# PhucNguyenAH/tacotron2_subword

Hardware: AMD Instinct MI355X
Metric: mel_frames_per_sec_train (higher is better)
Workload: dtype bf16; 1 GPU; BERT_Tacotron2 default hparams (SMA), full training iteration fwd+loss+bwd+clip+Adam, B=64/GPU, 100 phones, 60 sub-word tokens, 400 frames, 80-mel; global_batch=64, frames_per_item=400, parallelism=dp1, torch_ops=loss reductions, cat/transpose copies, persistent_chains=True, recurrent_steps_bf16=True

## Files before the change

include/t2amd.h:

```cpp
#ifndef T2AMD_H
#define T2AMD_H
#include <stddef.h>
#include <stdint.h>

#ifdef __cplusplus
extern "C" {
#endif

#define T2_ATTN_SMA 0
#define T2_ATTN_LSA 1
#define T2_ATTN_DCA 4
#define T2_ATTN_GMM 3
#define T2_ATTN_FWD2 2

enum {
    T2_SITE_PRENET1 = 1, T2_SITE_PRENET2 = 2, T2_SITE_PRENET1_SUB = 3, T2_SITE_PRENET2_SUB = 4,
    T2_SITE_ATT_H = 5, T2_SITE_ATT_C = 6, T2_SITE_ATT_H_SUB = 7, T2_SITE_ATT_C_SUB = 8,
    T2_SITE_DEC_H = 9, T2_SITE_DEC_C = 10, T2_SITE_NOISE = 11, T2_SITE_NOISE_SUB = 12,
    T2_SITE_ENC0 = 16,
    T2_SITE_ENCSUB0 = 20,
    T2_SITE_POSTNET0 = 24
};

const char* t2_last_error(void);
// ... 107 lines not shown
int t2_decoder_forward(const t2_dims* dims, const t2_decoder_weights* w, const t2_decoder_fwd_args* a, void* stream);

typedef struct t2_lstm_grads { float *w_ih, *w_hh, *b_ih, *b_hh; } t2_lstm_grads;
typedef struct t2_attention_grads { float *wq, *wm, *v, *loc_conv, *loc_dense, *mlp_b1, *mlp_w2, *mlp_b2, *dca_T, *dca_bT, *dca_P; } t2_attention_grads;
typedef struct t2_decoder_grads {
    float *prenet_w1, *prenet_w2, *prenet_sub_w1, *prenet_sub_w2;
    t2_lstm_grads att, att_sub;
    t2_attention_grads attn, attn_sub;
    t2_lstm_grads dec;
    float *proj_w, *proj_b, *gate_w, *gate_b;
} t2_decoder_grads;
typedef struct t2_decoder_bwd_layout {
    size_t total_floats;
    size_t ddout, ddin, dgd, dga, dgas, dctx, dctxs, dq, dqs, dv, dvs, dpm, dpms, carry, carrys;
    size_t carryc, carrycs, dlconv, dlconvs, dldense, dldenses;
    size_t dcd, dca, dcas, partd, parta, dp2, dp2s, dp1, dmel_t, dgate_t, dg16a, dg16d, colsum_ws, gemm_ws, gemm_ws_floats;
    size_t chain, chain_floats;
} t2_decoder_bwd_layout;
int t2_decoder_bwd_layout_query(const t2_dims* dims, int B, int T, int Tin, int Tsub, t2_decoder_bwd_layout* out);
typedef struct t2_decoder_bwd_args {
    int B, T, Tin, Tsub;
    const float* memory; const float* memory_sub;
    const float* align; const float* align_sub;
    const float* d_mel;
    const float* d_gate;
    const float* d_align;
    const float* d_align_sub;
    float* d_memory;
    float* d_memory_sub;
    const float* ws;
    float* bws;
    int training; int prenet_dropout; uint64_t seed;
    int defer_weight_grads;
} t2_decoder_bwd_args;
int t2_decoder_backward(const t2_dims* dims, const t2_decoder_weights* w, const t2_decoder_grads* g,
                        const t2_decoder_bwd_args* a, void* stream);

typedef struct t2_decoder_infer_args {
    int B, Tin, Tsub, max_steps, poll_every;
    float gate_threshold;
    const float* memory; const float* memory_sub;
    const int32_t* mem_lengths; const int32_t* sub_lengths;
    float* mel_out;
    float* gate_out;
    float* align;
    float* align_sub;
    int32_t* stop_index;
    int32_t* done_count;
    float* ws;
    int prenet_dropout; uint64_t seed;
    int* steps_run_host;
} t2_decoder_infer_args;
int t2_decoder_infer(const t2_dims* dims, const t2_decoder_weights* w, const t2_decoder_infer_args* a, void* stream);

int t2_finalize_bct(const float* in_btc, float* out_bct, int B, int T, int C, const int32_t* lengths, float fill, void* stream);
int t2_mask_bt(float* x, int B, int T, const int32_t* lengths, float fill, void* stream);

typedef struct t2_conv_bn_args {
    int B, T, Cin, Cout, K;
    const float* x;
    const float* w; const float* bias;
    const float* gamma; const float* beta;
    float* run_mean; float* run_var;
    int training; float eps; int act; float drop_p; uint64_t seed; uint32_t site;
    const float* residual;
    float* z; float* mean; float* invstd; float* var;
    float* y;
    float* ws; size_t ws_floats;
    const void* x16; void* y16; int handoff;
} t2_conv_bn_args;
int t2_conv_bn_forward(const t2_conv_bn_args* a, void* stream);
typedef struct t2_conv_bn_bwd_args {
    int B, T, Cin, Cout, K;
    const float* x; const float* w; const float* gamma; const float* beta;
    const float* z; const float* mean; const float* invstd;
    int training; float eps; int act; float drop_p; uint64_t seed; uint32_t site;
    const float* dy;
    float* dw; float* dbias; float* dgamma; float* dbeta;
    float* dx; int dx_accumulate;
    float* ws; size_t ws_floats;
    const void* x16; int handoff;
} t2_conv_bn_bwd_args;
int t2_conv_bn_backward(const t2_conv_bn_bwd_args* a, void* stream);

int t2_embedding_forward(const int64_t* ids, const float* table, float* out, int rows, int dim, void* stream);
int t2_embedding_backward(const int64_t* ids, const float* dout, float* dtable, int rows, int dim, int vocab, void* stream);

typedef struct t2_lstm_seq_args {
    int nstreams, B, T, H;
    const float* pre[4];
    const float* w_hh[4];
    int reverse[4];
    const int32_t* lengths;
    float* h[4]; long ldh;
    float* c[4];
    float* gates[4];
    float* ws; size_t ws_floats;
} t2_lstm_seq_args;
size_t t2_lstm_seq_chain_ws_floats(int nstreams, int B, int H, int backward);
int t2_lstm_seq_forward(const t2_lstm_seq_args* a, void* stream);
typedef struct t2_lstm_seq_bwd_args {
    int nstreams, B, T, H;
    const float* w_hh[4]; int reverse[4];
    const float* h[4]; long ldh; const float* c[4]; const float* gates[4];
    const float* dh[4]; long lddh;
    float* dpre[4];
    float* dw_hh[4];
    float* ws; size_t ws_floats;
} t2_lstm_seq_bwd_args;
int t2_lstm_seq_backward(const t2_lstm_seq_bwd_args* a, void* stream);

typedef struct t2_gemm_args {
    const float* A; const float* B; float* C; int M, N, K;
    long sam, sak, sbn, sbk, ldc; int batch; long bsA, bsB, bsC;
    float alpha, beta; const float* bias; int act; int crow_mod; long crow_mul;
    float* ws; size_t ws_bytes; int splitk;
} t2_gemm_args;
int t2_gemm_ex(const t2_gemm_args* a, void* stream);
int t2_prof_gemm(const t2_gemm_args* a, int reps, float* ms_total, float* ms_kernel, void* stream);
enum { T2_GEMM_F32_64 = 0, T2_GEMM_F32_128, T2_GEMM_BF16CONV, T2_GEMM_SRC128, T2_GEMM_SRC256, T2_GEMM_SRC256KM };
enum { T2_GEMM_OPERAND_FP32 = 0, T2_GEMM_OPERAND_STAGED, T2_GEMM_OPERAND_CALLER };
typedef struct t2_gemm_plan_opts {
    int conv_a, conv_b, conv_T, conv_C, fp32_only;
    int a16, b16; long lda16, ldb16; int a16_kmajor, b16_kmajor, split16;
} t2_gemm_plan_opts;
typedef struct t2_gemm_plan_info {
    int kernel; const char* name;
    int split;
    int splitk, kchunks;
    int a_src, b_src;
    size_t stage_bytes_a, stage_bytes_b;
} t2_gemm_plan_info;
int t2_gemm_plan(const t2_gemm_args* a, const t2_gemm_plan_opts* opts, t2_gemm_plan_info* out);
enum { T2_CHAIN_LSTM = 0, T2_CHAIN_SMA, T2_CHAIN_LSA, T2_CHAIN_ENC };
enum { T2_CHAIN_FORWARD = 0, T2_CHAIN_BACKWARD };
enum { T2_CHAIN_OK = 0, T2_CHAIN_REFUSE_SHAPE, T2_CHAIN_REFUSE_NO_INSTANCE, T2_CHAIN_REFUSE_DEVICE, T2_CHAIN_REFUSE_CLAIM,
       T2_CHAIN_REFUSE_QUERY_PART, T2_CHAIN_REFUSE_LDS, T2_CHAIN_REFUSE_LSA_RESIDENT, T2_CHAIN_REFUSE_SHORT_MEMORY,
       T2_CHAIN_REFUSE_LSA_SPLIT, T2_CHAIN_REFUSE_NO_SAVED_TILES, T2_CHAIN_REFUSE_WORKSPACE, T2_CHAIN_REFUSALS };
enum { T2_CHAIN_PARTS = 11 };
typedef struct t2_chain_shape {
    int kind, dec, NS, B, H, E, A, P, M, Hd, F, Kc, Tin[2];
    int saved_tiles;
    size_t ws_floats;
} t2_chain_shape;
typedef struct t2_chain_plan_info {
    int covered, reason; const char* reason_text;
    int instance; const char* instance_name; int grid; size_t lds_bytes;
    int UT, RT, CS, MT, lds_Tc, lds_Tin, lds_Jp, lds_Jm, Jp[2], Jm[2];
    size_t q_bytes, total_bytes, ws_bytes;
    size_t part_off[T2_CHAIN_PARTS], part_bytes[T2_CHAIN_PARTS]; const char* part_name[T2_CHAIN_PARTS];
    size_t clear_off, clear_bytes, pass_clear_bytes[3];
} t2_chain_plan_info;
int t2_chain_plan(const t2_chain_shape* shape, int direction, int cus, int claimed, int no_resident, t2_chain_plan_info* out);
enum { T2_PASS_FORWARD = 0, T2_PASS_BACKWARD, T2_PASS_INFER };
enum { T2_PASS_MAX_BOUNDS = 64 };
typedef struct t2_pass_env {
    int precision, split_steps, chain, chain_bwd, overlap, cus, claimed, no_resident, saved_tiles;
} t2_pass_env;
typedef struct t2_pass_chain {
    int asked, on, reason; const char* reason_text;
    int instance; const char* instance_name; int grid;
} t2_pass_chain;
typedef struct t2_scratch_carve {
    size_t w_ih16_off, w_ih16_bytes, dg16_off, dg16_bytes, rest_off, rest_bytes, total_bytes;
} t2_scratch_carve;
typedef struct t2_decoder_pass_plan_info {
    t2_decoder_layout layout; t2_decoder_bwd_layout bwd_layout;
    int use16, split, pre16;
    t2_scratch_carve scratch;
    t2_pass_chain chain_a, chain_b;
    int chained, clear, saves_tiles, overlap;
    int nbounds, bounds[T2_PASS_MAX_BOUNDS];
    int poison_words, poll; size_t shadow_floats;
    int defer, share, chunk_cast; size_t ddin_ws_off, ddin_ws_bytes;
    int dec_wgrads, dec_wgrads_staged, tail_on_side, tail_share;
    t2_scratch_carve tail_scratch;
    int nsplit, lsa_chain, dq_parts;
} t2_decoder_pass_plan_info;
int t2_decoder_pass_plan(const t2_dims* dims, int pass, int B, int T, int Tin, int Tsub, const t2_pass_env* env, int defer_weight_grads,
                         int poll_every, t2_decoder_pass_plan_info* out);
int t2_conv_handoff_plan(const t2_gemm_args* a, const t2_gemm_plan_opts* opts, int* taken, t2_gemm_plan_info* out);
int t2_colsum(const float* x, long ld, int M, int N, float* out, float* scratch, void* stream);
int t2_mask_btc(float* x, int B, int T, int C, const int32_t* lengths, float fill, void* stream);

typedef struct t2_softdtw_plan_info {
    int threads;
    int rows_per_thread;
    int passes;
    size_t d_floats;
    size_t r_floats;
    size_t e_floats;
} t2_softdtw_plan_info;
int t2_softdtw_plan(int B, int N, int M, float gamma, int need_grad, t2_softdtw_plan_info* out);
typedef struct t2_softdtw_dist_args {
    int B, N, M, d;
    const float* x;
    const float* y;
    float* Ds;
} t2_softdtw_dist_args;
int t2_softdtw_dist(const t2_softdtw_dist_args* a, void* stream);
typedef struct t2_softdtw_fwd_args {
// ... 428 lines not shown
```

tacotron2_subword_amd/_lib.py:

```python
from __future__ import annotations

import ctypes as C
import os

import torch

_HERE = os.path.dirname(os.path.abspath(__file__))
LIB_PATH = os.environ.get("T2AMD_LIB") or os.path.join(_HERE, "libt2amd.so")

ATTN_SMA, ATTN_LSA, ATTN_FWD2, ATTN_GMM, ATTN_DCA = 0, 1, 2, 3, 4

SITE = dict(PRENET1=1, PRENET2=2, PRENET1_SUB=3, PRENET2_SUB=4, ATT_H=5, ATT_C=6, ATT_H_SUB=7, ATT_C_SUB=8,
            DEC_H=9, DEC_C=10, NOISE=11, NOISE_SUB=12, ENC0=16, ENCSUB0=20, POSTNET0=24)

_fp = C.POINTER(C.c_float)
_ip = C.POINTER(C.c_int32)


class Dims(C.Structure):
    _fields_ = [("n_mel", C.c_int), ("prenet_dim", C.c_int), ("enc_dim", C.c_int), ("att_rnn_dim", C.c_int),
                ("dec_rnn_dim", C.c_int), ("att_dim", C.c_int), ("loc_filters", C.c_int), ("loc_kernel", C.c_int),
                ("attention_kind", C.c_int), ("p_att_dropout", C.c_float), ("p_dec_dropout", C.c_float),
                ("p_prenet_dropout", C.c_float), ("n_streams", C.c_int),
                ("score_mask_value", C.c_float), ("score_mask_value_sub", C.c_float), ("score_mask_given", C.c_int)]
# ... 15 lines not shown
                ("dec", LstmWeights), ("proj_w", C.c_void_p), ("proj_b", C.c_void_p), ("gate_w", C.c_void_p), ("gate_b", C.c_void_p)]


_LAYOUT_FIELDS = ["total_floats", "x", "p1", "p2", "p1s", "p2s", "pm", "pms", "prea", "preas", "ga", "gas",
                  "cna", "cnas", "ca", "cas", "din", "psel", "psels", "wcum", "wcums", "pred", "gd", "cnd", "cd",
                  "dout", "qs", "qss", "qpart", "w1t", "w16a", "w16as", "w16d", "wt16a", "wt16as", "wt16d", "din16", "dh16",
                  "gemm_ws", "gemm_ws_floats", "chain", "chain_floats", "usave", "usaves", "locsave", "locsaves"]


class DecoderLayout(C.Structure):
    _fields_ = [(n, C.c_size_t) for n in _LAYOUT_FIELDS]


class DecoderFwdArgs(C.Structure):
    _fields_ = [("B", C.c_int), ("T", C.c_int), ("Tin", C.c_int), ("Tsub", C.c_int),
                ("memory", C.c_void_p), ("memory_sub", C.c_void_p), ("mem_lengths", C.c_void_p), ("sub_lengths", C.c_void_p),
                ("mels", C.c_void_p), ("mel_out", C.c_void_p), ("gate_out", C.c_void_p), ("align", C.c_void_p),
                ("align_sub", C.c_void_p), ("ws", C.c_void_p), ("training", C.c_int), ("prenet_dropout", C.c_int),
                ("seed", C.c_uint64), ("phase", C.c_int)]


class DecoderInferArgs(C.Structure):
    _fields_ = [("B", C.c_int), ("Tin", C.c_int), ("Tsub", C.c_int), ("max_steps", C.c_int), ("poll_every", C.c_int),
                ("gate_threshold", C.c_float),
                ("memory", C.c_void_p), ("memory_sub", C.c_void_p), ("mem_lengths", C.c_void_p), ("sub_lengths", C.c_void_p),
                ("mel_out", C.c_void_p), ("gate_out", C.c_void_p), ("align", C.c_void_p), ("align_sub", C.c_void_p),
                ("stop_index", C.c_void_p), ("done_count", C.c_void_p), ("ws", C.c_void_p),
                ("prenet_dropout", C.c_int), ("seed", C.c_uint64), ("steps_run_host", C.POINTER(C.c_int))]


class LstmGrads(C.Structure):
    _fields_ = LstmWeights._fields_


class AttentionGrads(C.Structure):
    _fields_ = AttentionWeights._fields_


class DecoderGrads(C.Structure):
    _fields_ = [("prenet_w1", C.c_void_p), ("prenet_w2", C.c_void_p), ("prenet_sub_w1", C.c_void_p), ("prenet_sub_w2", C.c_void_p),
                ("att", LstmGrads), ("att_sub", LstmGrads), ("attn", AttentionGrads), ("attn_sub", AttentionGrads),
                ("dec", LstmGrads), ("proj_w", C.c_void_p), ("proj_b", C.c_void_p), ("gate_w", C.c_void_p), ("gate_b", C.c_void_p)]


_BWD_LAYOUT_FIELDS = ["total_floats", "ddout", "ddin", "dgd", "dga", "dgas", "dctx", "dctxs", "dq", "dqs", "dv", "dvs",
                      "dpm", "dpms", "carry", "carrys", "carryc", "carrycs", "dlconv", "dlconvs", "dldense", "dldenses", "dcd", "dca", "dcas", "partd", "parta", "dp2", "dp2s", "dp1",
                      "dmel_t", "dgate_t", "dg16a", "dg16d", "colsum_ws", "gemm_ws", "gemm_ws_floats", "chain", "chain_floats"]


class DecoderBwdLayout(C.Structure):
    _fields_ = [(n, C.c_size_t) for n in _BWD_LAYOUT_FIELDS]


class DecoderBwdArgs(C.Structure):
    _fields_ = [("B", C.c_int), ("T", C.c_int), ("Tin", C.c_int), ("Tsub", C.c_int),
                ("memory", C.c_void_p), ("memory_sub", C.c_void_p), ("align", C.c_void_p), ("align_sub", C.c_void_p),
                ("d_mel", C.c_void_p), ("d_gate", C.c_void_p), ("d_align", C.c_void_p), ("d_align_sub", C.c_void_p),
                ("d_memory", C.c_void_p), ("d_memory_sub", C.c_void_p), ("ws", C.c_void_p), ("bws", C.c_void_p),
                ("training", C.c_int), ("prenet_dropout", C.c_int), ("seed", C.c_uint64), ("defer_weight_grads", C.c_int)]


class ConvBnArgs(C.Structure):
    _fields_ = [("B", C.c_int), ("T", C.c_int), ("Cin", C.c_int), ("Cout", C.c_int), ("K", C.c_int),
                ("x", C.c_void_p), ("w", C.c_void_p), ("bias", C.c_void_p), ("gamma", C.c_void_p), ("beta", C.c_void_p),
                ("run_mean", C.c_void_p), ("run_var", C.c_void_p),
                ("training", C.c_int), ("eps", C.c_float), ("act", C.c_int), ("drop_p", C.c_float), ("seed", C.c_uint64),
                ("site", C.c_uint32), ("residual", C.c_void_p),
                ("z", C.c_void_p), ("mean", C.c_void_p), ("invstd", C.c_void_p), ("var", C.c_void_p), ("y", C.c_void_p),
                ("ws", C.c_void_p), ("ws_floats", C.c_size_t),
                ("x16", C.c_void_p), ("y16", C.c_void_p), ("handoff", C.c_int)]


class ConvBnBwdArgs(C.Structure):
    _fields_ = [("B", C.c_int), ("T", C.c_int), ("Cin", C.c_int), ("Cout", C.c_int), ("K", C.c_int),
                ("x", C.c_void_p), ("w", C.c_void_p), ("gamma", C.c_void_p), ("beta", C.c_void_p),
                ("z", C.c_void_p), ("mean", C.c_void_p), ("invstd", C.c_void_p),
                ("training", C.c_int), ("eps", C.c_float), ("act", C.c_int), ("drop_p", C.c_float), ("seed", C.c_uint64),
                ("site", C.c_uint32), ("dy", C.c_void_p),
                ("dw", C.c_void_p), ("dbias", C.c_void_p), ("dgamma", C.c_void_p), ("dbeta", C.c_void_p),
                ("dx", C.c_void_p), ("dx_accumulate", C.c_int), ("ws", C.c_void_p), ("ws_floats", C.c_size_t),
                ("x16", C.c_void_p), ("handoff", C.c_int)]


_P4 = C.c_void_p * 4
_I4 = C.c_int * 4


class LstmSeqArgs(C.Structure):
    _fields_ = [("nstreams", C.c_int), ("B", C.c_int), ("T", C.c_int), ("H", C.c_int),
                ("pre", _P4), ("w_hh", _P4), ("reverse", _I4), ("lengths", C.c_void_p),
                ("h", _P4), ("ldh", C.c_long), ("c", _P4), ("gates", _P4), ("ws", C.c_void_p), ("ws_floats", C.c_size_t)]


class LstmSeqBwdArgs(C.Structure):
    _fields_ = [("nstreams", C.c_int), ("B", C.c_int), ("T", C.c_int), ("H", C.c_int),
                ("w_hh", _P4), ("reverse", _I4), ("h", _P4), ("ldh", C.c_long), ("c", _P4), ("gates", _P4),
                ("dh", _P4), ("lddh", C.c_long), ("dpre", _P4), ("dw_hh", _P4), ("ws", C.c_void_p), ("ws_floats", C.c_size_t)]


class GemmArgs(C.Structure):
    _fields_ = [("A", C.c_void_p), ("B", C.c_void_p), ("C", C.c_void_p), ("M", C.c_int), ("N", C.c_int), ("K", C.c_int),
                ("sam", C.c_long), ("sak", C.c_long), ("sbn", C.c_long), ("sbk", C.c_long), ("ldc", C.c_long),
                ("batch", C.c_int), ("bsA", C.c_long), ("bsB", C.c_long), ("bsC", C.c_long),
                ("alpha", C.c_float), ("beta", C.c_float), ("bias", C.c_void_p), ("act", C.c_int),
                ("crow_mod", C.c_int), ("crow_mul", C.c_long), ("ws", C.c_void_p), ("ws_bytes", C.c_size_t), ("splitk", C.c_int)]


class GemmPlanOpts(C.Structure):
    _fields_ = [("conv_a", C.c_int), ("conv_b", C.c_int), ("conv_T", C.c_int), ("conv_C", C.c_int), ("fp32_only", C.c_int),
                ("a16", C.c_int), ("b16", C.c_int), ("lda16", C.c_long), ("ldb16", C.c_long),
                ("a16_kmajor", C.c_int), ("b16_kmajor", C.c_int), ("split16", C.c_int)]


class GemmPlanInfo(C.Structure):
    _fields_ = [("kernel", C.c_int), ("name", C.c_char_p), ("split", C.c_int), ("splitk", C.c_int), ("kchunks", C.c_int),
                ("a_src", C.c_int), ("b_src", C.c_int), ("stage_bytes_a", C.c_size_t), ("stage_bytes_b", C.c_size_t)]


CHAIN_PARTS = 11
CHAIN_KINDS = dict(lstm=0, sma=1, lsa=2, enc=3)


class ChainShape(C.Structure):
    _fields_ = [(n, C.c_int) for n in ("kind", "dec", "NS", "B", "H", "E", "A", "P", "M", "Hd", "F", "Kc")] + \
               [("Tin", C.c_int * 2), ("saved_tiles", C.c_int), ("ws_floats", C.c_size_t)]


class ChainPlanInfo(C.Structure):
    _fields_ = [("covered", C.c_int), ("reason", C.c_int), ("reason_text", C.c_char_p),
                ("instance", C.c_int), ("instance_name", C.c_char_p), ("grid", C.c_int), ("lds_bytes", C.c_size_t)] + \
               [(n, C.c_int) for n in ("UT", "RT", "CS", "MT", "lds_Tc", "lds_Tin", "lds_Jp", "lds_Jm")] + \
               [("Jp", C.c_int * 2), ("Jm", C.c_int * 2), ("q_bytes", C.c_size_t), ("total_bytes", C.c_size_t), ("ws_bytes", C.c_size_t),
                ("part_off", C.c_size_t * CHAIN_PARTS), ("part_bytes", C.c_size_t * CHAIN_PARTS), ("part_name", C.c_char_p * CHAIN_PARTS),
                ("clear_off", C.c_size_t), ("clear_bytes", C.c_size_t), ("pass_clear_bytes", C.c_size_t * 3)]


PASS_KINDS = dict(forward=0, backward=1, infer=2)
PASS_MAX_BOUNDS = 64


class PassEnv(C.Structure):
    _fields_ = [(n, C.c_int) for n in ("precision", "split_steps", "chain", "chain_bwd", "overlap", "cus", "claimed", "no_resident", "saved_tiles")]


class PassChain(C.Structure):
    _fields_ = [("asked", C.c_int), ("on", C.c_int), ("reason", C.c_int), ("reason_text", C.c_char_p),
                ("instance", C.c_int), ("instance_name", C.c_char_p), ("grid", C.c_int)]


class ScratchCarve(C.Structure):
    _fields_ = [(n, C.c_size_t) for n in ("w_ih16_off", "w_ih16_bytes", "dg16_off", "dg16_bytes", "rest_off", "rest_bytes", "total_bytes")]


class DecoderPassPlanInfo(C.Structure):
    _fields_ = [("layout", DecoderLayout), ("bwd_layout", DecoderBwdLayout)] + \
               [(n, C.c_int) for n in ("use16", "split", "pre16")] + [("scratch", ScratchCarve), ("chain_a", PassChain), ("chain_b", PassChain)] + \
               [(n, C.c_int) for n in ("chained", "clear", "saves_tiles", "overlap", "nbounds")] + [("bounds", C.c_int * PASS_MAX_BOUNDS)] + \
               [("poison_words", C.c_int), ("poll", C.c_int), ("shadow_floats", C.c_size_t)] + \
               [(n, C.c_int) for n in ("defer", "share", "chunk_cast")] + [("ddin_ws_off", C.c_size_t), ("ddin_ws_bytes", C.c_size_t)] + \
               [(n, C.c_int) for n in ("dec_wgrads", "dec_wgrads_staged", "tail_on_side", "tail_share")] + [("tail_scratch", ScratchCarve)] + \
               [(n, C.c_int) for n in ("nsplit", "lsa_chain", "dq_parts")]


class SoftDtwPlanInfo(C.Structure):
    _fields_ = [("threads", C.c_int), ("rows_per_thread", C.c_int), ("passes", C.c_int),
                ("d_floats", C.c_size_t), ("r_floats", C.c_size_t), ("e_floats", C.c_size_t)]
# ... 183 lines not shown


class WaveglowForwardArgs(C.Structure):
    _fields_ = [("B", C.c_int), ("T", C.c_int), ("n_mel", C.c_int), ("n_samples", C.c_long), ("packed", C.c_void_p), ("logdet_w", C.c_void_p),
                ("mel", C.c_void_p), ("audio", C.c_void_p), ("workspace", C.c_void_p), ("z", C.c_void_p), ("log_s_host", C.POINTER(C.c_void_p)),
                ("logdet", C.c_void_p), ("sigma", C.c_float), ("sums", C.c_void_p), ("nll_item", C.c_void_p), ("loss", C.c_void_p),
                ("kernel_ms_host", C.POINTER(C.c_double))]


class WaveglowHeadArgs(C.Structure):
    _fields_ = [("B", C.c_int), ("n_group", C.c_int), ("n_samples", C.c_long), ("audio", C.c_void_p), ("w", C.c_void_p), ("audio_out", C.c_void_p)]


class WaveglowTailArgs(C.Structure):
    _fields_ = [("B", C.c_int), ("nc", C.c_int), ("n_half", C.c_int), ("L", C.c_int), ("n_peel", C.c_int), ("n_group", C.c_int), ("z_offset", C.c_int),
                ("out", C.c_void_p), ("w_end", C.c_void_p), ("b_end", C.c_void_p), ("audio_in", C.c_void_p), ("w_next", C.c_void_p),
                ("audio_out", C.c_void_p), ("z", C.c_void_p), ("log_s", C.c_void_p), ("part_s", C.c_void_p), ("part_z", C.c_void_p)]


class WaveglowBackwardInfo(C.Structure):
    _fields_ = [("L", C.c_long), ("n_tensors", C.c_int), ("saved_bytes", C.c_size_t), ("workspace_bytes", C.c_size_t), ("grad_floats", C.c_size_t),
                ("packed_bwd_bytes", C.c_size_t), ("n_slots", C.c_size_t)]


class WaveglowTrainForwardArgs(C.Structure):
    _fields_ = [("fwd", WaveglowForwardArgs), ("saved", C.c_void_p)]


class WaveglowBackwardArgs(C.Structure):
    _fields_ = [("B", C.c_int), ("T", C.c_int), ("n_mel", C.c_int), ("n_samples", C.c_long), ("packed", C.c_void_p), ("packed_bwd", C.c_void_p),
                ("saved", C.c_void_p), ("mel", C.c_void_p), ("audio", C.c_void_p), ("dz", C.c_void_p), ("dlog_s_host", C.POINTER(C.c_void_p)),
                ("workspace", C.c_void_p), ("grad", C.c_void_p), ("kernel_ms_host", C.POINTER(C.c_double))]


class WaveglowWeightGradArgs(C.Structure):
    _fields_ = [("B", C.c_int), ("M", C.c_int), ("nc", C.c_int), ("n_cond", C.c_int), ("L", C.c_int), ("taps", C.c_int), ("d", C.c_int),
                ("a_rows", C.c_int), ("x_rows", C.c_int),
                ("a", C.c_void_p), ("x", C.c_void_p), ("spect", C.c_void_p), ("dw_x", C.c_void_p), ("dw_spect", C.c_void_p), ("db", C.c_void_p),
                ("workspace", C.c_void_p), ("db2", C.c_void_p)]


class WaveglowStartBackwardArgs(C.Structure):
    _fields_ = [("B", C.c_int), ("nc", C.c_int), ("c", C.c_int), ("n_half", C.c_int), ("L", C.c_int), ("dx", C.c_void_p), ("w_start", C.c_void_p),
                ("audio_in", C.c_void_p), ("d_in", C.c_void_p), ("dw_start", C.c_void_p), ("db_start", C.c_void_p), ("workspace", C.c_void_p)]


class WaveglowHeadBackwardArgs(C.Structure):
    _fields_ = [("B", C.c_int), ("n_group", C.c_int), ("n_samples", C.c_long), ("d_in", C.c_void_p), ("audio", C.c_void_p), ("part", C.c_void_p),
                ("dw", C.c_void_p)]


class WaveglowGateBackwardArgs(C.Structure):
    _fields_ = [("B", C.c_int), ("nc", C.c_int), ("L", C.c_int), ("last", C.c_int), ("dx", C.c_void_p), ("d_out", C.c_void_p), ("w_rs", C.c_void_p),
                ("t", C.c_void_p), ("g", C.c_void_p), ("packed_ws", C.c_void_p), ("du", C.c_void_p), ("acts", C.c_void_p)]


class WaveglowConvBackwardArgs(C.Structure):
    _fields_ = [("B", C.c_int), ("nc", C.c_int), ("n_cond", C.c_int), ("L", C.c_int), ("d", C.c_int), ("first_dx", C.c_int), ("first_spect", C.c_int),
                ("du", C.c_void_p), ("w_in", C.c_void_p), ("w_cond", C.c_void_p), ("packed_ws", C.c_void_p), ("dx", C.c_void_p), ("d_spect", C.c_void_p)]


class WaveglowTailBackwardArgs(C.Structure):
    _fields_ = [("B", C.c_int), ("nc", C.c_int), ("n_half", C.c_int), ("L", C.c_int), ("n_peel", C.c_int), ("n_group", C.c_int), ("z_offset", C.c_int),
                ("out", C.c_void_p), ("w_end", C.c_void_p), ("b_end", C.c_void_p), ("audio_in", C.c_void_p), ("w_next", C.c_void_p), ("d_next", C.c_void_p),
                ("dz", C.c_void_p), ("dlog_s", C.c_void_p), ("d_out", C.c_void_p), ("d_in", C.c_void_p), ("part", C.c_void_p), ("dw_end", C.c_void_p),
                ("db_end", C.c_void_p), ("dw_next", C.c_void_p)]


class WaveglowUpsampleBackwardArgs(C.Structure):
    _fields_ = [("B", C.c_int), ("n_mel", C.c_int), ("T", C.c_int), ("n_group", C.c_int), ("n_samples", C.c_long),
                ("mel", C.c_void_p), ("d_spect", C.c_void_p), ("dw", C.c_void_p), ("db", C.c_void_p)]


WAVEGLOW_KERNELS = ("upsample", "start", "gated_conv", "res_skip", "couple")
WAVEGLOW_FORWARD_KERNELS = ("upsample", "start", "gated_conv", "res_skip", "head", "tail", "sums")
WAVEGLOW_BACKWARD_KERNELS = ("tail_backward", "gate_backward", "conv_backward", "cond_backward", "weight_grad", "weight_grad_reduce", "start_backward",
                             "upsample_backward")
WAVEGLOW_GATED, WAVEGLOW_RES_SKIP, WAVEGLOW_UPSAMPLE = 0, 1, 2

ABI_VERSION = 4

EXPORTS = ["t2_last_error", "t2_version", "t2_chain_status", "t2_chain_status_clear", "t2_debug_report_abort", "t2_debug_occupy", "t2_chain_claimed", "t2_set_precision", "t2_get_precision", "t2_gemm_counts", "t2_set_gemm_split_min_mflop", "t2_set_split_steps", "t2_get_split_steps", "t2_step_counts", "t2_set_overlap", "t2_set_chain", "t2_get_chain", "t2_set_chain_bwd", "t2_set_gemm_staging", "t2_set_gemm_fold", "t2_set_bn_fuse", "t2_get_bn_fuse", "t2_bn_fuse_counts", "t2_side_join", "t2_defer_counts", "t2_decoder_layout_query", "t2_decoder_forward", "t2_decoder_infer",
           "t2_decoder_bwd_layout_query", "t2_decoder_backward", "t2_decoder_pass_plan", "t2_prof_enable", "t2_prof_collect", "t2_adam_chunks", "t2_adam_step", "t2_adam_norm",
           "t2_conv_bn_forward", "t2_conv_bn_backward", "t2_embedding_forward", "t2_embedding_backward",
           "t2_lstm_seq_forward", "t2_lstm_seq_backward", "t2_lstm_seq_chain_ws_floats", "t2_gemm_ex", "t2_prof_gemm", "t2_gemm_plan", "t2_chain_plan", "t2_conv_handoff_plan", "t2_colsum", "t2_mask_btc",
           "t2_finalize_bct", "t2_mask_bt", "t2_gemm", "t2_rng_keep_mask", "t2_rng_normal",
           "t2_softdtw_plan", "t2_softdtw_dist", "t2_softdtw_forward", "t2_softdtw_backward", "t2_softdtw_dist_backward",
           "t2_ssim_plan", "t2_ssim_forward", "t2_ssim_backward",
           "t2_bert_plan", "t2_bert_pack", "t2_bert_forward", "t2_bert_embed_ln", "t2_bert_layernorm", "t2_bert_attention",
           "t2_hifigan_plan", "t2_hifigan_pack", "t2_hifigan_forward", "t2_vocoder_packed_floats", "t2_vocoder_conv1d", "t2_vocoder_conv_transpose1d",
           "t2_stft_plan", "t2_stft_pack", "t2_stft_analysis", "t2_stft_synthesis", "t2_melspec_plan", "t2_melspec_pack", "t2_melspec",
           "t2_waveglow_plan", "t2_waveglow_pack", "t2_waveglow_infer", "t2_waveglow_packed_floats", "t2_waveglow_gated_conv", "t2_waveglow_res_skip",
           "t2_waveglow_upsample", "t2_waveglow_couple", "t2_waveglow_forward_plan", "t2_waveglow_forward", "t2_waveglow_logdet",
           "t2_waveglow_logdet_matrices", "t2_waveglow_head", "t2_waveglow_tail",
           "t2_waveglow_backward_plan", "t2_waveglow_grad_offsets", "t2_waveglow_pack_backward", "t2_waveglow_train_forward", "t2_waveglow_backward",
           "t2_waveglow_weight_grad_ws_floats", "t2_waveglow_weight_grad", "t2_waveglow_gate_backward", "t2_waveglow_conv_backward_packed_floats",
           "t2_waveglow_conv_backward", "t2_waveglow_tail_backward", "t2_waveglow_upsample_backward", "t2_waveglow_start_backward", "t2_waveglow_head_backward"]

_lib = None


def lib() -> C.CDLL:
    global _lib
    if _lib is None:
        if not os.path.exists(LIB_PATH):
            raise RuntimeError(f"{LIB_PATH} is missing: the HIP extension must be built (see __graft_entry__.build); "
                               "there is no CPU fallback for the product path")
        L = C.CDLL(LIB_PATH)
        L.t2_last_error.restype = C.c_char_p
        if L.t2_version() != ABI_VERSION:
            raise RuntimeError(f"{LIB_PATH} speaks ABI version {L.t2_version()}, this binding {ABI_VERSION}: rebuild the library "
                               "(the argument structs differ in size between versions)")
        L.t2_chain_status.argtypes = [C.POINTER(C.c_uint32)]
        L.t2_debug_report_abort.argtypes = [C.c_uint32, C.c_void_p]
        L.t2_debug_occupy.argtypes = [C.c_int, C.c_int, C.c_void_p]
        L.t2_gemm.argtypes = [C.c_void_p, C.c_void_p, C.c_void_p, C.c_int, C.c_int, C.c_int, C.c_long, C.c_long, C.c_long,
                              C.c_long, C.c_long, C.c_void_p, C.c_int, C.c_float, C.c_float, C.c_void_p, C.c_size_t,
                              C.c_int, C.c_void_p]
        L.t2_rng_keep_mask.argtypes = [C.c_uint64, C.c_uint32, C.c_uint32, C.c_float, C.c_void_p, C.c_void_p]
        L.t2_rng_normal.argtypes = [C.c_uint64, C.c_uint32, C.c_uint32, C.c_void_p, C.c_void_p]
        L.t2_decoder_layout_query.argtypes = [C.POINTER(Dims), C.c_int, C.c_int, C.c_int, C.c_int, C.POINTER(DecoderLayout)]
        L.t2_decoder_forward.argtypes = [C.POINTER(Dims), C.POINTER(DecoderWeights), C.POINTER(DecoderFwdArgs), C.c_void_p]
        L.t2_decoder_infer.argtypes = [C.POINTER(Dims), C.POINTER(DecoderWeights), C.POINTER(DecoderInferArgs), C.c_void_p]
        L.t2_decoder_bwd_layout_query.argtypes = [C.POINTER(Dims), C.c_int, C.c_int, C.c_int, C.c_int, C.POINTER(DecoderBwdLayout)]
        L.t2_decoder_backward.argtypes = [C.POINTER(Dims), C.POINTER(DecoderWeights), C.POINTER(DecoderGrads),
                                          C.POINTER(DecoderBwdArgs), C.c_void_p]
        L.t2_decoder_pass_plan.argtypes = [C.POINTER(Dims), C.c_int, C.c_int, C.c_int, C.c_int, C.c_int, C.POINTER(PassEnv), C.c_int, C.c_int,
                                           C.POINTER(DecoderPassPlanInfo)]
        L.t2_conv_bn_forward.argtypes = [C.POINTER(ConvBnArgs), C.c_void_p]
        L.t2_conv_bn_backward.argtypes = [C.POINTER(ConvBnBwdArgs), C.c_void_p]
        L.t2_embedding_forward.argtypes = [C.c_void_p, C.c_void_p, C.c_void_p, C.c_int, C.c_int, C.c_void_p]
        L.t2_embedding_backward.argtypes = [C.c_void_p, C.c_void_p, C.c_void_p, C.c_int, C.c_int, C.c_int, C.c_void_p]
        L.t2_lstm_seq_forward.argtypes = [C.POINTER(LstmSeqArgs), C.c_void_p]
        L.t2_lstm_seq_backward.argtypes = [C.POINTER(LstmSeqBwdArgs), C.c_void_p]
        L.t2_lstm_seq_chain_ws_floats.argtypes, L.t2_lstm_seq_chain_ws_floats.restype = [C.c_int, C.c_int, C.c_int, C.c_int], C.c_size_t
        L.t2_gemm_ex.argtypes = [C.POINTER(GemmArgs), C.c_void_p]
        L.t2_prof_gemm.argtypes = [C.POINTER(GemmArgs), C.c_int, C.POINTER(C.c_float), C.POINTER(C.c_float), C.c_void_p]
        L.t2_gemm_plan.argtypes = [C.POINTER(GemmArgs), C.POINTER(GemmPlanOpts), C.POINTER(GemmPlanInfo)]
        L.t2_chain_plan.argtypes = [C.POINTER(ChainShape), C.c_int, C.c_int, C.c_int, C.c_int, C.POINTER(ChainPlanInfo)]
        L.t2_conv_handoff_plan.argtypes = [C.POINTER(GemmArgs), C.POINTER(GemmPlanOpts), C.POINTER(C.c_int), C.POINTER(GemmPlanInfo)]
        L.t2_colsum.argtypes = [C.c_void_p, C.c_long, C.c_int, C.c_int, C.c_void_p, C.c_void_p, C.c_void_p]
        L.t2_mask_btc.argtypes = [C.c_void_p, C.c_int, C.c_int, C.c_int, C.c_void_p, C.c_float, C.c_void_p]
        L.t2_prof_enable.argtypes = [C.c_int]
        L.t2_gemm_counts.argtypes = [C.POINTER(C.c_uint64), C.c_int]
        L.t2_set_split_steps.argtypes = [C.c_int]
        L.t2_step_counts.argtypes = [C.POINTER(C.c_uint64), C.c_int]
        L.t2_bn_fuse_counts.argtypes = [C.POINTER(C.c_uint64), C.c_int]
        L.t2_defer_counts.argtypes = [C.POINTER(C.c_uint64), C.c_int]
        L.t2_set_gemm_split_min_mflop.argtypes = [C.c_int]
        L.t2_prof_collect.argtypes = [C.c_int, C.POINTER(C.c_double), C.POINTER(C.c_int)]
        L.t2_finalize_bct.argtypes = [C.c_void_p, C.c_void_p, C.c_int, C.c_int, C.c_int, C.c_void_p, C.c_float, C.c_void_p]
        L.t2_mask_bt.argtypes = [C.c_void_p, C.c_int, C.c_int, C.c_void_p, C.c_float, C.c_void_p]
        L.t2_softdtw_plan.argtypes = [C.c_int, C.c_int, C.c_int, C.c_float, C.c_int, C.POINTER(SoftDtwPlanInfo)]
        L.t2_softdtw_dist.argtypes = [C.POINTER(SoftDtwDistArgs), C.c_void_p]
        L.t2_softdtw_forward.argtypes = [C.POINTER(SoftDtwFwdArgs), C.c_void_p]
        L.t2_softdtw_backward.argtypes = [C.POINTER(SoftDtwBwdArgs), C.c_void_p]
        L.t2_softdtw_dist_backward.argtypes = [C.POINTER(SoftDtwDistBwdArgs), C.c_void_p]
        L.t2_ssim_plan.argtypes = [C.c_int, C.c_int, C.c_int, C.c_int, C.c_int, C.POINTER(SsimPlanInfo)]
        L.t2_ssim_forward.argtypes = [C.POINTER(SsimFwdArgs), C.c_void_p]
        L.t2_ssim_backward.argtypes = [C.POINTER(SsimBwdArgs), C.c_void_p]
        L.t2_bert_plan.argtypes = [C.POINTER(BertConfig), C.c_int, C.c_long, C.c_int, C.c_int, C.POINTER(BertPlanInfo)]
        L.t2_bert_pack.argtypes = [C.POINTER(BertConfig), C.POINTER(C.c_void_p), C.c_int, C.c_void_p, C.c_void_p]
        L.t2_bert_forward.argtypes = [C.POINTER(BertConfig), C.POINTER(BertFwdArgs), C.c_void_p]
        L.t2_bert_embed_ln.argtypes = [C.POINTER(BertEmbedLnArgs), C.c_void_p]
        L.t2_bert_layernorm.argtypes = [C.POINTER(BertLayernormArgs), C.c_void_p]
        L.t2_bert_attention.argtypes = [C.POINTER(BertAttentionArgs), C.c_void_p]
        L.t2_hifigan_plan.argtypes = [C.POINTER(HifiganConfig), C.c_int, C.c_int, C.POINTER(HifiganPlanInfo)]
        L.t2_hifigan_pack.argtypes = [C.POINTER(HifiganConfig), C.POINTER(C.c_void_p), C.POINTER(C.c_void_p), C.c_int, C.c_void_p, C.c_void_p]
        L.t2_hifigan_forward.argtypes = [C.POINTER(HifiganConfig), C.POINTER(HifiganFwdArgs), C.c_void_p]
        L.t2_vocoder_packed_floats.argtypes, L.t2_vocoder_packed_floats.restype = [C.c_int, C.c_int, C.c_int, C.c_int], C.c_size_t
        L.t2_vocoder_conv1d.argtypes = [C.POINTER(VocoderConvArgs), C.c_void_p]
        L.t2_vocoder_conv_transpose1d.argtypes = [C.POINTER(VocoderConvArgs), C.c_void_p]
        L.t2_stft_plan.argtypes = [C.c_int, C.c_int, C.c_int, C.POINTER(StftPlanInfo)]
        L.t2_stft_pack.argtypes = [C.c_int, C.c_int, C.c_void_p, C.c_void_p, C.c_void_p, C.c_void_p, C.c_void_p]
        L.t2_stft_analysis.argtypes = [C.POINTER(StftAnalysisArgs), C.c_void_p]
        L.t2_stft_synthesis.argtypes = [C.POINTER(StftSynthesisArgs), C.c_void_p]
        L.t2_melspec_plan.argtypes = [C.c_int, C.c_int, C.c_int, C.c_int, C.c_long, C.c_int, C.POINTER(MelspecPlanInfo)]
        L.t2_melspec_pack.argtypes = [C.c_int, C.c_int, C.c_void_p, C.c_void_p, C.c_void_p, C.c_void_p]
        L.t2_melspec.argtypes = [C.POINTER(MelspecArgs), C.c_void_p]
        L.t2_waveglow_plan.argtypes = [C.POINTER(WaveglowConfig), C.c_int, C.c_int, C.POINTER(WaveglowPlanInfo)]
        L.t2_waveglow_pack.argtypes = [C.POINTER(WaveglowConfig), C.POINTER(C.c_void_p), C.c_int, C.c_void_p, C.c_void_p]
        L.t2_waveglow_infer.argtypes = [C.POINTER(WaveglowConfig), C.POINTER(WaveglowInferArgs), C.c_void_p]
        L.t2_waveglow_packed_floats.argtypes, L.t2_waveglow_packed_floats.restype = [C.c_int, C.c_int, C.c_int, C.c_int], C.c_size_t
        L.t2_waveglow_gated_conv.argtypes = [C.POINTER(WaveglowGatedArgs), C.c_void_p]
        L.t2_waveglow_res_skip.argtypes = [C.POINTER(WaveglowResSkipArgs), C.c_void_p]
        L.t2_waveglow_upsample.argtypes = [C.POINTER(WaveglowUpsampleArgs), C.c_void_p]
        L.t2_waveglow_couple.argtypes = [C.POINTER(WaveglowCoupleArgs), C.c_void_p]
        L.t2_waveglow_forward_plan.argtypes = [C.POINTER(WaveglowConfig), C.c_int, C.c_int, C.c_long, C.POINTER(WaveglowForwardInfo)]
        L.t2_waveglow_forward.argtypes = [C.POINTER(WaveglowConfig), C.POINTER(WaveglowForwardArgs), C.c_void_p]
        L.t2_waveglow_logdet.argtypes = [C.POINTER(WaveglowConfig), C.c_void_p, C.c_void_p, C.c_void_p]
        L.t2_waveglow_logdet_matrices.argtypes = [C.c_void_p, C.c_int, C.c_int, C.c_void_p, C.c_void_p]
        L.t2_waveglow_head.argtypes = [C.POINTER(WaveglowHeadArgs), C.c_void_p]
        L.t2_waveglow_tail.argtypes = [C.POINTER(WaveglowTailArgs), C.c_void_p]
        L.t2_waveglow_backward_plan.argtypes = [C.POINTER(WaveglowConfig), C.c_int, C.c_int, C.c_long, C.POINTER(WaveglowBackwardInfo)]
        L.t2_waveglow_grad_offsets.argtypes = [C.POINTER(WaveglowConfig), C.POINTER(C.c_size_t), C.c_int]
        L.t2_waveglow_pack_backward.argtypes = [C.POINTER(WaveglowConfig), C.POINTER(C.c_void_p), C.c_int, C.c_void_p, C.c_void_p]
        L.t2_waveglow_train_forward.argtypes = [C.POINTER(WaveglowConfig), C.POINTER(WaveglowTrainForwardArgs), C.c_void_p]
        L.t2_waveglow_backward.argtypes = [C.POINTER(WaveglowConfig), C.POINTER(WaveglowBackwardArgs), C.c_void_p]
        L.t2_waveglow_weight_grad_ws_floats.argtypes, L.t2_waveglow_weight_grad_ws_floats.restype = [C.c_int] * 6, C.c_size_t
        L.t2_waveglow_weight_grad.argtypes = [C.POINTER(WaveglowWeightGradArgs), C.c_void_p]
        L.t2_waveglow_gate_backward.argtypes = [C.POINTER(WaveglowGateBackwardArgs), C.c_void_p]
        L.t2_waveglow_conv_backward_packed_floats.argtypes, L.t2_waveglow_conv_backward_packed_floats.restype = [C.c_int, C.c_int], C.c_size_t
        L.t2_waveglow_conv_backward.argtypes = [C.POINTER(WaveglowConvBackwardArgs), C.c_void_p]
        L.t2_waveglow_tail_backward.argtypes = [C.POINTER(WaveglowTailBackwardArgs), C.c_void_p]
        L.t2_waveglow_upsample_backward.argtypes = [C.POINTER(WaveglowUpsampleBackwardArgs), C.c_void_p]
        L.t2_waveglow_start_backward.argtypes = [C.POINTER(WaveglowStartBackwardArgs), C.c_void_p]
        L.t2_waveglow_head_backward.argtypes = [C.POINTER(WaveglowHeadBackwardArgs), C.c_void_p]
        _lib = L
    return _lib


def check(rc: int) -> None:
    if rc != 0:
        raise RuntimeError(f"t2amd call failed ({rc}): {lib().t2_last_error().decode()}")


def ptr(t: torch.Tensor | None) -> int | None:
    if t is None:
        return None
# ... 416 lines not shown
```

tacotron2_subword_amd/blocks.py:

```python
from __future__ import annotations

import ctypes as C

import torch

from . import _lib as L

ACT_NONE, ACT_RELU, ACT_TANH = 0, 1, 2
CONV_HANDOFF = True
_WS = {}


def _scratch(dev, n_floats: int) -> torch.Tensor:
    key = (dev, torch.cuda.current_stream(dev).cuda_stream if dev.type == "cuda" else 0)
    t = _WS.get(key)
    if t is None or t.numel() < n_floats:
        t = torch.empty(int(n_floats * 1.25) + 1024, dtype=torch.float32, device=dev)
        _WS[key] = t
    return t


def _stage_terms() -> int:
    return 3 if L.get_precision() == "bf16x3" else 1


def gemm_ex(A, Bm, out, M, N, K, sam, sak, sbn, sbk, ldc, *, bias=None, act=0, alpha=1.0, beta=0.0, crow_mod=0, crow_mul=0,
            batch=1, bsA=0, bsB=0, bsC=0, splitk_ws=True):
    ws = _scratch(out.device, (8 << 20) * _stage_terms()) if splitk_ws and beta == 0.0 else None
    a = L.GemmArgs(L.ptr(A), L.ptr(Bm), L.ptr(out), M, N, K, sam, sak, sbn, sbk, ldc, batch, bsA, bsB, bsC, alpha, beta,
                   L.ptr(bias), act, crow_mod, crow_mul, L.ptr(ws), 0 if ws is None else ws.numel() * 4, 0)
    L.check(L.lib().t2_gemm_ex(C.byref(a), L.stream()))
    return out


def colsum(x2d: torch.Tensor) -> torch.Tensor:
    M, N = x2d.shape
    out = torch.empty(N, dtype=torch.float32, device=x2d.device)
    sc = torch.empty(64 * N, dtype=torch.float32, device=x2d.device)
    L.check(L.lib().t2_colsum(L.ptr(x2d), x2d.stride(0), M, N, L.ptr(out), L.ptr(sc), L.stream()))
    return out


class _LinearFn(torch.autograd.Function):

    @staticmethod
    def forward(ctx, x, W, b):
        shape = x.shape
        x2 = x.reshape(-1, shape[-1]).contiguous()
        M, K = x2.shape
        N = W.shape[0]
        y = torch.empty(M, N, dtype=torch.float32, device=x.device)
        gemm_ex(x2, W, y, M, N, K, K, 1, W.stride(0), 1, N, bias=b)
        ctx.save_for_backward(x2, W)
        ctx.has_bias, ctx.shape = b is not None, shape
        return y.view(*shape[:-1], N)

    @staticmethod
    def backward(ctx, dy):
        x2, W = ctx.saved_tensors
        M, K = x2.shape
        N = W.shape[0]
        dy2 = dy.reshape(M, N).contiguous()
        dx = dW = db = None
        if ctx.needs_input_grad[0]:
            dx = torch.empty(M, K, dtype=torch.float32, device=dy.device)
            gemm_ex(dy2, W, dx, M, K, N, N, 1, 1, W.stride(0), K)
            dx = dx.view(ctx.shape)
        if ctx.needs_input_grad[1]:
            dW = torch.empty(N, K, dtype=torch.float32, device=dy.device)
            gemm_ex(dy2, x2, dW, N, K, M, 1, N, 1, K, K)
        if ctx.has_bias and ctx.needs_input_grad[2]:
            db = colsum(dy2)
        return dx, dW, db


def linear(x, W, b=None):
    return _LinearFn.apply(x, W, b)


class _EmbeddingFn(torch.autograd.Function):
    @staticmethod
    def forward(ctx, ids, table):
        ids = ids.contiguous().long()
        rows, D = ids.numel(), table.shape[1]
        out = torch.empty(*ids.shape, D, dtype=torch.float32, device=table.device)
        L.check(L.lib().t2_embedding_forward(L.ptr(ids), L.ptr(table), L.ptr(out), rows, D, L.stream()))
        ctx.save_for_backward(ids)
        ctx.vocab = table.shape[0]
        return out

    @staticmethod
    def backward(ctx, dout):
        (ids,) = ctx.saved_tensors
        dout = dout.contiguous()
        D = dout.shape[-1]
        dtable = torch.empty(ctx.vocab, D, dtype=torch.float32, device=dout.device)
        L.check(L.lib().t2_embedding_backward(L.ptr(ids), L.ptr(dout), L.ptr(dtable), ids.numel(), D, ctx.vocab, L.stream()))
        return None, dtable


def embedding(ids, table):
    return _EmbeddingFn.apply(ids, table)


class _ConvStackFn(torch.autograd.Function):

    @staticmethod
    def forward(ctx, x, cfg, *params):
        x = x.contiguous()
        B, T, _ = x.shape
        n = len(cfg["acts"])
        dev = x.device
        saved, cur, cur16 = [], x, None
        handoff = CONV_HANDOFF and L.get_precision() == "bf16"
        for i in range(n):
            w, bias, gamma, beta = params[4 * i:4 * i + 4]
            rm, rv = cfg["buffers"][i]
            Cout, Cin, K = w.shape
            M = B * T
            z = torch.empty(M, Cout, dtype=torch.float32, device=dev)
            y = torch.empty(B, T, Cout, dtype=torch.float32, device=dev)
            st = torch.empty(3, Cout, dtype=torch.float32, device=dev)
            nws = Cout * Cin * K + 4 + 128 * Cout + _stage_terms() * ((M * Cin + Cout * Cin * K) // 2) + 4096
            ws = _scratch(dev, nws)
            res = x if (cfg["residual"] and i == n - 1) else None
            y16 = torch.empty(B, T, Cout, dtype=torch.bfloat16, device=dev) if handoff and i + 1 < n else None
            a = L.ConvBnArgs(B, T, Cin, Cout, K, L.ptr(cur), L.ptr(w.detach()), L.ptr(bias.detach()), L.ptr(gamma.detach()),
                             L.ptr(beta.detach()), L.ptr(rm), L.ptr(rv), int(cfg["training"]), 1e-5, cfg["acts"][i],
                             cfg["drop_p"] if cfg["training"] else 0.0, cfg["seed"], cfg["site0"] + i, L.ptr(res),
                             L.ptr(z), L.ptr(st[0]), L.ptr(st[1]), L.ptr(st[2]), L.ptr(y), L.ptr(ws), ws.numel(),
                             L.ptr(cur16), L.ptr(y16), int(handoff))
            L.check(L.lib().t2_conv_bn_forward(C.byref(a), L.stream()))
            saved.append((cur, z, st, cur16))
            cur, cur16 = y, y16
        ctx.cfg, ctx.saved_acts, ctx.params, ctx.handoff = cfg, saved, [p.detach() for p in params], handoff
        return cur

    @staticmethod
    def backward(ctx, dy):
        cfg, params = ctx.cfg, ctx.params
        n = len(cfg["acts"])
        dev = dy.device
        dy = dy.contiguous()
        d_res = dy if cfg["residual"] else None
        grads = [None] * (4 * n)
        for i in range(n - 1, -1, -1):
            w, bias, gamma, beta = params[4 * i:4 * i + 4]
            xin, z, st, xin16 = ctx.saved_acts[i]
            B, T, Cin = xin.shape
            Cout, _, K = w.shape
            M = B * T
            dw, db = torch.empty_like(w), torch.empty_like(bias)
            dg, dbt = torch.empty_like(gamma), torch.empty_like(beta)
            need_dx = i > 0 or ctx.needs_input_grad[0]
            dx = torch.empty(B, T, Cin, dtype=torch.float32, device=dev) if need_dx else None
            nws = M * Cout + Cout * Cin * K + 128 * Cout + 16 + (8 << 20) + _stage_terms() * ((M * (Cout + K * max(Cin, Cout))) // 2) + Cout * Cin * K
            ws = _scratch(dev, nws)
            a = L.ConvBnBwdArgs(B, T, Cin, Cout, K, L.ptr(xin), L.ptr(w), L.ptr(gamma), L.ptr(beta), L.ptr(z), L.ptr(st[0]), L.ptr(st[1]),
                                int(cfg["training"]), 1e-5, cfg["acts"][i], cfg["drop_p"] if cfg["training"] else 0.0, cfg["seed"],
                                cfg["site0"] + i, L.ptr(dy), L.ptr(dw), L.ptr(db), L.ptr(dg), L.ptr(dbt), L.ptr(dx), 0,
                                L.ptr(ws), ws.numel(), L.ptr(xin16), int(ctx.handoff and L.get_precision() == "bf16"))
            L.check(L.lib().t2_conv_bn_backward(C.byref(a), L.stream()))
            grads[4 * i:4 * i + 4] = [dw, db, dg, dbt]
            dy = dx
        if dy is not None and d_res is not None:
            dy = dy + d_res
        ctx.saved_acts = None
        return (dy, None) + tuple(grads)


def conv_bn_stack(x, layers, acts, *, training, drop_p, seed, site0, residual=False):
    params, buffers = [], []
    for conv, bn in layers:
        params += [conv.weight, conv.bias, bn.weight, bn.bias]
        buffers.append((bn.running_mean, bn.running_var))
        if training:
            bn.num_batches_tracked += 1
    cfg = dict(acts=list(acts), buffers=buffers, training=bool(training), drop_p=float(drop_p), seed=int(seed), site0=int(site0),
               residual=bool(residual))
    return _ConvStackFn.apply(x, cfg, *params)


class _BiLstmFn(torch.autograd.Function):

    @staticmethod
    def forward(ctx, x, lengths, w_ih, w_hh, b_ih, b_hh, w_ih_r, w_hh_r, b_ih_r, b_hh_r):
        B, T, E = x.shape
        H = w_hh.shape[1]
        dev = x.device
        xt = x.transpose(0, 1).contiguous()
        pre = torch.empty(2, T * B, 4 * H, dtype=torch.float32, device=dev)
        bsum = torch.stack((b_ih.detach() + b_hh.detach(), b_ih_r.detach() + b_hh_r.detach()))
        for d, W in enumerate((w_ih, w_ih_r)):
            gemm_ex(xt, W.detach(), pre[d], T * B, 4 * H, E, E, 1, W.stride(0), 1, 4 * H, bias=bsum[d])
        out = torch.empty(T, B, 2 * H, dtype=torch.float32, device=dev)
        cells = torch.empty(2, T, B, H, dtype=torch.float32, device=dev)
        gates = torch.empty(2, T, B, 4 * H, dtype=torch.float32, device=dev)
        a = L.LstmSeqArgs()
        a.nstreams, a.B, a.T, a.H = 2, B, T, H
        a.pre[0], a.pre[1] = pre[0].data_ptr(), pre[1].data_ptr()
        a.w_hh[0], a.w_hh[1] = L.ptr(w_hh.detach()), L.ptr(w_hh_r.detach())
        a.reverse[0], a.reverse[1] = 0, 1
        a.lengths = L.ptr(lengths)
        a.h[0], a.h[1] = out.data_ptr(), out.data_ptr() + 4 * H
        a.ldh = 2 * H
        a.c[0], a.c[1] = cells[0].data_ptr(), cells[1].data_ptr()
        a.gates[0], a.gates[1] = gates[0].data_ptr(), gates[1].data_ptr()
        xws = torch.empty(int(L.lib().t2_lstm_seq_chain_ws_floats(2, B, H, 0)), dtype=torch.float32, device=dev)
        a.ws, a.ws_floats = L.ptr(xws), xws.numel()
        L.check(L.lib().t2_lstm_seq_forward(C.byref(a), L.stream()))
        ctx.save_for_backward(xt, out, cells, gates, w_ih, w_hh, w_ih_r, w_hh_r)
        ctx.dims = (B, T, E, H)
        return out.transpose(0, 1).contiguous()

    @staticmethod
    def backward(ctx, dout):
        xt, out, cells, gates, w_ih, w_hh, w_ih_r, w_hh_r = ctx.saved_tensors
        B, T, E, H = ctx.dims
        dev = dout.device
        dh = dout.transpose(0, 1).contiguous()
        dpre = torch.empty(2, T * B, 4 * H, dtype=torch.float32, device=dev)
        dwhh = torch.empty(2, 4 * H, H, dtype=torch.float32, device=dev)
        nws = max(2 * (B * H + 8 * B * H) + 64, int(L.lib().t2_lstm_seq_chain_ws_floats(2, B, H, 1))) + (8 << 20) * _stage_terms()
        ws = _scratch(dev, nws)
        a = L.LstmSeqBwdArgs()
        a.nstreams, a.B, a.T, a.H = 2, B, T, H
        a.w_hh[0], a.w_hh[1] = L.ptr(w_hh), L.ptr(w_hh_r)
        a.reverse[0], a.reverse[1] = 0, 1
        a.h[0], a.h[1] = out.data_ptr(), out.data_ptr() + 4 * H
        a.ldh = 2 * H
        a.c[0], a.c[1] = cells[0].data_ptr(), cells[1].data_ptr()
        a.gates[0], a.gates[1] = gates[0].data_ptr(), gates[1].data_ptr()
        a.dh[0], a.dh[1] = dh.data_ptr(), dh.data_ptr() + 4 * H
        a.lddh = 2 * H
        a.dpre[0], a.dpre[1] = dpre[0].data_ptr(), dpre[1].data_ptr()
        a.dw_hh[0], a.dw_hh[1] = dwhh[0].data_ptr(), dwhh[1].data_ptr()
        a.ws, a.ws_floats = L.ptr(ws), ws.numel()
        L.check(L.lib().t2_lstm_seq_backward(C.byref(a), L.stream()))
        TB = T * B
        dxt = torch.empty(TB, E, dtype=torch.float32, device=dev)
        res = []
        for d, W in enumerate((w_ih, w_ih_r)):
            gemm_ex(dpre[d], W, dxt, TB, E, 4 * H, 4 * H, 1, 1, W.stride(0), E, beta=float(d))
            dW = torch.empty(4 * H, E, dtype=torch.float32, device=dev)
            gemm_ex(dpre[d], xt, dW, 4 * H, E, TB, 1, 4 * H, 1, E, E)
            db = colsum(dpre[d])
            res.append((dW, dwhh[d], db, db))
        dx = dxt.view(T, B, E).transpose(0, 1).contiguous()
        return (dx, None) + res[0] + res[1]


def bilstm(x, lengths, lstm):
    ln = None if lengths is None else lengths.to(dtype=torch.int32).contiguous()
    return _BiLstmFn.apply(x, ln, lstm.weight_ih_l0, lstm.weight_hh_l0, lstm.bias_ih_l0, lstm.bias_hh_l0,
                           lstm.weight_ih_l0_reverse, lstm.weight_hh_l0_reverse, lstm.bias_ih_l0_reverse, lstm.bias_hh_l0_reverse)
```

tacotron2_subword_amd/build.py:

```python
from __future__ import annotations

import os
import shutil
import subprocess

_HERE = os.path.dirname(os.path.abspath(__file__))
CSRC = os.path.join(_HERE, "csrc")
OUT = os.path.join(_HERE, "libt2amd.so")
SOURCES = ["gemm.hip", "gemm_f32.hip", "gemm_bf16conv.hip", "gemm_dispatch.hip", "lstm.hip", "chain_plan.hip", "chain.hip", "chain_bwd.hip", "chain_enc.hip", "attention.hip", "attention_lsa_bwd.hip", "attention_gmm.hip", "attention_dca.hip", "conv.hip", "elementwise.hip", "infer.hip", "optim.hip", "softdtw.hip", "ssim.hip", "bert.hip", "vocoder.hip", "waveglow.hip", "stft.hip", "melspec.hip", "decoder_plan.hip", "decoder.hip", "c_api.hip"]


def _newest(paths):
    return max(os.path.getmtime(p) for p in paths)


def build(force: bool = False, verbose: bool = False) -> str:
    srcs = [os.path.join(CSRC, s) for s in SOURCES]
    deps = srcs + [os.path.join(CSRC, h) for h in os.listdir(CSRC) if h.endswith(".h")]
    deps.append(os.path.join(os.path.dirname(_HERE), "include", "t2amd.h"))
    if not force and os.path.exists(OUT) and os.path.getmtime(OUT) >= _newest(deps):
        return OUT
    hipcc = shutil.which("hipcc") or "/opt/rocm/bin/hipcc"
    if not os.path.exists(hipcc):
        raise RuntimeError("hipcc not found: cannot build the HIP extension")
    objs = []
    procs = []
    os.makedirs(os.path.join(_HERE, "build"), exist_ok=True)
    for s in srcs:
        o = os.path.join(_HERE, "build", os.path.basename(s) + ".o")
        objs.append(o)
        if not force and os.path.exists(o) and os.path.getmtime(o) >= _newest(deps):
            continue
        cmd = [hipcc, "--offload-arch=gfx950", "-O3", "-std=c++17", "-fPIC", "-Wno-pass-failed"] + os.environ.get("T2_EXTRA_HIPCC_FLAGS", "").split() + ["-c", s, "-o", o]
        if verbose:
            print(" ".join(cmd))
        procs.append((cmd, subprocess.Popen(cmd, stdout=subprocess.PIPE, stderr=subprocess.STDOUT)))
    for cmd, p in procs:
        out, _ = p.communicate()
        if p.returncode != 0:
            raise RuntimeError("hipcc failed: " + " ".join(cmd) + "\n" + out.decode(errors="replace"))
    cmd = [hipcc, "--offload-arch=gfx950", "-shared", "-fPIC", "-o", OUT] + objs
    r = subprocess.run(cmd, stdout=subprocess.PIPE, stderr=subprocess.STDOUT)
    if r.returncode != 0:
        raise RuntimeError("link failed: " + r.stdout.decode(errors="replace"))
    return OUT


if __name__ == "__main__":
    print(build(verbose=True))
```

tacotron2_subword_amd/csrc/c_api.hip:

```cpp
#include <fcntl.h>
#include <stdarg.h>
#include <stdio.h>
#include <sys/file.h>
#include <unistd.h>
#include <stdlib.h>
#include <string.h>

#include "../../include/t2amd.h"
#include "kernels.h"
#include "chain_plan.h"
#include "driver.h"

static thread_local char g_err[512] = "";

void t2_set_error(const char* fmt, ...) {
    va_list ap;
    va_start(ap, fmt);
    vsnprintf(g_err, sizeof(g_err), fmt, ap);
    va_end(ap);
}

#include <algorithm>
#include <mutex>
#include <vector>
// ... 128 lines not shown

extern "C" {

const char* t2_last_error(void) { return g_err; }
int t2_version(void) { return T2_ABI_VERSION; }
int t2_chain_status(uint32_t* out_host) {
    T2_REQUIRE(out_host, "null argument");
    const unsigned* w = chain_sticky_words();
    T2_REQUIRE(w, "t2_chain_status: no status block");
    for (int i = 0; i < 4; ++i) out_host[i] = __atomic_load_n(w + i, __ATOMIC_RELAXED);
    return 0;
}
int t2_chain_status_clear(void) {
    unsigned* w = chain_sticky_words();
    T2_REQUIRE(w, "t2_chain_status_clear: no status block");
    for (int i = 0; i < 4; ++i) __atomic_store_n(w + i, 0u, __ATOMIC_RELAXED);
    return 0;
}
int t2_debug_report_abort(uint32_t code, void* stream) {
    unsigned* w = chain_sticky_words();
    T2_REQUIRE(w, "t2_debug_report_abort: no status block");
    hipLaunchKernelGGL(status_report_kernel, dim3(1), dim3(64), 0, (hipStream_t)stream, w, code);
    T2_LAUNCH_CHECK();
    return 0;
}
int t2_chain_claimed(void) { return chain_device_claim() ? 1 : 0; }
int t2_debug_occupy(int workgroups, int milliseconds, void* stream) {
    T2_REQUIRE(workgroups >= 1 && workgroups <= 256 && milliseconds >= 1 && milliseconds <= 5000, "t2_debug_occupy: 1..256 workgroups, 1..5000 ms");
    unsigned* w = chain_sticky_words();
    T2_REQUIRE(w, "t2_debug_occupy: no status block");
    const size_t smem = 96 * 1024;
    T2_TRY_RC(t2_allow_dynamic_lds(reinterpret_cast<const void*>(occupy_kernel), smem));
    hipLaunchKernelGGL(occupy_kernel, dim3(workgroups), dim3(256), smem, (hipStream_t)stream, (unsigned long long)milliseconds * 100000ull, w + 8);
    T2_LAUNCH_CHECK();
    return 0;
}
int t2_set_precision(int mode) {
    T2_REQUIRE(mode >= 0 && mode <= 2, "t2_set_precision: mode must be 0 (fp32), 1 (bf16 operands) or 2 (split-bf16 large GEMMs), not %d", mode);
    set_precision(mode);
    return 0;
}
int t2_get_precision(void) { return get_precision(); }
int t2_set_gemm_split_min_mflop(int mflop) { set_gemm_split_min_mflop(mflop); return 0; }
int t2_gemm_counts(uint64_t* out_host, int reset) {
    T2_REQUIRE(out_host, "null argument");
    gemm_counts(out_host, reset);
    return 0;
}
int t2_set_split_steps(int on) { g_split_steps = on != 0; return 0; }
int t2_get_split_steps(void) { return g_split_steps; }
int t2_step_counts(uint64_t* out_host, int reset) {
    T2_REQUIRE(out_host, "null argument");
    for (int i = 0; i < 6; ++i) { out_host[i] = g_step_counts[i]; if (reset) g_step_counts[i] = 0; }
    return 0;
}
int t2_set_overlap(int on) { g_overlap = on != 0; return 0; }
int t2_set_chain(int on) { g_chain = on != 0; return 0; }
int t2_get_chain(void) { return g_chain; }
int t2_set_chain_bwd(int on) { g_chain_bwd = on != 0; return 0; }
int t2_set_gemm_staging(int on) { set_gemm_staging(on); return 0; }
int t2_set_gemm_fold(int on) { set_gemm_fold(on); return 0; }
int t2_set_bn_fuse(int on) { set_bn_fuse(on); return 0; }
int t2_get_bn_fuse(void) { return get_bn_fuse(); }
int t2_bn_fuse_counts(uint64_t* out_host, int reset) {
    T2_REQUIRE(out_host, "null argument");
    bn_fuse_counts(out_host, reset);
    return 0;
}
int t2_defer_counts(uint64_t* out_host, int reset) {
    T2_REQUIRE(out_host, "null argument");
    for (int i = 0; i < 2; ++i) { out_host[i] = g_defer_counts[i]; if (reset) g_defer_counts[i] = 0; }
    return 0;
}
int t2_side_join(void* stream) {
    Side* side = nullptr;
    T2_TRY(side_get(&side));
    hipEvent_t e;
    T2_TRY(side_event(*side, 0, &e));
    T2_CHECK_HIP(hipEventRecord(e, side->s));
    T2_CHECK_HIP(hipStreamWaitEvent((hipStream_t)stream, e, 0));
    return 0;
}

int t2_conv_bn_forward(const t2_conv_bn_args* a, void* stream) {
    T2_REQUIRE(a, "null argument");
    const size_t nw = (size_t)a->Cout * a->Cin * a->K;
    T2_REQUIRE(a->ws_floats >= nw + 128 * (size_t)a->Cout, "t2_conv_bn_forward: workspace too small");
    ConvBnFwd f{};
    f.x = a->x; f.B = a->B; f.T = a->T; f.Cin = a->Cin; f.Cout = a->Cout; f.K = a->K;
    f.w = a->w; f.bias = a->bias; f.gamma = a->gamma; f.beta = a->beta; f.run_mean = a->run_mean; f.run_var = a->run_var;
    f.training = a->training; f.eps = a->eps; f.act = a->act; f.drop_p = a->drop_p; f.seed = a->seed; f.site = a->site;
    f.residual = a->residual; f.z = a->z; f.mean = a->mean; f.invstd = a->invstd; f.var = a->var; f.y = a->y;
    f.wperm = a->ws; f.scratch = a->ws + align4(nw);
    const size_t used = align4(nw) + 128 * (size_t)a->Cout;
    if (a->ws_floats > used) { f.gemm_ws = a->ws + used; f.gemm_ws_bytes = (a->ws_floats - used) * sizeof(float); }
    f.handoff = a->handoff; f.x16 = static_cast<const __bf16*>(a->x16); f.y16 = static_cast<__bf16*>(a->y16);
    return conv_bn_fwd(f, (hipStream_t)stream);
}

int t2_conv_bn_backward(const t2_conv_bn_bwd_args* a, void* stream) {
    T2_REQUIRE(a, "null argument");
    const size_t nw = align4((size_t)a->Cout * a->Cin * a->K), ndz = align4((size_t)a->B * a->T * a->Cout), nsc = 128 * (size_t)a->Cout;
    T2_REQUIRE(a->ws_floats >= nw + ndz + nsc, "t2_conv_bn_backward: workspace too small");
    ConvBnBwd f{};
    f.x = a->x; f.B = a->B; f.T = a->T; f.Cin = a->Cin; f.Cout = a->Cout; f.K = a->K;
    f.w = a->w; f.gamma = a->gamma; f.beta = a->beta; f.z = a->z; f.mean = a->mean; f.invstd = a->invstd;
    f.training = a->training; f.eps = a->eps; f.act = a->act; f.drop_p = a->drop_p; f.seed = a->seed; f.site = a->site;
    f.dy = a->dy; f.dw = a->dw; f.dbias = a->dbias; f.dgamma = a->dgamma; f.dbeta = a->dbeta;
    f.dx = a->dx; f.dx_accumulate = a->dx_accumulate;
    f.dz = a->ws; f.wperm = a->ws + ndz; f.scratch = a->ws + ndz + nw;
    f.gemm_ws = a->ws + ndz + nw + nsc; f.gemm_ws_bytes = (a->ws_floats - (ndz + nw + nsc)) * sizeof(float);
    f.handoff = a->handoff; f.x16 = static_cast<const __bf16*>(a->x16);
    return conv_bn_bwd(f, (hipStream_t)stream);
}

int t2_embedding_forward(const int64_t* ids, const float* table, float* out, int rows, int dim, void* stream) {
    return embedding_fwd(reinterpret_cast<const long*>(ids), table, out, rows, dim, (hipStream_t)stream);
}
int t2_embedding_backward(const int64_t* ids, const float* dout, float* dtable, int rows, int dim, int vocab, void* stream) {
    return embedding_bwd(reinterpret_cast<const long*>(ids), dout, dtable, rows, dim, vocab, (hipStream_t)stream);
}

int t2_lstm_seq_forward(const t2_lstm_seq_args* a, void* stream) {
    T2_REQUIRE(a && a->nstreams >= 1 && a->nstreams <= kMaxLstmStreams, "t2_lstm_seq_forward: bad nstreams");
    T2_REQUIRE(a->H % 64 == 0, "t2_lstm_seq_forward: H=%d must be a multiple of 64", a->H);
    const int B = a->B, T = a->T, H = a->H;
    ChainPlan plan{CHAIN_REFUSE_WORKSPACE};
    if (g_chain && a->ws && a->ws_floats) plan = plan_here(plan_enc_chain, enc_chain_shape(a->nstreams, B, H, 0, a->ws_floats * sizeof(float)));
    if (plan.refusal == CHAIN_OK) {
        EncChainDesc d{};
        d.ND = a->nstreams; d.B = B; d.T = T; d.H = H; d.lengths = a->lengths; d.ldh = a->ldh;
        for (int s = 0; s < a->nstreams; ++s) {
            d.pre[s] = a->pre[s]; d.w_hh[s] = a->w_hh[s]; d.reverse[s] = a->reverse[s];
            d.h[s] = a->h[s]; d.c[s] = a->c[s]; d.gates[s] = a->gates[s];
        }
        return enc_chain_fwd(d, plan, a->ws, a->ws_floats, (hipStream_t)stream);
    }
    for (int step = 0; step < T; ++step) {
        LstmStepDesc d{};
        d.nstreams = a->nstreams; d.B = B; d.H = H; d.drop_p = 0.f;
        for (int s = 0; s < a->nstreams; ++s) {
            LstmStream& st = d.st[s];
            const int t = a->reverse[s] ? T - 1 - step : step;
            const int tp = a->reverse[s] ? t + 1 : t - 1;
            st.pre = a->pre[s] + (long)t * B * 4 * H; st.ldpre = 4 * H;
            if (step > 0) {
                st.seg[0] = LstmSeg{a->h[s] + (long)tp * B * a->ldh, a->ldh, a->w_hh[s], (long)H, H};
                st.nseg = 1;
                st.c_prev = a->c[s] + (long)tp * B * H; st.ldc_prev = H;
            }
            st.gates = a->gates[s] + (long)t * B * 4 * H; st.ldgates = 4 * H;
            st.c_out = a->c[s] + (long)t * B * H; st.ldc_out = H;
            st.h_out = a->h[s] + (long)t * B * a->ldh; st.ldh_out = a->ldh;
            st.lengths = a->lengths; st.t = t;
        }
        T2_TRY(lstm_step_fwd(d, (hipStream_t)stream));
    }
    return 0;
}

size_t t2_lstm_seq_chain_ws_floats(int nstreams, int B, int H, int backward) { return enc_chain_ws_floats(nstreams, B, H, backward); }

int t2_lstm_seq_backward(const t2_lstm_seq_bwd_args* a, void* stream) {
    T2_REQUIRE(a && a->nstreams >= 1 && a->nstreams <= kMaxLstmStreams, "t2_lstm_seq_backward: bad nstreams");
    const int B = a->B, T = a->T, H = a->H, ns = a->nstreams;
    const int ks = lstm_bwd_ksplit(4 * H);
    hipStream_t s = (hipStream_t)stream;
    float* dc = a->ws;
    float* part = dc + align4((size_t)ns * B * H);
    float* gws = part + align4((size_t)ns * ks * B * H);
    T2_REQUIRE(a->ws_floats >= (size_t)(gws - a->ws), "t2_lstm_seq_backward: workspace too small");
    const size_t gws_bytes = (a->ws_floats - (size_t)(gws - a->ws)) * sizeof(float);
    ChainPlan plan{CHAIN_REFUSE_WORKSPACE};
    if (g_chain && g_chain_bwd && a->ws_floats) plan = plan_here(plan_enc_chain, enc_chain_shape(ns, B, H, 1, a->ws_floats * sizeof(float)));
    const bool chain = plan.refusal == CHAIN_OK;
    if (chain) {
        EncChainBwdDesc d{};
        d.ND = ns; d.B = B; d.T = T; d.H = H; d.lddh = a->lddh;
        for (int i = 0; i < ns; ++i) {
            d.w_hh[i] = a->w_hh[i]; d.reverse[i] = a->reverse[i]; d.c[i] = a->c[i]; d.gates[i] = a->gates[i];
            d.dh[i] = a->dh[i]; d.dpre[i] = a->dpre[i];
        }
        T2_TRY(enc_chain_bwd(d, plan, a->ws, a->ws_floats, s));
    }
    for (int step = 0; step < (chain ? 0 : T); ++step) {
        LstmBwdPointDesc p{};
        p.nstreams = ns; p.B = B; p.H = H; p.drop_p = 0.f; p.first = step == 0;
        LstmBwdGemmDesc g{};
        g.nstreams = ns; g.B = B; g.H4 = 4 * H; g.KS = ks; g.NC = H;
        for (int i = 0; i < ns; ++i) {
            const int t = a->reverse[i] ? step : T - 1 - step;
            const int tprev = a->reverse[i] ? t + 1 : t - 1;
            const bool has_prev = a->reverse[i] ? (t + 1 < T) : (t > 0);
            LstmBwdStream& st = p.st[i];
            st.dh1 = a->dh[i] + (long)t * B * a->lddh; st.lddh1 = a->lddh;
            st.part = part + (size_t)i * ks * B * H; st.nparts = ks; st.part_stride = (long)B * H; st.ldpart = H; st.part_col = 0;
            st.gates = a->gates[i] + (long)t * B * 4 * H; st.ldgates = 4 * H;
            st.c_new = a->c[i] + (long)t * B * H; st.ldc_new = H;
            if (has_prev) { st.c_prev = a->c[i] + (long)tprev * B * H; st.ldc_prev = H; }
            st.dc_state = dc + (size_t)i * B * H;
            st.dg = a->dpre[i] + (long)t * B * 4 * H; st.lddg = 4 * H;
            g.st[i].dg = st.dg; g.st[i].lddg = 4 * H;
            g.st[i].seg[0] = LstmBwdSeg{a->w_hh[i], (long)H, H}; g.st[i].nseg = 1;
            g.st[i].part = part + (size_t)i * ks * B * H;
        }
        T2_TRY(lstm_bwd_pointwise(p, s));
        if (step + 1 < T) T2_TRY(lstm_bwd_gemm(g, s));
    }
    for (int i = 0; i < ns; ++i) {
        if (T < 2) { T2_TRY(fill_f32(a->dw_hh[i], 0.f, (size_t)4 * H * H, s)); continue; }
        GemmDesc w = gemm_desc();
        const long rowsB = (long)B;
        w.A = a->reverse[i] ? a->dpre[i] : a->dpre[i] + rowsB * 4 * H; w.sam = 1; w.sak = 4 * H;
        w.B = a->reverse[i] ? a->h[i] + rowsB * a->ldh : a->h[i]; w.sbk = a->ldh; w.sbn = 1;
        w.C = a->dw_hh[i]; w.ldc = H; w.M = 4 * H; w.N = H; w.K = (T - 1) * B;
        w.ws = gws; w.ws_bytes = gws_bytes;
        T2_TRY(gemm(w, s));
    }
    return 0;
}

static GemmDesc desc_of(const t2_gemm_args& a) {
    GemmDesc g = gemm_desc();
    g.A = a.A; g.B = a.B; g.C = a.C; g.M = a.M; g.N = a.N; g.K = a.K;
    g.sam = a.sam; g.sak = a.sak; g.sbn = a.sbn; g.sbk = a.sbk; g.ldc = a.ldc;
    g.batch = a.batch > 0 ? a.batch : 1; g.bsA = a.bsA; g.bsB = a.bsB; g.bsC = a.bsC;
    g.alpha = a.alpha; g.beta = a.beta; g.bias1 = a.bias; g.act = a.act;
    g.crow_mod = a.crow_mod; g.crow_mul = a.crow_mul;
    g.ws = a.ws; g.ws_bytes = a.ws_bytes; g.splitk = a.splitk;
    return g;
}
int t2_gemm_ex(const t2_gemm_args* a, void* stream) {
    T2_REQUIRE(a, "null argument");
    return gemm(desc_of(*a), (hipStream_t)stream);
}
static GemmDesc desc_of(const t2_gemm_args& a, const t2_gemm_plan_opts* o) {
    GemmDesc g = desc_of(a);
    if (o) {
        g.conv_a = o->conv_a; g.conv_b = o->conv_b; g.conv_T = o->conv_T; g.conv_C = o->conv_C; g.fp32_only = o->fp32_only;
        const __bf16* copy = reinterpret_cast<const __bf16*>(uintptr_t(256));
        if (o->a16) { g.A16 = copy; g.lda16 = o->lda16; g.a16_kmajor = o->a16_kmajor; }
        if (o->b16) { g.B16 = copy; g.ldb16 = o->ldb16; g.b16_kmajor = o->b16_kmajor; }
        g.split16 = o->split16;
    }
    return g;
}
static t2_gemm_plan_info info_of(const GemmPlan& p) {
    return t2_gemm_plan_info{(int)p.kernel, gemm_plan_name(p), p.split, p.splitk, p.kchunks, (int)p.a.src, (int)p.b.src, p.a.bytes, p.b.bytes};
}
int t2_gemm_plan(const t2_gemm_args* a, const t2_gemm_plan_opts* o, t2_gemm_plan_info* out) {
    T2_REQUIRE(a && out, "null argument");
    GemmPlan p;
    T2_TRY(gemm_plan(desc_of(*a, o), &p));
    *out = info_of(p);
    return 0;
}
int t2_chain_plan(const t2_chain_shape* z, int direction, int cus, int claimed, int no_resident, t2_chain_plan_info* out) {
    T2_REQUIRE(z && out && (direction == T2_CHAIN_FORWARD || direction == T2_CHAIN_BACKWARD), "t2_chain_plan: null argument or bad direction");
    ChainShape c{};
    c.kind = z->kind; c.dec = z->dec; c.NS = z->NS; c.B = z->B; c.H = z->H; c.E = z->E; c.A = z->A; c.P = z->P; c.M = z->M; c.Hd = z->Hd; c.F = z->F; c.Kc = z->Kc;
    c.Tin[0] = z->Tin[0]; c.Tin[1] = z->Tin[1]; c.backward = direction; c.saved_tiles = z->saved_tiles != 0; c.ws_bytes = z->ws_floats * sizeof(float);
    const ChainEnv env{cus, claimed != 0, no_resident != 0};
    const ChainPlan p = z->kind == T2_CHAIN_ENC ? plan_enc_chain(c, env) : direction == T2_CHAIN_BACKWARD ? plan_chain_bwd(c, env) : plan_chain_fwd(c, env);
    t2_chain_plan_info o{};
    o.covered = p.refusal == CHAIN_OK; o.reason = p.refusal; o.reason_text = chain_refusal_text(p.refusal);
    if (o.covered) {
        T2_REQUIRE(p.ws_bytes >= p.total, "t2_chain_plan: exchange space too small (%zu bytes, the chain needs %zu)", p.ws_bytes, p.total);
        o.instance = p.instance; o.instance_name = chain_instance_name(p.instance); o.grid = p.grid; o.lds_bytes = p.lds_bytes;
        o.UT = p.UT; o.RT = p.RT; o.CS = p.CS; o.MT = p.MT; o.lds_Tc = p.lds_Tc; o.lds_Tin = p.lds_Tin; o.lds_Jp = p.lds_Jp; o.lds_Jm = p.lds_Jm;
        for (int s = 0; s < 2; ++s) { o.Jp[s] = p.Jp[s]; o.Jm[s] = p.Jm[s]; }
        o.q_bytes = p.q_bytes; o.total_bytes = p.total; o.ws_bytes = p.ws_bytes;
        static_assert(CHAIN_PARTS == T2_CHAIN_PARTS, "t2_chain_plan_info carries every part");
        for (int i = 0; i < CHAIN_PARTS; ++i) { o.part_off[i] = p.part[i].off; o.part_bytes[i] = p.part[i].bytes; o.part_name[i] = chain_part_name(i); }
        o.clear_off = p.clear.off; o.clear_bytes = p.clear.bytes;
        for (int w = 0; w < 3 && z->kind != T2_CHAIN_ENC && direction == T2_CHAIN_FORWARD; ++w) o.pass_clear_bytes[w] = chain_fwd_clear_range(p.ws_bytes, (ChainWsClear)w).bytes;
    }
    *out = o;
    return 0;
}
int t2_conv_handoff_plan(const t2_gemm_args* a, const t2_gemm_plan_opts* o, int* taken, t2_gemm_plan_info* out) {
    T2_REQUIRE(a && taken && out, "null argument");
    const GemmDesc offered = desc_of(*a, o);
    GemmDesc plain = offered;
    plain.A16 = plain.B16 = nullptr; plain.a16_kmajor = plain.b16_kmajor = 0; plain.lda16 = plain.ldb16 = 0;
    GemmPlan p;
    T2_TRY(gemm_plan(plain, &p));
    *taken = gemm_handoff(plain, offered, &p);
    *out = info_of(p);
    return 0;
}
static int time_gemm(const GemmDesc& g, int reps, float* ms, hipStream_t s) {
    hipEvent_t e0, e1;
    T2_CHECK_HIP(hipEventCreate(&e0)); T2_CHECK_HIP(hipEventCreate(&e1));
    int rc = gemm(g, s);
    T2_CHECK_HIP(hipEventRecord(e0, s));
    for (int i = 0; i < reps && rc == 0; ++i) rc = gemm(g, s);
    T2_CHECK_HIP(hipEventRecord(e1, s));
    T2_CHECK_HIP(hipEventSynchronize(e1));
    T2_CHECK_HIP(hipEventElapsedTime(ms, e0, e1));
    *ms /= reps;
    hipEventDestroy(e0); hipEventDestroy(e1);
    return rc;
}
int t2_prof_gemm(const t2_gemm_args* a, int reps, float* ms_total, float* ms_kernel, void* stream) {
    T2_REQUIRE(a && reps > 0 && ms_total && ms_kernel, "t2_prof_gemm: bad arguments");
    T2_REQUIRE(get_precision() != 0 && a->M % 128 == 0 && a->N % 128 == 0 && a->K % 64 == 0 && (a->batch <= 1) && a->ws,
               "t2_prof_gemm: bf16 or split-bf16 mode, whole-tile shapes and scratch only");
    hipStream_t s = (hipStream_t)stream;
    GemmDesc g = desc_of(*a);
    GemmPlan p, q;
    T2_TRY(gemm_plan(g, &p));
    T2_REQUIRE(p.a.src == GemmSrc::staged && p.b.src == GemmSrc::staged, "t2_prof_gemm: refused, gemm() runs this product on kernel %s, which stages no bf16 copies", gemm_plan_name(p));
    T2_TRY(time_gemm(g, reps, ms_total, s));
    unsigned char* w8 = reinterpret_cast<unsigned char*>(a->ws);
    __bf16* a16 = reinterpret_cast<__bf16*>(w8); __bf16* b16 = reinterpret_cast<__bf16*>(w8 + p.a.bytes);
    T2_TRY(stage_planned(g.A, p.a, p.split, a16, s));
    T2_TRY(stage_planned(g.B, p.b, p.split, b16, s));
    g.A16 = a16; g.lda16 = p.a.ld; g.B16 = b16; g.ldb16 = p.b.ld;
// ... 211 lines not shown
```

tacotron2_subword_amd/csrc/conv.hip:

```cpp
#include "kernels.h"
#include <atomic>
#include <cstdlib>

namespace t2 {

namespace {

inline int env_int(const char* name, int dflt) { const char* v = getenv(name); return v && *v ? atoi(v) : dflt; }
inline int grid_for(size_t n, int block = 256, int cap = 8192) {
    size_t g = (n + block - 1) / block;
    return (int)(g < 1 ? 1 : (g > (size_t)cap ? cap : g));
}

template <class OUT, class IDX>
__global__ void permute_w_fwd_kernel(const float* __restrict__ w, OUT* __restrict__ wp, int Co, int Ci, int K) {
    const IDX n = (IDX)Co * Ci * K;
    for (IDX i = blockIdx.x * (IDX)blockDim.x + threadIdx.x; i < n; i += (IDX)gridDim.x * blockDim.x) {
        const IDX ci = i % (IDX)Ci, r = i / (IDX)Ci, dk = r % (IDX)K, co = r / (IDX)K;
        wp[i] = (OUT)w[(co * Ci + ci) * K + dk];
    }
}
template <class OUT, class IDX>
__global__ void permute_w_bwd_kernel(const float* __restrict__ w, OUT* __restrict__ wt, int Co, int Ci, int K) {
    const IDX n = (IDX)Co * Ci * K;
    for (IDX i = blockIdx.x * (IDX)blockDim.x + threadIdx.x; i < n; i += (IDX)gridDim.x * blockDim.x) {
        const IDX co = i % (IDX)Co, r = i / (IDX)Co, dk = r % (IDX)K, ci = r / (IDX)K;
        wt[i] = (OUT)w[(co * Ci + ci) * K + ((IDX)K - 1 - dk)];
    }
}
template <class OUT>
void permute_w(bool bwd, const float* w, OUT* out, int Co, int Ci, int K, hipStream_t s) {
    const size_t n = (size_t)Co * Ci * K;
    const dim3 grid(grid_for(n)), block(256);
    if (n < (1ull << 31)) {
        if (bwd) hipLaunchKernelGGL((permute_w_bwd_kernel<OUT, uint32_t>), grid, block, 0, s, w, out, Co, Ci, K);
        else hipLaunchKernelGGL((permute_w_fwd_kernel<OUT, uint32_t>), grid, block, 0, s, w, out, Co, Ci, K);
    } else {
        if (bwd) hipLaunchKernelGGL((permute_w_bwd_kernel<OUT, size_t>), grid, block, 0, s, w, out, Co, Ci, K);
        else hipLaunchKernelGGL((permute_w_fwd_kernel<OUT, size_t>), grid, block, 0, s, w, out, Co, Ci, K);
    }
}
__global__ void unpermute_dw_kernel(const float* __restrict__ dwp, float* __restrict__ dw, int Co, int Ci, int K) {
    const size_t n = (size_t)Co * Ci * K;
    for (size_t i = blockIdx.x * (size_t)blockDim.x + threadIdx.x; i < n; i += (size_t)gridDim.x * blockDim.x) {
        const int dk = (int)(i % K); const size_t r = i / K; const int ci = (int)(r % Ci), co = (int)(r / Ci);
        dw[i] = dwp[((size_t)co * K + dk) * Ci + ci];
    }
}

struct BnElem {
    const float* z; const float* mean; const float* invstd; const float* gamma; const float* beta;
    int C; int act; float drop_p; RngKey key;
};
__device__ __forceinline__ float act_fwd(float u, int act) {
    return act == ACT_RELU ? fmaxf(u, 0.f) : (act == ACT_TANH ? tanhf(u) : u);
}

struct BnCol { float mean, inv, ga, be; };
template <int MODE>
__device__ __forceinline__ float colreduce_term(const BnElem& e, const BnCol& k, float scale, float z, float g, uint32_t i,
                                                float& a0, float& a1) {
#pragma clang fp contract(off)
    if (MODE == 0) a0 += z;
    else if (MODE == 1) { const float d = z - k.mean; a0 = fmaf(d, d, a0); }
    else {
        const float xh = (z - k.mean) * k.inv, u = fmaf(xh, k.ga, k.be);
        if (e.drop_p > 0.f) g = rng_keep(e.key, i, e.drop_p) ? g * scale : 0.f;
        if (e.act == ACT_RELU) g = u > 0.f ? g : 0.f;
        else if (e.act == ACT_TANH) { const float t = tanhf(u); g *= fmaf(-t, t, 1.0f); }
        const float gx = g * xh;
        a0 += g; a1 += gx;
    }
    return g;
}
template <int MODE, int V, bool FIN>
__global__ void __launch_bounds__(kColThreads) colreduce_stage1_kernel(BnElem e, const float* __restrict__ dy, float* __restrict__ du,
                                                                       int M, int slabs, float* scratch, float* __restrict__ mean_out) {
    static_assert(!FIN || MODE == 1, "only the centred squares have a sum to finish");
    constexpr int R = MODE == 2 ? (V == 4 ? 8 : 16) : 16;
    static_assert(MODE == 2 || V != 2, "the forward passes run with 16-byte groups or one column per lane");
    const int C = e.C;
    const int lane = threadIdx.x % kColLanes, sub = threadIdx.x / kColLanes;
    const int c = (blockIdx.x * kColLanes + lane) * V;
    const int rows = (M + slabs - 1) / slabs;
    const int m0 = blockIdx.y * rows, m1 = min(M, m0 + rows);
    __shared__ float p0[4][kColLanes * V], p1[4][kColLanes * V];
    __shared__ float fin[FIN ? kColLanes * V : 1];
    if (FIN) {
        block_ordered_sums(scratch, C, slabs, blockIdx.x * kColLanes * V, kColLanes * V, fin);
        __syncthreads();
        scratch += (size_t)slabs * C;
    }
    float a0[V] = {}, a1[V] = {};
    if (c < C) {
        BnCol col[V];
#pragma unroll
        for (int k = 0; k < V; ++k) {
            if (FIN) {
                col[k].mean = fin[lane * V + k] / (float)M;
                if (blockIdx.y == 0 && sub == 0) mean_out[c + k] = col[k].mean;
            } else
                col[k].mean = MODE >= 1 ? e.mean[c + k] : 0.f;
            col[k].inv = MODE == 2 ? e.invstd[c + k] : 0.f; col[k].ga = MODE == 2 ? e.gamma[c + k] : 0.f; col[k].be = MODE == 2 ? e.beta[c + k] : 0.f;
        }
        const float scale = e.drop_p > 0.f ? 1.0f / (1.0f - e.drop_p) : 1.0f;
        struct Row { ColVec<V> z, g; };
        rows_in_flight<R, Row>(m0 + sub, m1,
            [&](int m) {
                const size_t i = (size_t)m * C + c;
                Row r;
                r.z = load_cols<V>(e.z + i);
                if (MODE == 2) r.g = load_cols<V>(dy + i);
                return r;
            },
// ... 169 lines not shown
    if (sub == 0 && c < C) {
#pragma unroll
        for (int k = 0; k < V; ++k) {
            const int l = lane * V + k;
            dbias_part[(size_t)blockIdx.y * C + c + k] = part[0][l] + part[1][l] + part[2][l] + part[3][l];
        }
    }
}
__global__ void invstd_from_var_kernel(const float* var, int C, float eps, float* invstd) {
    const int c = blockIdx.x * blockDim.x + threadIdx.x;
    if (c < C) invstd[c] = 1.0f / sqrtf(var[c] + eps);
}

__global__ void embedding_fwd_kernel(const long* __restrict__ ids, const float* __restrict__ table, float* __restrict__ out, int rows, int D) {
    const size_t n = (size_t)rows * (D / 4);
    for (size_t i = blockIdx.x * (size_t)blockDim.x + threadIdx.x; i < n; i += (size_t)gridDim.x * blockDim.x) {
        const int r = (int)(i / (D / 4)), q = (int)(i % (D / 4));
        reinterpret_cast<f32x4*>(out)[i] = reinterpret_cast<const f32x4*>(table + ids[r] * (long)D)[q];
    }
}
constexpr int kEmbThreads = 256, kEmbWaves = kEmbThreads / 64, kEmbRounds = 32;
template <int V>
__global__ __launch_bounds__(kEmbThreads) void embedding_bwd_kernel(const long* __restrict__ ids, const float* __restrict__ dout,
                                                                    float* __restrict__ dtable, int rows, int D) {
    const int v = blockIdx.x;
    extern __shared__ int hits[];
    __shared__ __attribute__((aligned(16))) int wave_cnt[2][kEmbRounds][kEmbWaves];
    const int tid = threadIdx.x, wave = tid >> 6, lane = tid & 63;
    const unsigned long long below = (1ull << lane) - 1ull;
    int run = 0;
    for (int r0 = 0, it = 0; r0 < rows; r0 += kEmbRounds * kEmbThreads, ++it) {
        long id[kEmbRounds];
#pragma unroll
        for (int j = 0; j < kEmbRounds; ++j) {
            const int r = r0 + j * kEmbThreads + tid;
            id[j] = r < rows ? ids[r] : -1;
        }
        unsigned mine = 0;
#pragma unroll
        for (int j = 0; j < kEmbRounds; ++j) mine |= (id[j] == v ? 1u : 0u) << j;
        int (*wc)[kEmbWaves] = wave_cnt[it & 1];
#pragma unroll
        for (int j = 0; j < kEmbRounds; ++j) {
            const unsigned long long m = __ballot((mine >> j) & 1u);
            if (lane == 0) wc[j][wave] = __popcll(m);
        }
        __syncthreads();
#pragma unroll
        for (int j = 0; j < kEmbRounds; ++j) {
            int base = run, tot = 0;
#pragma unroll
            for (int w = 0; w < kEmbWaves; ++w) { const int cw = wc[j][w]; if (w < wave) base += cw; tot += cw; }
            const bool hit = (mine >> j) & 1u;
            const unsigned long long m = __ballot(hit);
            if (hit) hits[base + __popcll(m & below)] = r0 + j * kEmbThreads + tid;
            run += tot;
        }
    }
    __syncthreads();
    const int nhit = run;
    typedef float vec __attribute__((ext_vector_type(V)));
    for (int c = tid * V; c < D; c += kEmbThreads * V) {
        vec acc = 0.f;
        int h = 0;
        for (; h + 8 <= nhit; h += 8) {
            vec x[8];
#pragma unroll
            for (int j = 0; j < 8; ++j) x[j] = *reinterpret_cast<const vec*>(dout + (size_t)hits[h + j] * D + c);
#pragma unroll
            for (int j = 0; j < 8; ++j) acc += x[j];
        }
        for (; h < nhit; ++h) acc += *reinterpret_cast<const vec*>(dout + (size_t)hits[h] * D + c);
        *reinterpret_cast<vec*>(dtable + (size_t)v * D + c) = acc;
    }
}

bool bn_vectorisable(const BnElem& e, const void* p, const void* q) {
    for (const void* a : {(const void*)e.z, (const void*)e.mean, (const void*)e.invstd, (const void*)e.gamma, (const void*)e.beta, p, q})
        if (!cols_vectorisable(a, e.C, e.C)) return false;
    return true;
}
inline bool aligned8(const void* p) { return (reinterpret_cast<uintptr_t>(p) & 7) == 0; }
inline size_t round256(size_t n) { return (n + 255) & ~(size_t)255; }
inline bool same_route(const GemmPlan& p, const GemmPlan& q) { return p.kernel == q.kernel && p.split == q.split && p.splitk == q.splitk && p.kchunks == q.kchunks; }

std::atomic<int> g_bn_fuse{env_int("T2_BN_FUSE", 1)};
std::atomic<uint64_t> g_bn_counts[3];

inline int col_blocks(int C, int V) { return (C + V * kColLanes - 1) / (V * kColLanes); }
int col_width(int C, int slabs, bool vec, bool narrow) {
    if (!vec) return 1;
    if (narrow && slabs >= 48) {
        for (int v = 4; v > 1; v >>= 1)
            if (col_blocks(C, v) * slabs * (kColThreads / kWave) >= 2048) return v;
        return 1;
    }
    return 4;
}

template <int MODE, bool FIN>
int colreduce_stage1(const BnElem& e, const float* dy, float* du, int M, float* scratch, float* mean_out, int V, hipStream_t s) {
    const int slabs = col_slabs(M);
    const dim3 grid(col_blocks(e.C, V), slabs), block(kColThreads);
    if (V == 4) hipLaunchKernelGGL((colreduce_stage1_kernel<MODE, 4, FIN>), grid, block, 0, s, e, dy, du, M, slabs, scratch, mean_out);
    else if constexpr (MODE == 2) {
        if (V == 2) hipLaunchKernelGGL((colreduce_stage1_kernel<2, 2, false>), grid, block, 0, s, e, dy, du, M, slabs, scratch, mean_out);
        else hipLaunchKernelGGL((colreduce_stage1_kernel<2, 1, false>), grid, block, 0, s, e, dy, du, M, slabs, scratch, mean_out);
    } else hipLaunchKernelGGL((colreduce_stage1_kernel<MODE, 1, FIN>), grid, block, 0, s, e, dy, du, M, slabs, scratch, mean_out);
    T2_LAUNCH_CHECK();
    return 0;
}
template <int MODE>
int colreduce(const BnElem& e, const float* dy, float* du, int M, float eps, float* out0, float* out1, float* scratch, hipStream_t s) {
    const int slabs = col_slabs(M);
    const bool vec = cols_vectorisable(e.z, e.C, e.C) && cols_vectorisable(dy, e.C, e.C) && cols_vectorisable(du, e.C, e.C);
    T2_TRY_RC((colreduce_stage1<MODE, false>(e, dy, du, M, scratch, nullptr, col_width(e.C, slabs, vec, false), s)));
    hipLaunchKernelGGL(colreduce_stage2_kernel, dim3((e.C + 255) / 256), dim3(256), 0, s, scratch, e.C, slabs, M, MODE, eps, out0, out1,
                       (const float*)nullptr, 0.f, (float*)nullptr, (float*)nullptr);
    T2_LAUNCH_CHECK();
    return 0;
}

}

void set_bn_fuse(int on) { g_bn_fuse = on != 0; }
int get_bn_fuse() { return g_bn_fuse; }
void bn_fuse_counts(uint64_t* out, int reset) {
    for (int i = 0; i < 3; ++i) { out[i] = g_bn_counts[i]; if (reset) g_bn_counts[i] = 0; }
}

int conv_bn_fwd(const ConvBnFwd& a, hipStream_t s) {
    const int M = a.B * a.T;
    T2_REQUIRE(a.Cin % 4 == 0 && a.K % 2 == 1, "conv_bn_fwd: Cin=%d must be a multiple of 4 and the kernel size odd (%d)", a.Cin, a.K);
    T2_REQUIRE((size_t)M * a.Cout < (1ull << 32), "conv_bn_fwd: B*T*Cout too large for 32-bit RNG indices");
    const size_t nw = (size_t)a.Cout * a.Cin * a.K;
    GemmDesc g = gemm_desc();
    g.A = a.x; g.conv_a = 1; g.conv_T = a.T; g.conv_C = a.Cin; g.conv_pad = (a.K - 1) / 2;
    g.B = a.wperm; g.sbn = (long)a.K * a.Cin; g.sbk = 1;
    g.C = a.z; g.ldc = a.Cout; g.M = M; g.N = a.Cout; g.K = a.K * a.Cin; g.bias1 = a.bias;
    g.ws = a.gemm_ws; g.ws_bytes = a.gemm_ws_bytes;
    GemmDesc g16 = g;
    g16.A16 = a.x16; g16.lda16 = a.Cin;
    g16.B16 = reinterpret_cast<const __bf16*>(a.wperm); g16.ldb16 = (long)a.K * a.Cin;
    if (a.handoff && gemm_handoff(g, g16)) {
        g = g16;
        permute_w(false, a.w, reinterpret_cast<__bf16*>(a.wperm), a.Cout, a.Cin, a.K, s);
    } else
        permute_w(false, a.w, a.wperm, a.Cout, a.Cin, a.K, s);
    T2_LAUNCH_CHECK();
    T2_TRY_RC(gemm(g, s));
    BnElem e{a.z, a.mean, a.invstd, a.gamma, a.beta, a.Cout, a.act, a.drop_p, rng_key(a.seed, a.site)};
    const size_t n = (size_t)M * a.Cout;
    if (a.training && get_bn_fuse()) {
        const int slabs = col_slabs(M);
        const int V = col_width(e.C, slabs, cols_vectorisable(e.z, e.C, e.C), false);
        T2_TRY_RC((colreduce_stage1<0, false>(e, nullptr, nullptr, M, a.scratch, nullptr, V, s)));
        T2_TRY_RC((colreduce_stage1<1, true>(e, nullptr, nullptr, M, a.scratch, a.mean, V, s)));
        hipLaunchKernelGGL(colreduce_stage2_kernel, dim3((a.Cout + 255) / 256), dim3(256), 0, s, a.scratch + (size_t)slabs * e.C, a.Cout, slabs, M, 1,
                           a.eps, a.invstd, a.var, a.mean, 0.1f, a.run_mean, a.run_var);
        T2_LAUNCH_CHECK();
        ++g_bn_counts[0];
    } else if (a.training) {
        T2_TRY_RC(colreduce<0>(e, nullptr, nullptr, M, a.eps, a.mean, nullptr, a.scratch, s));
        T2_TRY_RC(colreduce<1>(e, nullptr, nullptr, M, a.eps, a.invstd, a.var, a.scratch, s));
        if (a.run_mean) {
            hipLaunchKernelGGL(bn_running_kernel, dim3((a.Cout + 255) / 256), dim3(256), 0, s, a.mean, a.var, a.Cout, M, 0.1f, a.run_mean, a.run_var);
            T2_LAUNCH_CHECK();
        }
    } else {
        T2_CHECK_HIP(hipMemcpyAsync(a.mean, a.run_mean, sizeof(float) * a.Cout, hipMemcpyDeviceToDevice, s));
        hipLaunchKernelGGL(invstd_from_var_kernel, dim3((a.Cout + 255) / 256), dim3(256), 0, s, a.run_var, a.Cout, a.eps, a.invstd);
        T2_LAUNCH_CHECK();
    }
    if (bn_vectorisable(e, a.residual, a.y) && aligned8(a.y16))
        hipLaunchKernelGGL(bn_apply_kernel<4>, dim3(grid_for(n / 4)), dim3(256), 0, s, e, a.residual, a.y, a.y16, n);
    else
        hipLaunchKernelGGL(bn_apply_kernel<1>, dim3(grid_for(n)), dim3(256), 0, s, e, a.residual, a.y, a.y16, n);
    T2_LAUNCH_CHECK();
    return 0;
}

int conv_bn_bwd(const ConvBnBwd& a, hipStream_t s) {
    const int M = a.B * a.T;
    const size_t n = (size_t)M * a.Cout;
    BnElem e{a.z, a.mean, a.invstd, a.gamma, a.beta, a.Cout, a.act, a.drop_p, rng_key(a.seed, a.site)};
    GemmDesc g = gemm_desc();
    g.A = a.dz; g.sam = 1; g.sak = a.Cout;
    g.B = a.x; g.conv_b = 1; g.conv_T = a.T; g.conv_C = a.Cin; g.conv_pad = (a.K - 1) / 2;
    g.C = a.wperm; g.ldc = (long)a.K * a.Cin; g.M = a.Cout; g.N = a.K * a.Cin; g.K = M;
    g.ws = a.gemm_ws; g.ws_bytes = a.gemm_ws_bytes;
    const bool fold = get_gemm_fold() != 0;
    if (fold) { g.C = a.dw; g.ccol_mod = a.Cin; g.ccol_mul = a.K; }
    GemmDesc h = gemm_desc();
    h.A = a.dz; h.conv_a = 1; h.conv_T = a.T; h.conv_C = a.Cout; h.conv_pad = (a.K - 1) / 2;
    h.B = a.wperm; h.sbn = (long)a.K * a.Cout; h.sbk = 1;
    h.C = a.dx; h.ldc = a.Cin; h.M = M; h.N = a.Cin; h.K = a.K * a.Cout;
    h.beta = a.dx_accumulate ? 1.f : 0.f;
    h.ws = a.gemm_ws; h.ws_bytes = a.gemm_ws_bytes;
    if (a.dx) T2_REQUIRE(a.Cout % 4 == 0, "conv_bn_bwd: Cout=%d must be a multiple of 4", a.Cout);
    __bf16* dz16 = nullptr;
    bool w16 = false;
    const size_t dz16_bytes = round256(n * sizeof(__bf16));
    if (a.handoff && a.gemm_ws && (reinterpret_cast<uintptr_t>(a.gemm_ws) & 15) == 0 && a.gemm_ws_bytes >= dz16_bytes) {
        float* behind = a.gemm_ws + dz16_bytes / sizeof(float);
        GemmDesc g16 = g, h16 = h;
        g16.ws = h16.ws = behind; g16.ws_bytes = h16.ws_bytes = a.gemm_ws_bytes - dz16_bytes;
        g16.A16 = h16.A16 = reinterpret_cast<const __bf16*>(a.gemm_ws);
        g16.lda16 = a.Cout; g16.a16_kmajor = 1; h16.lda16 = a.Cout;
        g16.B16 = a.x16; g16.ldb16 = a.Cin; g16.b16_kmajor = 1;
        h16.B16 = reinterpret_cast<const __bf16*>(a.wperm); h16.ldb16 = (long)a.K * a.Cout;
        const bool tw = gemm_handoff(g, g16);
        bool tx = a.dx && gemm_handoff(h, h16);
        if (tx && !tw) {
            GemmDesc gb = g;
            gb.ws = behind; gb.ws_bytes = g16.ws_bytes;
            if (same_route(plan_gemm(g), plan_gemm(gb))) g = gb; else tx = false;
        }
        if (tw) g = g16;
        if (tx) { h = h16; w16 = true; }
        if (tw || tx) dz16 = reinterpret_cast<__bf16*>(a.gemm_ws);
    }
    const size_t nw = (size_t)a.Cout * a.Cin * a.K;
    if (get_bn_fuse()) {
        const int slabs = col_slabs(M);
        const bool vec = cols_vectorisable(e.z, e.C, e.C) && cols_vectorisable(a.dy, e.C, e.C) && cols_vectorisable(a.dz, e.C, e.C);
        const int V = col_width(e.C, slabs, vec, true);
        T2_TRY_RC((colreduce_stage1<2, false>(e, a.dy, a.dz, M, a.scratch, nullptr, V, s)));
        float* part = (size_t)a.Cin * a.K >= 64 ? a.wperm : nullptr;
        const dim3 grid(col_blocks(e.C, V), slabs), block(kColThreads);
        if (V == 4) hipLaunchKernelGGL(bn_bwd_dz_cols_kernel<4>, grid, block, 0, s, e, a.dz, a.scratch, M, slabs, a.training, a.dz, dz16, a.dbeta, a.dgamma, part);
        else if (V == 2) hipLaunchKernelGGL(bn_bwd_dz_cols_kernel<2>, grid, block, 0, s, e, a.dz, a.scratch, M, slabs, a.training, a.dz, dz16, a.dbeta, a.dgamma, part);
        else hipLaunchKernelGGL(bn_bwd_dz_cols_kernel<1>, grid, block, 0, s, e, a.dz, a.scratch, M, slabs, a.training, a.dz, dz16, a.dbeta, a.dgamma, part);
        T2_LAUNCH_CHECK();
        if (part) T2_TRY_RC(colsum_finish(part, M, a.Cout, a.dbias, s));
        else T2_TRY_RC(colsum(a.dz, a.Cout, M, a.Cout, a.dbias, nullptr, a.scratch, s));
        ++g_bn_counts[part ? 1 : 2];
    } else {
        T2_TRY_RC(colreduce<2>(e, a.dy, a.dz, M, a.eps, a.dbeta, a.dgamma, a.scratch, s));
        if (bn_vectorisable(e, a.dz, a.dbeta) && cols_vectorisable(a.dgamma, e.C, e.C))
            hipLaunchKernelGGL(bn_bwd_dz_kernel<4>, dim3(grid_for(n / 4)), dim3(256), 0, s, e, a.dz, a.dbeta, a.dgamma, M, a.training, a.dz, dz16, n);
        else
            hipLaunchKernelGGL(bn_bwd_dz_kernel<1>, dim3(grid_for(n)), dim3(256), 0, s, e, a.dz, a.dbeta, a.dgamma, M, a.training, a.dz, dz16, n);
        T2_LAUNCH_CHECK();
        T2_TRY_RC(colsum(a.dz, a.Cout, M, a.Cout, a.dbias, nullptr, a.scratch, s));
    }
    T2_TRY_RC(gemm(g, s));
    if (!fold) {
        hipLaunchKernelGGL(unpermute_dw_kernel, dim3(grid_for(nw)), dim3(256), 0, s, a.wperm, a.dw, a.Cout, a.Cin, a.K);
        T2_LAUNCH_CHECK();
    }
    if (a.dx) {
        if (w16) permute_w(true, a.w, reinterpret_cast<__bf16*>(a.wperm), a.Cout, a.Cin, a.K, s);
        else permute_w(true, a.w, a.wperm, a.Cout, a.Cin, a.K, s);
        T2_LAUNCH_CHECK();
        T2_TRY_RC(gemm(h, s));
    }
    return 0;
}

int embedding_fwd(const long* ids, const float* table, float* out, int rows, int D, hipStream_t s) {
    T2_REQUIRE(D % 4 == 0, "embedding: dim %d must be a multiple of 4", D);
    hipLaunchKernelGGL(embedding_fwd_kernel, dim3(grid_for((size_t)rows * (D / 4))), dim3(256), 0, s, ids, table, out, rows, D);
    T2_LAUNCH_CHECK();
    return 0;
}
int embedding_bwd(const long* ids, const float* dout, float* dtable, int rows, int D, int vocab, hipStream_t s) {
    const size_t smem = (size_t)rows * sizeof(int);
    T2_REQUIRE(smem <= 150 * 1024, "embedding_bwd: %d tokens do not fit the LDS hit list", rows);
    const bool vec = cols_vectorisable(dout, D, D) && cols_vectorisable(dtable, D, D);
    const void* fn = vec ? reinterpret_cast<const void*>(embedding_bwd_kernel<4>) : reinterpret_cast<const void*>(embedding_bwd_kernel<1>);
    T2_TRY_RC(t2_allow_dynamic_lds(fn, smem));
    if (vec) hipLaunchKernelGGL(embedding_bwd_kernel<4>, dim3(vocab), dim3(kEmbThreads), smem, s, ids, dout, dtable, rows, D);
    else hipLaunchKernelGGL(embedding_bwd_kernel<1>, dim3(vocab), dim3(kEmbThreads), smem, s, ids, dout, dtable, rows, D);
    T2_LAUNCH_CHECK();
    return 0;
}

}
```

tacotron2_subword_amd/csrc/decoder.hip:

```cpp
#include <stdlib.h>
#include <string.h>

#include <algorithm>
#include <mutex>
#include <unordered_map>
#include <vector>

#include "../../include/t2amd.h"
#include "kernels.h"
#include "chain_plan.h"
#include "decoder_plan.h"
#include "driver.h"

using namespace t2;

__global__ __launch_bounds__(256) void poison_if_aborted_kernel(const unsigned* __restrict__ status, int nwords, float* __restrict__ a, size_t na,
                                                                float* __restrict__ b, size_t nb) {
    unsigned any = 0;
    for (int i = 0; i < nwords; ++i) any |= status[i];
    if (!any) return;
    const float qnan = __builtin_nanf("");
    for (size_t i = (size_t)blockIdx.x * 256 + threadIdx.x; i < na; i += (size_t)gridDim.x * 256) a[i] = qnan;
    for (size_t i = (size_t)blockIdx.x * 256 + threadIdx.x; i < nb; i += (size_t)gridDim.x * 256) b[i] = qnan;
}
// ... 60 lines not shown
void saved_tiles_note(const void* ws, bool saved) {
    std::lock_guard<std::mutex> lk(g_saved_mu);
    if (g_saved_tiles.size() > 4096) g_saved_tiles.clear();
    g_saved_tiles[ws] = saved;
}
bool saved_tiles_have(const void* ws) {
    std::lock_guard<std::mutex> lk(g_saved_mu);
    auto it = g_saved_tiles.find(ws);
    return it != g_saved_tiles.end() && it->second;
}

PassEnv pass_env_here(const void* fwd_ws, bool device) {
    PassEnv env{get_precision(), g_split_steps != 0, g_chain != 0, g_chain_bwd != 0, g_overlap != 0, ChainEnv{0, false, false}, fwd_ws && saved_tiles_have(fwd_ws)};
    if (device && env.chain) env.chain_env = chain_env(false);
    return env;
}
template <class Plan>
auto pass_plan_here(PassEnv env, Plan plan) {
    auto p = plan(env);
    if (p.chain_a.on || p.chain_b.on) { env.chain_env = chain_env(true); p = plan(env); }
    return p;
}

void shape_into(const ChainShape& z, ChainDesc* d) {
    d->kind = z.kind; d->dec = z.dec; d->NS = z.NS; d->B = z.B; d->H = z.H; d->E = z.E; d->A = z.A; d->P = z.P; d->M = z.M; d->Hd = z.Hd; d->F = z.F; d->Kc = z.Kc;
    d->st[0].Tin = z.Tin[0]; d->st[1].Tin = z.Tin[1];
}
void shape_into(const ChainShape& z, ChainBwdDesc* d) {
    d->kind = z.kind; d->NS = z.NS; d->B = z.B; d->H = z.H; d->E = z.E; d->A = z.A; d->F = z.F; d->Kc = z.Kc;
    d->st[0].Tin = z.Tin[0]; d->st[1].Tin = z.Tin[1];
}

struct Dec {
    const t2_dims& d; const t2_decoder_weights& w; const DecPlan p; float* ws;
    bool training; bool prenet_dropout; uint64_t seed; hipStream_t s;
    int max_pos;
    const Sizes& z = p.z; const t2_decoder_layout& L = p.L; const InferShadows& I = p.I; const bool teacher = p.teacher;
    StreamRef st[2]{};
    hipStream_t sd = nullptr;
    Dec(const Dec&) = delete;
    __bf16* RowA(int parity, int s) const { return reinterpret_cast<__bf16*>(ws + I.rows_a) + (size_t)(parity * 2 + s) * z.B * I.Ka; }
    __bf16* RowD(int parity) const { return reinterpret_cast<__bf16*>(ws + I.rows_d) + (size_t)parity * z.B * I.Kd; }
    float* P(size_t off) const { return ws + off; }
    __bf16* P16(size_t off) const { return reinterpret_cast<__bf16*>(ws + off); }
    unsigned char* scratch(size_t off) const { return reinterpret_cast<unsigned char*>(ws + L.gemm_ws) + off; }
    GemmDesc in(const ScratchPart& part, GemmDesc m) const { m.ws = reinterpret_cast<float*>(scratch(part.off)); m.ws_bytes = part.bytes; return m; }
    long R(int t) const { return (long)t * z.B; }
};

GemmDesc product(const float* A, long sam, long sak, const float* B, long sbn, long sbk, float* C, long ldc, int M, int N, int K) {
    GemmDesc g = gemm_desc();
    g.A = A; g.sam = sam; g.sak = sak;
    g.B = B; g.sbn = sbn; g.sbk = sbk;
    g.C = C; g.ldc = ldc; g.M = M; g.N = N; g.K = K;
    return g;
}
GemmDesc linear(const float* X, long ldx, const float* W, long ldw, float* Y, long ldy, int M, int N, int K) {
    return product(X, ldx, 1, W, ldw, 1, Y, ldy, M, N, K);
}

int prenet(const Dec& c, int s, const float* X, long ldx, int M, float* P1, float* P2, long ldp, uint32_t base, uint32_t mstride) {
    const Sizes& z = c.z; const StreamRef& r = c.st[s];
    auto layer = [&](const float* in, long ldin, const float* W, int K, float* out, uint32_t site) {
        GemmDesc g = linear(in, ldin, W, K, out, ldp, M, z.P, K);
        g.act = ACT_RELU;
        if (c.prenet_dropout) {
            g.drop_p = c.d.p_prenet_dropout; g.seed = c.seed; g.site = site;
            g.drop_base = base; g.drop_mstride = mstride;
        }
        return gemm(g, c.s);
    };
    T2_TRY(layer(X, ldx, r.prenet_w1, z.M, P1, r.site_p1));
    return layer(P1, ldp, r.prenet_w2, z.P, P2, r.site_p2);
}

int cast_part(const float* src, long lds, __bf16* dst, size_t lo, long ldd, int rows, int cols, bool transpose, bool split, hipStream_t s) {
    if (split) return transpose ? cast_transpose_split_bf16(src, lds, dst, dst + lo, ldd, rows, cols, s) : cast_rows_split_bf16(src, lds, dst, dst + lo, ldd, rows, cols, s);
    return transpose ? cast_transpose_bf16(src, lds, dst, ldd, rows, cols, s) : cast_rows_bf16(src, lds, dst, ldd, rows, cols, s);
}
int cast_shadows(const Dec& c, bool split) {
    const Sizes& z = c.z;
    const long K = z.Ha + z.E, ldi = z.P + z.E;
    const size_t loa = (size_t)4 * z.Ha * K, lod = (size_t)4 * z.Hd * z.Hd;
    for (int s = 0; s < z.NS; ++s) {
        const t2_lstm_weights& lw = *c.st[s].lw;
        __bf16 *f = c.P16(c.st[s].w16), *tr = c.P16(c.st[s].wt16);
        T2_TRY(cast_part(lw.w_hh, z.Ha, f, loa, K, 4 * z.Ha, z.Ha, false, split, c.s));
        T2_TRY(cast_part(lw.w_ih + z.P, ldi, f + z.Ha, loa, K, 4 * z.Ha, z.E, false, split, c.s));
        T2_TRY(cast_part(lw.w_ih + z.P, ldi, tr, loa, 4 * z.Ha, 4 * z.Ha, z.E, true, split, c.s));
        T2_TRY(cast_part(lw.w_hh, z.Ha, tr + (long)z.E * 4 * z.Ha, loa, 4 * z.Ha, 4 * z.Ha, z.Ha, true, split, c.s));
    }
    T2_TRY(cast_part(c.w.dec.w_hh, z.Hd, c.P16(c.L.w16d), lod, z.Hd, 4 * z.Hd, z.Hd, false, split, c.s));
    return cast_part(c.w.dec.w_hh, z.Hd, c.P16(c.L.wt16d), lod, 4 * z.Hd, 4 * z.Hd, z.Hd, true, split, c.s);
}

AttnKind kernel_kind(int kind) {
    return kind == T2_ATTN_GMM ? AttnKind::GMM : kind == T2_ATTN_DCA ? AttnKind::DCA : kind == T2_ATTN_SMA ? AttnKind::SMA : AttnKind::LSA;
}

DcaWeights dca_weights(const t2_attention_weights& aw) {
    DcaWeights w{};
    w.bW = aw.mlp_b1; w.V = aw.mlp_w2; w.F = aw.loc_conv; w.U = aw.loc_dense; w.T = aw.dca_T; w.bT = aw.dca_bT; w.v = aw.v; w.P = aw.dca_P;
    return w;
}

int att_lstm_step(const Dec& c, int t) {
    const Sizes& z = c.z; const t2_decoder_layout& L = c.L;
    LstmStepDesc d{};
    d.nstreams = z.NS; d.B = z.B; d.H = z.Ha; d.seed = c.seed;
    d.drop_p = c.training ? c.d.p_att_dropout : 0.f;
    float* DIN = c.P(L.din);
    for (int s = 0; s < z.NS; ++s) {
        LstmStream& st = d.st[s]; const StreamRef& r = c.st[s];
        const t2_lstm_weights& lw = *r.lw;
        const int hoff = r.hoff, coff = r.coff;
        int n = 0;
        if (!c.teacher) {
            st.seg[n++] = LstmSeg{c.P(r.p2) + c.R(t) * z.P, (long)z.P, lw.w_ih, (long)(z.P + z.E), z.P};
            st.bias1 = lw.b_ih; st.bias2 = lw.b_hh;
        } else {
            st.pre = c.P(r.prea) + c.R(t) * 4 * z.Ha; st.ldpre = 4 * z.Ha;
        }
        if (t > 0) {
            st.seg[n++] = LstmSeg{DIN + c.R(t - 1) * z.WD + coff, (long)z.WD, lw.w_ih + z.P, (long)(z.P + z.E), z.E};
            st.seg[n++] = LstmSeg{DIN + c.R(t - 1) * z.WD + hoff, (long)z.WD, lw.w_hh, (long)z.Ha, z.Ha};
            st.c_prev = c.P(r.ca) + c.R(t - 1) * z.Ha; st.ldc_prev = z.Ha;
        }
        st.nseg = n;
        st.gates = c.P(r.ga) + c.R(t) * 4 * z.Ha; st.ldgates = 4 * z.Ha;
        st.c_new = c.P(r.cna) + c.R(t) * z.Ha; st.ldc_new = z.Ha;
        st.c_out = c.P(r.ca) + c.R(t) * z.Ha; st.ldc_out = z.Ha;
        st.h_out = DIN + c.R(t) * z.WD + hoff; st.ldh_out = z.WD;
        st.site_h = r.site_h; st.site_c = r.site_c;
        st.idx_base = (uint32_t)(c.R(t) * z.Ha); st.idx_bstride = (uint32_t)z.Ha;
        st.wq = r.aw->wq; st.A = z.A;
        st.qpart = c.P(L.qpart) + (size_t)s * (z.Ha / 8) * z.B * z.A;
        if (c.p.use16 && !c.teacher) {
            st.nseg = 0;
            st.x16 = c.RowA(t & 1, s); st.ldx16 = c.I.Ka; st.w16 = c.P16(c.I.wa[s]); st.ldw16 = c.I.Ka; st.k16 = c.I.Ka;
            st.h16_out = c.RowA((t + 1) & 1, s); st.ldh16 = c.I.Ka;
            st.h16_out2 = c.RowD(t & 1) + hoff; st.ldh16_2 = c.I.Kd;
        } else if (c.p.use16) {
            __bf16* D16 = c.P16(L.din16);
            st.nseg = 0;
            st.x16 = D16 + (t > 0 ? c.R(t - 1) * z.WD + hoff : 0); st.ldx16 = z.WD;
            st.w16 = c.P16(r.w16); st.ldw16 = z.Ha + z.E; st.k16 = t > 0 ? z.Ha + z.E : 0;
            st.h16_out = D16 + c.R(t) * z.WD + hoff; st.ldh16 = z.WD;
        } else if (c.p.split && c.teacher) {
            st.nseg = 0;
            st.xs = DIN + (t > 0 ? c.R(t - 1) * z.WD + hoff : 0); st.ldxs = z.WD;
            st.w16 = c.P16(r.w16); st.w16lo = c.P16(split_lo_a(z, r.w16)); st.ldw16 = z.Ha + z.E; st.k16 = t > 0 ? z.Ha + z.E : 0;
        }
    }
    ProfScope ps(PK_LSTM_ATT_FWD, c.s);
    int family = 0;
    return counted(lstm_step_fwd(d, c.s, &family), 0, family);
}

int attention_step(const Dec& c, int t) {
    const Sizes& z = c.z; const t2_decoder_layout& L = c.L;
    AttnStepDesc d{};
    d.nstreams = z.NS; d.B = z.B; d.A = z.A; d.E = z.E;
    const int abi_kind = c.d.attention_kind; d.kind = kernel_kind(abi_kind);
    d.F = c.d.loc_filters; d.Kc = c.d.loc_kernel; d.seed = c.seed; d.first = t == 0;
    d.noise_std = (c.training && abi_kind == T2_ATTN_SMA) ? 2.0f : 0.f;
    d.max_pos = c.max_pos;
// ... 887 lines not shown
```

tacotron2_subword_amd/csrc/gemm.hip:

```cpp
#include "gemm_common.h"

namespace t2 {
namespace gemm_detail {
namespace {
struct Raw16 { bf16x8 a[4], b[4]; unsigned ok; };
template <bool CONV_A>
__device__ __forceinline__ void issue16(const __bf16* __restrict__ A, long lda, const __bf16* __restrict__ B, long ldb, int k0,
                                        ConvAddr cv, const int (&tpos)[4], Raw16& r) {
    r.ok = ~0u;
    int shift = 0, ka = k0;
    if constexpr (CONV_A) { const int dk = k0 / cv.C; ka = k0 - dk * cv.C; shift = dk - cv.pad; }
#pragma unroll
    for (int i = 0; i < 4; ++i) {
        const int q = threadIdx.x + i * 256;
        long row = q >> 3;
        if constexpr (CONV_A) {
            const bool ok = (unsigned)(tpos[i] + shift) < (unsigned)cv.T;
            if (ok) row += shift; else r.ok &= ~(1u << i);
        }
        r.a[i] = *reinterpret_cast<const bf16x8*>(A + row * lda + ka + (q & 7) * 8);
    }
#pragma unroll
    for (int i = 0; i < 4; ++i) {
        const int q = threadIdx.x + i * 256;
// ... 386 lines not shown
template <bool SPLIT>
__global__ void stage_kc_kernel(const float* __restrict__ src, long ld, __bf16* __restrict__ dst, int rows, int K, int lo_slot, int row_group) {
    const int k8 = K >> 3;
    const long total = (long)rows * k8;
    for (long t = blockIdx.x * (long)blockDim.x + threadIdx.x; t < total; t += (long)gridDim.x * blockDim.x) {
        const long row = t / k8; const int k = (int)(t - row * k8) * 8;
        const float* p = src + row * ld + k;
        const f32x4 lo4 = *reinterpret_cast<const f32x4*>(p), hi4 = *reinterpret_cast<const f32x4*>(p + 4);
        if constexpr (SPLIT) {
            long o, step;
            if (row_group) { o = ((row / row_group) * 3 * row_group + row % row_group) * (long)K + k; step = (long)row_group * K; }
            else { o = row * 3 * (long)K + (k >> 6) * 192 + (k & 63); step = 64; }
            store_cast8<true>(dst + o, step, lo_slot, lo4, hi4);
        } else {
            store_cast8<false>(dst + row * (long)K + k, 0, 0, lo4, hi4);
        }
    }
}
template <bool SPLIT>
__global__ __launch_bounds__(256) void stage_mc_kernel(const float* __restrict__ src, long ld, __bf16* __restrict__ dst, int rows, int K, int lo_slot) {
    __shared__ float tile[64][65];
    const int r0 = blockIdx.x * 64, k0 = blockIdx.y * 64;
#pragma unroll
    for (int i = 0; i < 4; ++i) {
        const int k = (threadIdx.x >> 4) + 16 * i, r4 = (threadIdx.x & 15) * 4;
        const f32x4 v = *reinterpret_cast<const f32x4*>(src + (long)(k0 + k) * ld + r0 + r4);
#pragma unroll
        for (int j = 0; j < 4; ++j) tile[k][r4 + j] = v[j];
    }
    __syncthreads();
    constexpr int T = SPLIT ? 3 : 1;
#pragma unroll
    for (int i = 0; i < 2; ++i) {
        const int kg = threadIdx.x & 7, row = (threadIdx.x >> 3) + 32 * i;
        f32x4 a, b;
#pragma unroll
        for (int j = 0; j < 4; ++j) { a[j] = tile[kg * 8 + j][row]; b[j] = tile[kg * 8 + 4 + j][row]; }
        store_cast8<SPLIT>(dst + (long)(r0 + row) * T * K + T * (long)k0 + kg * 8, 64, lo_slot, a, b);
    }
}

int launch_stage(const float* src, bool kc, long ld, __bf16* dst, int rows, int K, bool split, int lo_slot, int row_group, hipStream_t s) {
    if (kc) {
        long blocks = ((long)rows * (K >> 3) + 255) / 256;
        if (blocks > 8192) blocks = 8192;
        hipLaunchKernelGGL(split ? stage_kc_kernel<true> : stage_kc_kernel<false>, dim3((unsigned)blocks), dim3(256), 0, s, src, ld, dst, rows, K, lo_slot, row_group);
    } else {
        hipLaunchKernelGGL(split ? stage_mc_kernel<true> : stage_mc_kernel<false>, dim3(rows / 64, K / 64), dim3(256), 0, s, src, ld, dst, rows, K, lo_slot);
    }
    T2_LAUNCH_CHECK();
    return 0;
}

}

int launch_gemm_bf16src(const GemmK& g, GemmKernel kernel, const __bf16* pa, long lda, const __bf16* pb, long ldb, dim3 grid, hipStream_t s) {
    const GemmDesc& d = g.d;
    if (kernel == GemmKernel::src256km && d.conv_b) return launch_bf16src256<false, true, true>(g, pa, lda, pb, ldb, grid, s);
    if (kernel == GemmKernel::src256km) return launch_bf16src256<false, true, false>(g, pa, lda, pb, ldb, grid, s);
    if (kernel == GemmKernel::src256 && d.conv_a) return launch_bf16src256<true, false, false>(g, pa, lda, pb, ldb, grid, s);
    if (kernel == GemmKernel::src256) return launch_bf16src256<false, false, false>(g, pa, lda, pb, ldb, grid, s);
    if (d.conv_a) return launch_bf16src<true>(g, pa, lda, pb, ldb, grid, s);
    return launch_bf16src<false>(g, pa, lda, pb, ldb, grid, s);
}

}

using gemm_detail::aligned16;

int stage_bf16(const float* src, bool kc, long ld, __bf16* dst, int rows, int K, hipStream_t s) {
    T2_REQUIRE(rows > 0 && K > 0 && rows % 64 == 0 && K % 64 == 0 && ld % 4 == 0 && aligned16(src) && aligned16(dst),
               "stage_bf16: rows=%d K=%d ld=%ld must be whole 64-tiles of 16-byte aligned rows", rows, K, ld);
    return gemm_detail::launch_stage(src, kc, ld, dst, rows, K, false, 0, 0, s);
}

int stage_split_bf16(const float* src, bool kc, long ld, __bf16* dst, int rows, int K, int lo_slot, int row_group, hipStream_t s) {
    T2_REQUIRE(rows > 0 && K > 0 && rows % 64 == 0 && K % 64 == 0 && ld % 4 == 0 && aligned16(src) && aligned16(dst) &&
               (lo_slot == 1 || lo_slot == 2) && row_group >= 0 && (!row_group || (kc && rows % row_group == 0)),
               "stage_split_bf16: rows=%d K=%d ld=%ld must be whole 64-tiles of 16-byte aligned rows", rows, K, ld);
    return gemm_detail::launch_stage(src, kc, ld, dst, rows, K, true, lo_slot, row_group, s);
}

int stage_planned(const float* src, const GemmOperandPlan& o, bool split, __bf16* dst, hipStream_t s) {
    return gemm_detail::launch_stage(src, o.kc, o.ld_src, dst, o.rows, o.K, split, o.lo_slot, o.row_group, s);
}

}
```

tacotron2_subword_amd/csrc/kernels.h:

```cpp
#pragma once
#include "common.h"

namespace t2 {

enum Act : int { ACT_NONE = 0, ACT_RELU = 1, ACT_TANH = 2, ACT_GELU = 3 };

struct GemmDesc {
    const float* A; const float* B; float* C;
    int M, N, K;
    long sam, sak;
    long sbn, sbk;
    long ldc;
    int batch; long bsA, bsB, bsC;
    float alpha, beta;
    const float* bias1; const float* bias2;
    int act;
    float drop_p; uint64_t seed; uint32_t site;
    uint32_t drop_base, drop_mstride;
    float* ws; size_t ws_bytes;
    int splitk;
    int conv_a, conv_b, conv_T, conv_C, conv_pad;
    int fp32_only;
    const __bf16* A16; long lda16;
    const __bf16* B16; long ldb16;
// ... 228 lines not shown

struct ChainBwdStream {
    const __bf16* wt16; long ldwt;
    const float* dh1; long lddh1;
    const float* gates; const float* c_new; const float* c_out;
    float* dg;
    float* dc_state;
    float* dbias_part;
    uint32_t site_h, site_c;
    const float* dctx_a; long lddctx_a;
    const float* dctx_b; long lddctx_b;
    const float* dalign;
    const float* qs;
    const float* pm; const float* memory; int Tin;
    const float* psel; const float* align;
    const float* v; const float* wq;
    float* dctx_out;
    float* dq_out;
    float* dv_acc;
    float* dpm_acc;
    const float* wcum;
    const float* usave; const float* locsave;
    const float* loc_conv; const float* loc_dense;
    float* dconv_acc; float* ddense_acc;
    const __bf16* wdt16;
};
struct ChainBwdDesc {
    ChainBwdStream st[2]; int NS, B, T, t0, t1, H, kind;
    int E, A, F, Kc;
    float drop_p; uint64_t seed;
    unsigned char* X; unsigned char* PB; unsigned* err; unsigned pb_bytes;
    unsigned char* PBC; unsigned pbc_bytes; float* DQX; float* CARRYX;
    int lds_Tc;
};
size_t chain_bwd_ws_floats(int kind, int NS, int B, int Ha, int E, int A, int F, int Kc, int Hd);

struct EncChainDesc {
    int ND, B, T, H;
    const float* pre[2];
    const float* w_hh[2];
    int reverse[2];
    const int* lengths;
    float* h[2]; long ldh;
    float* c[2]; float* gates[2];
    float* X; unsigned* cnt; unsigned* err;
};
struct EncChainBwdDesc {
    int ND, B, T, H;
    const float* w_hh[2]; int reverse[2];
    const float* c[2]; const float* gates[2];
    const float* dh[2]; long lddh;
    float* dpre[2];
    float* X; float* PB; unsigned* cnt; unsigned* err;
};
size_t enc_chain_ws_floats(int ND, int B, int H, int backward);

struct StepTailDesc {
    int B, M, P, WO, NS, t;
    int do_proj, do_prenet;
    const float* dout; long lddout;
    const float* proj_w; const float* proj_b; const float* gate_w; const float* gate_b;
    float* mel_out; long ldmel; float* gate_out; long ldgate;
    float thr; int32_t* stop_index; int32_t* done;
    const float* x_in; long ldx_in;
    const float* w1t[2]; const float* w2[2];
    float* p1[2]; float* p2[2]; long ldp;
    __bf16* p2_16[2]; long ldp16;
    float drop_p; uint64_t seed; uint32_t site1[2], site2[2]; uint32_t drop_base, drop_mstride;
};
int step_tail(const StepTailDesc& d, hipStream_t s);

struct ConvBnFwd {
    const float* x; int B, T, Cin, Cout, K;
    const float* w; const float* bias;
    const float* gamma; const float* beta; float* run_mean; float* run_var;
    int training; float eps; int act; float drop_p; uint64_t seed; uint32_t site;
    const float* residual;
    float* z; float* mean; float* invstd; float* var;
    float* y;
    float* wperm; float* scratch;
    float* gemm_ws; size_t gemm_ws_bytes;
    int handoff;
    const __bf16* x16; __bf16* y16;
};
int conv_bn_fwd(const ConvBnFwd& a, hipStream_t s);
void set_bn_fuse(int on);
int get_bn_fuse();
void bn_fuse_counts(uint64_t* out, int reset);
struct ConvBnBwd {
    const float* x; int B, T, Cin, Cout, K;
    const float* w; const float* gamma; const float* beta;
    const float* z; const float* mean; const float* invstd;
    int training; float eps; int act; float drop_p; uint64_t seed; uint32_t site;
    const float* dy;
    float* dz;
    float* dw; float* dbias; float* dgamma; float* dbeta;
    float* dx; int dx_accumulate;
    float* wperm; float* scratch; float* gemm_ws; size_t gemm_ws_bytes;
    int handoff;
    const __bf16* x16;
};
int conv_bn_bwd(const ConvBnBwd& a, hipStream_t s);
int embedding_fwd(const long* ids, const float* table, float* out, int rows, int D, hipStream_t s);
int embedding_bwd(const long* ids, const float* dout, float* dtable, int rows, int D, int vocab, hipStream_t s);

constexpr int kSoftDtwMaxLen = 8192;
struct SoftDtwPlan { int threads, rows_per_thread, passes; size_t d_floats, r_floats, e_floats; };
int softdtw_plan(int B, int N, int M, float gamma, int need_grad, SoftDtwPlan* out);
struct SoftDtwDist { int B, N, M, d; const float* x; const float* y; float* Ds; };
int softdtw_dist(const SoftDtwDist& a, hipStream_t s);
struct SoftDtwArgs {
    int B, N, M; float gamma, bandwidth;
    const float* D; const float* Ds; const int* x_lengths; const int* y_lengths;
    float* R; float* value; float* E;
};
int softdtw_fwd(const SoftDtwArgs& a, hipStream_t s);
int softdtw_bwd(const SoftDtwArgs& a, hipStream_t s);
struct SoftDtwDistBwd {
    int B, N, M, d; const float* x; const float* y; const float* E; const float* grad_out;
    const int* x_lengths; const int* y_lengths; float* dX; float* dY;
};
int softdtw_dist_bwd(const SoftDtwDistBwd& a, hipStream_t s);

constexpr int kSsimTileH = 16, kSsimTileW = 64;
constexpr int kSsimMaxWs = 31;
struct SsimPlan { int tile_h, tile_w, tiles_h, tiles_w; long partials, partials_t; size_t partial_bytes, map_bytes, lds_fwd_bytes, lds_bwd_bytes; };
int ssim_plan(long N, long H, long W, int ws, int need_grad, SsimPlan* out);
struct SsimImage { float* p; long sn, sr, sc; };
struct SsimFwd {
    int B, C, H, W, ws, need_grad;
    SsimImage x, y, map;
    const float* taps;
    double* partial; double* coef;
    float* value; float* items;
};
int ssim_fwd(const SsimFwd& a, hipStream_t s);
struct SsimBwd {
    int B, C, H, W, ws, need_grad, per_item;
    SsimImage x, y, dx, dy;
    const float* taps; const double* coef; const float* grad;
};
int ssim_bwd(const SsimBwd& a, hipStream_t s);

constexpr int kVocTT = 128;
constexpr int kVocMaxPad = 60;
constexpr int kHifiganMaxUps = 6, kHifiganMaxKernels = 6, kHifiganMaxDilations = 3;
struct VocConv {
    int B, Cin, Cout; long L; int k, d, u;
    const float* x; const float* packed; const float* bias; const float* res; float* y;
    float slope; int accumulate; float scale;
};
size_t voc_packed_floats(int Cin, int Cout, int k, int u);
int voc_pack(const float* w, float* packed, int Cin, int Cout, int k, int u, hipStream_t s);
int voc_conv(const VocConv& a, hipStream_t s);
struct HifiganConfig {
    int resblock, n_mel, upsample_initial_channel;
    int num_upsamples, upsample_rates[kHifiganMaxUps], upsample_kernel_sizes[kHifiganMaxUps];
    int num_kernels, resblock_kernel_sizes[kHifiganMaxKernels];
    int num_dilations, resblock_dilation_sizes[kHifiganMaxKernels][kHifiganMaxDilations];
};
struct HifiganLayer { int kind, cin, cout, k, d, u; size_t w_off, b_off; };
struct HifiganPlan { long out_len; size_t buf_floats, workspace_bytes, packed_bytes; int n_layers; };
int hifigan_layers(const HifiganConfig& c, std::vector<HifiganLayer>* out, size_t* packed_floats);
int hifigan_plan(const HifiganConfig& c, int B, int T, HifiganPlan* out);
int hifigan_pack(const HifiganConfig& c, const float* const* weights, const float* const* biases, int n_layers, float* packed, hipStream_t s);
struct HifiganFwd { int B, T, n_mel; const float* packed; const float* mel; float* workspace; float* audio; float* pre_tanh; };
int hifigan_forward(const HifiganConfig& c, const HifiganFwd& a, hipStream_t s);

constexpr int kStftTile = 32;
constexpr int kStftMaxN = 4096;
constexpr int kStftMaxOverlap = 64;
struct StftPlan { int cutoff, overlap, bin_tiles, kchunks, col_tiles; long out_len; size_t fwd_floats, inv_floats, wsq_floats; };
int stft_plan(int N, int hop, int nf, StftPlan* out);
int stft_pack(int N, int hop, const float* fwd, const float* inv, const double* wsq, float* packed, hipStream_t s);
struct StftAnalysis { int B, N, hop; long n; const float* x; const float* packed; float* re; float* im; float* mag; float* phase; };
int stft_analysis(const StftAnalysis& a, hipStream_t s);
struct StftSynthesis { int B, N, hop, nf, mode, windowed; const float* a; const float* b; const float* bias; float strength; const float* packed; float* y; };
int stft_synthesis(const StftSynthesis& a, hipStream_t s);
int stft_pack_forward(int N, const float* fwd, float* packed, hipStream_t s);

constexpr int kMelMaxMels = 128;
constexpr int kMelPassBins = 64;
constexpr int kMelSplitBelow = 768;
__host__ __device__ inline long mel_frames(long len, int N, int hop, int pad) {
    return (len > pad && len + 2L * pad >= N) ? (len + 2L * pad - N) / hop + 1 : 0;
}
struct MelPlan { int cutoff, bin_tiles, kchunks, passes, row_tiles, splits; long nf_max, frame_tiles; size_t fwd_floats, mel_floats, split_scratch_floats; };
int melspec_plan(int N, int hop, int pad, int n_mels, long n, int B, MelPlan* out);
int melspec_pack(int N, int n_mels, const float* fwd, const float* melb, float* packed, hipStream_t s);
struct MelSpecArgs {
    int B, N, hop, pad, n_mels; long n;
    const float* x; const int* lengths; const float* packed; float* out; float* scratch; size_t scratch_floats; int* frame_lengths;
    float mag_eps, clip_val, C, pad_value;
    int time_major, return_power, force_splits;
};
int melspec(const MelSpecArgs& a, hipStream_t s);

struct AdamTensor { float* p; const float* g; float* m; float* v; long numel; int first_chunk; int pad_; };
int adam_chunks(long numel);
int adam_norm(const AdamTensor* table_dev, int n_tensors, int n_chunks, float* partial, float* norm_out, float max_norm, hipStream_t s);
int adam_step(const AdamTensor* table_dev, int n_tensors, int n_chunks, float* partial, float* norm_out, float max_norm,
              float lr, float b1, float b2, float eps, float wd, int step, hipStream_t s);

int rng_keep_mask(uint64_t seed, uint32_t site, uint32_t n, float p, uint8_t* out, hipStream_t s);
int rng_normal(uint64_t seed, uint32_t site, uint32_t n, float* out, hipStream_t s);
int teacher_inputs(const float* mel, float* X, int B, int M, int T, hipStream_t s);
int transpose_btc_to_bct(const float* in, float* out, int B, int T, int C, const int* lengths, float fill, hipStream_t s);
int mask_bt(float* x, int B, int T, const int* lengths, float fill, hipStream_t s);
int mask_btc(float* x, int B, int T, int C, const int* lengths, float fill, hipStream_t s);
int fill_f32(float* p, float v, size_t n, hipStream_t s);
int permute_rows(const float* in, float* out, int R1, int R2, int W, hipStream_t s);
int relu_drop_bwd(const float* dy, const float* y, float* dz, float scale, size_t n, hipStream_t s);
int colsum(const float* X, long ld, int M, int N, float* out, float* out2, float* scratch, hipStream_t s);
int colsum_finish(const float* partials, int M, int N, float* out, hipStream_t s);
int fold_halves(float* X, size_t rows, int A, hipStream_t s);
int batch_sum(const float* X, int B, int n, float* out, hipStream_t s);

}
```

tacotron2_subword_amd/model.py:

```python
from math import sqrt

import torch
from torch import nn

from . import _lib as L
from . import blocks
from . import ops
from .attention import (DynamicConvolutionAttention, ForwardAttentionV2, GMMAttention, LocationSensitiveAttention,
                        StepwiseMonotonicAttention)
from .layers import ConvNorm, LinearNorm
from .utils import get_mask_from_lengths, to_gpu


class Prenet(nn.Module):

    def __init__(self, in_dim, sizes):
        super().__init__()
        ins = [in_dim] + sizes[:-1]
        self.layers = nn.ModuleList([LinearNorm(i, o, bias=False) for i, o in zip(ins, sizes)])


class Postnet(nn.Module):

    def __init__(self, hparams):
        super().__init__()
        n, k = hparams.postnet_n_convolutions, hparams.postnet_kernel_size
        dims = [hparams.n_mel_channels] + [hparams.postnet_embedding_dim] * (n - 1) + [hparams.n_mel_channels]
        self.convolutions = nn.ModuleList()
        for i in range(n):
            self.convolutions.append(nn.Sequential(
                ConvNorm(dims[i], dims[i + 1], kernel_size=k, stride=1, padding=int((k - 1) / 2), dilation=1,
                         w_init_gain="tanh" if i < n - 1 else "linear"),
                nn.BatchNorm1d(dims[i + 1])))

    def forward_btc(self, x_btc, seed, residual=True):
        n = len(self.convolutions)
        layers = [(blk[0].conv, blk[1]) for blk in self.convolutions]
        return blocks.conv_bn_stack(x_btc, layers, [blocks.ACT_TANH] * (n - 1) + [blocks.ACT_NONE], training=self.training,
                                    drop_p=0.5, seed=seed, site0=L.SITE["POSTNET0"], residual=residual)

    def forward(self, x):
        y = self.forward_btc(x.transpose(1, 2).contiguous(), _next_seed(self), residual=False)
        return y.transpose(1, 2)


class Encoder(nn.Module):

    def __init__(self, hparams):
        super().__init__()
        E, k = hparams.encoder_embedding_dim, hparams.encoder_kernel_size
        self.convolutions = nn.ModuleList([
            nn.Sequential(ConvNorm(E, E, kernel_size=k, stride=1, padding=int((k - 1) / 2), dilation=1, w_init_gain="relu"),
                          nn.BatchNorm1d(E))
            for _ in range(hparams.encoder_n_convolutions)])
        self.lstm = nn.LSTM(E, int(E / 2), 1, batch_first=True, bidirectional=True)

    def forward_btc(self, x_btc, input_lengths, site0, seed):
        layers = [(blk[0].conv, blk[1]) for blk in self.convolutions]
        h = blocks.conv_bn_stack(x_btc, layers, [blocks.ACT_RELU] * len(layers), training=self.training, drop_p=0.5,
                                 seed=seed, site0=site0)
        return blocks.bilstm(h, input_lengths, self.lstm)

    def forward(self, x, input_lengths):
        return self.forward_btc(x.transpose(1, 2).contiguous(), input_lengths, L.SITE["ENC0"], _next_seed(self))

    def inference(self, x):
        return self.forward_btc(x.transpose(1, 2).contiguous(), None, L.SITE["ENC0"], _next_seed(self))


def _next_seed(module):
    module._t2_calls = getattr(module, "_t2_calls", 0) + 1
    rank = torch.distributed.get_rank() if torch.distributed.is_available() and torch.distributed.is_initialized() else 0
    return ((getattr(module, "base_seed", 1234) * 1000003 + module._t2_calls) * 64 + rank) & ((1 << 63) - 1)


class _FinalizeFn(torch.autograd.Function):

    @staticmethod
    def forward(ctx, x_btc, lengths, fill):
        return ops.finalize_bct(x_btc.contiguous(), lengths, fill)

    @staticmethod
    def backward(ctx, d):
        return d.transpose(1, 2).contiguous(), None, None


class _DecoderFn(torch.autograd.Function):

    @staticmethod
    def forward(ctx, memory, memory_sub, mels, mem_lengths, sub_lengths, cfg, *params):
# ... 145 lines not shown
                                              *self._params())
        return (mel if channels_last else mel.transpose(1, 2)), gate, al, alb

    def inference(self, memory, embeddings, channels_last=False):
        P, W = self._weights()
        with torch.no_grad():
            dp, steps, stop = ops.decoder_infer(W, self.dims, memory.contiguous(), None if embeddings is None else embeddings.contiguous(),
                                                max_steps=int(self.max_decoder_steps), gate_threshold=float(self.gate_threshold),
                                                prenet_dropout=self.prenet_dropout, seed=self._next_seed())
        stop = stop.cpu()
        ops.check_chain_status()
        flag = bool((stop >= 0).all())
        n = int(stop.max()) + 1 if flag else steps
        self.last_stop_index = stop
        self.last_steps_run, self.last_overshoot = steps, steps - n
        mel = dp.mel[:, :n]
        return ((mel if channels_last else mel.transpose(1, 2)), dp.gate[:, :n].unsqueeze(-1), dp.align[:, :n], dp.align_sub[:, :n], flag)


class BERT_Tacotron2(nn.Module):

    def __init__(self, hparams):
        super().__init__()
        hp = hparams
        self.mask_padding, self.fp16_run = hp.mask_padding, hp.fp16_run
        self.n_mel_channels, self.n_frames_per_step = hp.n_mel_channels, hp.n_frames_per_step
        self.embedding = nn.Embedding(hp.n_symbols, hp.symbols_embedding_dim)
        self.embedding_sub = nn.Embedding(hp.sub_n_symbols, hp.symbols_embedding_dim)
        val = sqrt(3.0) * sqrt(2.0 / (hp.n_symbols + hp.symbols_embedding_dim))
        self.embedding.weight.data.uniform_(-val, val)
        self.embedding_sub.weight.data.uniform_(-val, val)
        self.encoder = Encoder(hp)
        self.encoder_sub = Encoder(hp)
        self.linear_converter = LinearNorm(hp.encoder_embedding_dim + hp.BERT_embedding_dim, hp.encoder_embedding_dim)
        self.linear_converter_sub = LinearNorm(hp.encoder_embedding_dim + hp.BERT_embedding_dim, hp.encoder_embedding_dim)
        self.decoder = Decoder(hp)
        self.postnet = Postnet(hp)
        self.overlap_encoders, self._t2_side = True, None

    def parse_batch(self, batch):
        text, il, ilb, mel, gate, ol, sub, pcls, bcls, align = batch
        hm = getattr(batch, "host_max", None)
        if hm is None and not (il.is_cuda or ilb.is_cuda or ol.is_cuda):
            hm = (int(torch.max(torch.cat((il, ilb), 0))), int(torch.max(ol)))
        text, il, ilb = to_gpu(text).long(), to_gpu(il).long(), to_gpu(ilb).long()
        if hm is None:
            hm = (int(torch.max(torch.cat((il, ilb), 0)).item()), int(torch.max(ol).item()))
        max_in, max_out = int(hm[0]), int(hm[1])
        mel, gate, ol, align = to_gpu(mel).float(), to_gpu(gate).float(), to_gpu(ol).long(), to_gpu(align).float()
        return ((text, il, ilb, mel, (max_in, max_out), ol, to_gpu(sub), to_gpu(pcls), to_gpu(bcls)), (mel, gate, align))

    def parse_output(self, outputs, output_lengths=None):
        if self.mask_padding and output_lengths is not None:
            mask = ~get_mask_from_lengths(output_lengths, outputs[0].size(2))
            outputs[0].data.masked_fill_(mask[:, None, :], 0.0)
            outputs[1].data.masked_fill_(mask[:, None, :], 0.0)
            outputs[2].data.masked_fill_(mask, 1e3)
        return outputs

    def _front(self, ids, lengths, cls, sub, seed):
        emb, enc, conv = ((self.embedding_sub, self.encoder_sub, self.linear_converter_sub) if sub
                          else (self.embedding, self.encoder, self.linear_converter))
        x = blocks.embedding(ids, emb.weight)
        h = enc.forward_btc(x, lengths, L.SITE["ENCSUB0" if sub else "ENC0"], seed)
        cat = torch.cat([h, cls[:, :h.size(1)]], 2)
        return blocks.linear(cat, conv.linear_layer.weight, conv.linear_layer.bias)

    def _fronts(self, text, tl, pcls, sub_ids, bl, bcls, seed):
        if not (self.overlap_encoders and text.is_cuda):
            return self._front(text, tl, pcls, False, seed), self._front(sub_ids, bl, bcls, True, seed)
        cur = torch.cuda.current_stream()
        if self._t2_side is None:
            self._t2_side = torch.cuda.Stream(device=text.device)
        side = self._t2_side
        side.wait_stream(cur)
        with torch.cuda.stream(side):
            memory_sub = self._front(sub_ids, bl, bcls, True, seed)
        memory = self._front(text, tl, pcls, False, seed)
        cur.wait_stream(side)
        memory_sub.record_stream(cur)
        return memory, memory_sub

    def forward(self, inputs):
        text, tl, bl, mels, _, ol, sub_ids, pcls, bcls = inputs
        tl, bl, ol = tl.data, bl.data, ol.data
        seed = _next_seed(self)
        pre = None
        if self.overlap_encoders and text.is_cuda:
            pre = self.decoder.prologue(mels, text.shape[0], text.shape[1], sub_ids.shape[1])
        memory, memory_sub = self._fronts(text, tl, pcls, sub_ids, bl, bcls, seed)
        mel_btc, gate, al, alb = self.decoder(memory, memory_sub, mels, tl, bl, channels_last=True, pre=pre)
        post_btc = self.postnet.forward_btc(mel_btc, seed)
        if self.mask_padding and ol is not None:
            mel = _FinalizeFn.apply(mel_btc, ol, 0.0)
            post = _FinalizeFn.apply(post_btc, ol, 0.0)
            gate = gate.clone()
            ops.mask_bt_(gate.data, ol, 1e3)
            ops.mask_btc_(mel_btc.data, ol, 0.0)
        else:
            mel = _FinalizeFn.apply(mel_btc, None, 0.0)
            post = _FinalizeFn.apply(post_btc, None, 0.0)
        return [mel, post, gate, al, alb]

    def inference(self, inputs, embeddings, phoneme_embeddings_cls, bert_embeddings_cls):
        seed = _next_seed(self)
        memory, memory_sub = self._fronts(inputs, None, phoneme_embeddings_cls, embeddings, None, bert_embeddings_cls, seed)
        mel_btc, gate, al, alb, flag = self.decoder.inference(memory, memory_sub, channels_last=True)
        mel_btc = mel_btc.contiguous()
        post_btc = self.postnet.forward_btc(mel_btc, seed)
        return [ops.finalize_bct(mel_btc, None, 0.0), ops.finalize_bct(post_btc, None, 0.0), gate, al, alb, flag]


class Tacotron2(nn.Module):

    def __init__(self, hparams):
        super().__init__()
        hp = hparams
        self.mask_padding, self.fp16_run = hp.mask_padding, hp.fp16_run
        self.n_mel_channels, self.n_frames_per_step = hp.n_mel_channels, hp.n_frames_per_step
        self.embedding = nn.Embedding(hp.n_symbols, hp.symbols_embedding_dim)
        val = sqrt(3.0) * sqrt(2.0 / (hp.n_symbols + hp.symbols_embedding_dim))
        self.embedding.weight.data.uniform_(-val, val)
        self.encoder = Encoder(hp)
        self.decoder = Decoder(hp, single=True)
        self.postnet = Postnet(hp)

    def parse_batch(self, batch):
        text, il, mel, gate, ol = batch
        max_len = None if il.is_cuda else int(torch.max(il))
        text, il = to_gpu(text).long(), to_gpu(il).long()
        if max_len is None:
            max_len = int(torch.max(il).item())
        mel, gate, ol = to_gpu(mel).float(), to_gpu(gate).float(), to_gpu(ol).long()
        return ((text, il, mel, max_len, ol), (mel, gate))

    def forward(self, inputs):
        text, tl, mels, _, ol = inputs
        tl, ol = tl.data, ol.data
        seed = _next_seed(self)
        memory = self.encoder.forward_btc(blocks.embedding(text, self.embedding.weight), tl, L.SITE["ENC0"], seed)
        mel_btc, gate, al, _ = self.decoder(memory, None, mels, tl, None, channels_last=True)
        post_btc = self.postnet.forward_btc(mel_btc, seed)
        use_mask = self.mask_padding and ol is not None
        mel = _FinalizeFn.apply(mel_btc, ol if use_mask else None, 0.0)
        post = _FinalizeFn.apply(post_btc, ol if use_mask else None, 0.0)
        if use_mask:
            gate = gate.clone()
            ops.mask_bt_(gate.data, ol, 1e3)
            ops.mask_btc_(mel_btc.data, ol, 0.0)
        return [mel, post, gate, al]

    def inference(self, inputs):
        seed = _next_seed(self)
        memory = self.encoder.forward_btc(blocks.embedding(inputs, self.embedding.weight), None, L.SITE["ENC0"], seed)
        mel_btc, gate, al, _, flag = self.decoder.inference(memory, None, channels_last=True)
        mel_btc = mel_btc.contiguous()
        post_btc = self.postnet.forward_btc(mel_btc, seed)
        return [ops.finalize_bct(mel_btc, None, 0.0), ops.finalize_bct(post_btc, None, 0.0), gate, al]
```

Before: 1.062 million mel-frames/s.

## Batch weight bf16 casts into one prepare launch and share bf16 operand copies

Adds a per-model registry that records which weights need bf16 casts, transposed casts, conv-weight repacks and bias sums. At the start of each forward it runs all of them in a single batched kernel launch, so individual GEMMs and convs can take prepared weights instead of casting them per call. Linear and LSTM input-projection GEMMs now pass shared bf16 copy buffers, so the activation cast done in forward is reused by backward, and dy casts are shared between the dx and dW GEMMs. This saves many small cast kernels but keeps extra bf16 buffers alive and adds Python bookkeeping per call.

```diff
diff --git a/include/t2amd.h b/include/t2amd.h
--- a/include/t2amd.h
+++ b/include/t2amd.h
@@ -213,6 +213,24 @@
     const void* x16; int handoff;
 } t2_conv_bn_bwd_args;
 int t2_conv_bn_backward(const t2_conv_bn_bwd_args* a, void* stream);
+typedef struct t2_conv_prepared { const void* w; int bf16; int kind_out; } t2_conv_prepared;
+int t2_conv_bn_forward_prepared(const t2_conv_bn_args* a, t2_conv_prepared* p, void* stream);
+int t2_conv_bn_backward_prepared(const t2_conv_bn_bwd_args* a, t2_conv_prepared* p, void* stream);
+
+enum { T2_PREP_CAST_ROWS = 0, T2_PREP_CAST_TRANSPOSE = 1, T2_PREP_CONV_W_FWD = 2, T2_PREP_CONV_W_BWD = 3, T2_PREP_SUM2 = 4 };
+#define T2_PREP_CHUNK 8192
+#define T2_PREP_MAX_TAPS 7
+typedef struct t2_prep_row {
+    const float* src; const float* src2; void* dst;
+    long lds, ldd;
+    int kind, out_bf16;
+    int d0, d1, d2;
+    int first_chunk, n_chunks, tiles_x;
+} t2_prep_row;
+int t2_prep_plan_row(t2_prep_row* row, int first_chunk);
+int t2_prepare_operands(const t2_prep_row* table_dev, int n_rows, int n_chunks, void* stream);
+int t2_prep_counts(uint64_t* out_host, int reset);
+int t2_set_prep_fuse(int on);
 
 int t2_embedding_forward(const int64_t* ids, const float* table, float* out, int rows, int dim, void* stream);
 int t2_embedding_backward(const int64_t* ids, const float* dout, float* dtable, int rows, int dim, int vocab, void* stream);
@@ -248,6 +266,12 @@
     float* ws; size_t ws_bytes; int splitk;
 } t2_gemm_args;
 int t2_gemm_ex(const t2_gemm_args* a, void* stream);
+typedef struct t2_gemm_copies {
+    void* A16; long lda16; int a16_kmajor; int a_ready;
+    void* B16; long ldb16; int b16_kmajor; int b_ready;
+    int a_taken, b_taken;
+} t2_gemm_copies;
+int t2_gemm_ex16(const t2_gemm_args* a, t2_gemm_copies* c, void* stream);
 int t2_prof_gemm(const t2_gemm_args* a, int reps, float* ms_total, float* ms_kernel, void* stream);
 enum { T2_GEMM_F32_64 = 0, T2_GEMM_F32_128, T2_GEMM_BF16CONV, T2_GEMM_SRC128, T2_GEMM_SRC256, T2_GEMM_SRC256KM };
 enum { T2_GEMM_OPERAND_FP32 = 0, T2_GEMM_OPERAND_STAGED, T2_GEMM_OPERAND_CALLER };
diff --git a/tacotron2_subword_amd/_lib.py b/tacotron2_subword_amd/_lib.py
--- a/tacotron2_subword_amd/_lib.py
+++ b/tacotron2_subword_amd/_lib.py
@@ -121,6 +121,26 @@
                 ("x16", C.c_void_p), ("handoff", C.c_int)]
 
 
+class GemmCopies(C.Structure):
+    _fields_ = [("A16", C.c_void_p), ("lda16", C.c_long), ("a16_kmajor", C.c_int), ("a_ready", C.c_int),
+                ("B16", C.c_void_p), ("ldb16", C.c_long), ("b16_kmajor", C.c_int), ("b_ready", C.c_int),
+                ("a_taken", C.c_int), ("b_taken", C.c_int)]
+
+
+class ConvPrepared(C.Structure):
+    _fields_ = [("w", C.c_void_p), ("bf16", C.c_int), ("kind_out", C.c_int)]
+
+
+PREP_CAST_ROWS, PREP_CAST_TRANSPOSE, PREP_CONV_W_FWD, PREP_CONV_W_BWD, PREP_SUM2 = range(5)
+PREP_CHUNK, PREP_MAX_TAPS = 8192, 7
+
+
+class PrepRow(C.Structure):
+    _fields_ = [("src", C.c_void_p), ("src2", C.c_void_p), ("dst", C.c_void_p), ("lds", C.c_long), ("ldd", C.c_long),
+                ("kind", C.c_int), ("out_bf16", C.c_int), ("d0", C.c_int), ("d1", C.c_int), ("d2", C.c_int),
+                ("first_chunk", C.c_int), ("n_chunks", C.c_int), ("tiles_x", C.c_int)]
+
+
 _P4 = C.c_void_p * 4
 _I4 = C.c_int * 4
 
@@ -470,8 +490,9 @@
 
 EXPORTS = ["t2_last_error", "t2_version", "t2_chain_status", "t2_chain_status_clear", "t2_debug_report_abort", "t2_debug_occupy", "t2_chain_claimed", "t2_set_precision", "t2_get_precision", "t2_gemm_counts", "t2_set_gemm_split_min_mflop", "t2_set_split_steps", "t2_get_split_steps", "t2_step_counts", "t2_set_overlap", "t2_set_chain", "t2_get_chain", "t2_set_chain_bwd", "t2_set_gemm_staging", "t2_set_gemm_fold", "t2_set_bn_fuse", "t2_get_bn_fuse", "t2_bn_fuse_counts", "t2_side_join", "t2_defer_counts", "t2_decoder_layout_query", "t2_decoder_forward", "t2_decoder_infer",
            "t2_decoder_bwd_layout_query", "t2_decoder_backward", "t2_decoder_pass_plan", "t2_prof_enable", "t2_prof_collect", "t2_adam_chunks", "t2_adam_step", "t2_adam_norm",
-           "t2_conv_bn_forward", "t2_conv_bn_backward", "t2_embedding_forward", "t2_embedding_backward",
-           "t2_lstm_seq_forward", "t2_lstm_seq_backward", "t2_lstm_seq_chain_ws_floats", "t2_gemm_ex", "t2_prof_gemm", "t2_gemm_plan", "t2_chain_plan", "t2_conv_handoff_plan", "t2_colsum", "t2_mask_btc",
+           "t2_conv_bn_forward", "t2_conv_bn_backward", "t2_conv_bn_forward_prepared", "t2_conv_bn_backward_prepared",
+           "t2_prep_plan_row", "t2_prepare_operands", "t2_prep_counts", "t2_set_prep_fuse", "t2_embedding_forward", "t2_embedding_backward",
+           "t2_lstm_seq_forward", "t2_lstm_seq_backward", "t2_lstm_seq_chain_ws_floats", "t2_gemm_ex", "t2_gemm_ex16", "t2_prof_gemm", "t2_gemm_plan", "t2_chain_plan", "t2_conv_handoff_plan", "t2_colsum", "t2_mask_btc",
            "t2_finalize_bct", "t2_mask_bt", "t2_gemm", "t2_rng_keep_mask", "t2_rng_normal",
            "t2_softdtw_plan", "t2_softdtw_dist", "t2_softdtw_forward", "t2_softdtw_backward", "t2_softdtw_dist_backward",
            "t2_ssim_plan", "t2_ssim_forward", "t2_ssim_backward",
@@ -517,12 +538,19 @@
                                            C.POINTER(DecoderPassPlanInfo)]
         L.t2_conv_bn_forward.argtypes = [C.POINTER(ConvBnArgs), C.c_void_p]
         L.t2_conv_bn_backward.argtypes = [C.POINTER(ConvBnBwdArgs), C.c_void_p]
+        L.t2_conv_bn_forward_prepared.argtypes = [C.POINTER(ConvBnArgs), C.POINTER(ConvPrepared), C.c_void_p]
+        L.t2_conv_bn_backward_prepared.argtypes = [C.POINTER(ConvBnBwdArgs), C.POINTER(ConvPrepared), C.c_void_p]
+        L.t2_prep_plan_row.argtypes = [C.POINTER(PrepRow), C.c_int]
+        L.t2_prepare_operands.argtypes = [C.c_void_p, C.c_int, C.c_int, C.c_void_p]
+        L.t2_prep_counts.argtypes = [C.POINTER(C.c_uint64), C.c_int]
+        L.t2_set_prep_fuse.argtypes = [C.c_int]
         L.t2_embedding_forward.argtypes = [C.c_void_p, C.c_void_p, C.c_void_p, C.c_int, C.c_int, C.c_void_p]
         L.t2_embedding_backward.argtypes = [C.c_void_p, C.c_void_p, C.c_void_p, C.c_int, C.c_int, C.c_int, C.c_void_p]
         L.t2_lstm_seq_forward.argtypes = [C.POINTER(LstmSeqArgs), C.c_void_p]
         L.t2_lstm_seq_backward.argtypes = [C.POINTER(LstmSeqBwdArgs), C.c_void_p]
         L.t2_lstm_seq_chain_ws_floats.argtypes, L.t2_lstm_seq_chain_ws_floats.restype = [C.c_int, C.c_int, C.c_int, C.c_int], C.c_size_t
         L.t2_gemm_ex.argtypes = [C.POINTER(GemmArgs), C.c_void_p]
+        L.t2_gemm_ex16.argtypes = [C.POINTER(GemmArgs), C.POINTER(GemmCopies), C.c_void_p]
         L.t2_prof_gemm.argtypes = [C.POINTER(GemmArgs), C.c_int, C.POINTER(C.c_float), C.POINTER(C.c_float), C.c_void_p]
         L.t2_gemm_plan.argtypes = [C.POINTER(GemmArgs), C.POINTER(GemmPlanOpts), C.POINTER(GemmPlanInfo)]
         L.t2_chain_plan.argtypes = [C.POINTER(ChainShape), C.c_int, C.c_int, C.c_int, C.c_int, C.POINTER(ChainPlanInfo)]
diff --git a/tacotron2_subword_amd/blocks.py b/tacotron2_subword_amd/blocks.py
--- a/tacotron2_subword_amd/blocks.py
+++ b/tacotron2_subword_amd/blocks.py
@@ -5,6 +5,7 @@
 import torch
 
 from . import _lib as L
+from . import prepared
 
 ACT_NONE, ACT_RELU, ACT_TANH = 0, 1, 2
 CONV_HANDOFF = True
@@ -24,13 +25,47 @@
     return 3 if L.get_precision() == "bf16x3" else 1
 
 
+class Copy16:
+    __slots__ = ("buf", "ready", "transposed")
+
+    def __init__(self, like: torch.Tensor = None, buf: torch.Tensor = None, transposed: bool = False):
+        self.buf = torch.empty(like.shape, dtype=torch.bfloat16, device=like.device) if buf is None else buf
+        self.ready = buf is not None
+        self.transposed = transposed
+
+
+def share_copies() -> bool:
+    return prepared.enabled() and L.get_precision() == "bf16"
+
+
 def gemm_ex(A, Bm, out, M, N, K, sam, sak, sbn, sbk, ldc, *, bias=None, act=0, alpha=1.0, beta=0.0, crow_mod=0, crow_mul=0,
-            batch=1, bsA=0, bsB=0, bsC=0, splitk_ws=True):
+            batch=1, bsA=0, bsB=0, bsC=0, splitk_ws=True, a16: Copy16 = None, b16: Copy16 = None):
     ws = _scratch(out.device, (8 << 20) * _stage_terms()) if splitk_ws and beta == 0.0 else None
     a = L.GemmArgs(L.ptr(A), L.ptr(Bm), L.ptr(out), M, N, K, sam, sak, sbn, sbk, ldc, batch, bsA, bsB, bsC, alpha, beta,
                    L.ptr(bias), act, crow_mod, crow_mul, L.ptr(ws), 0 if ws is None else ws.numel() * 4, 0)
-    L.check(L.lib().t2_gemm_ex(C.byref(a), L.stream()))
-    return out
+    if a16 is None and b16 is None:
+        L.check(L.lib().t2_gemm_ex(C.byref(a), L.stream()))
+        return out
+    c = L.GemmCopies()
+    if a16 is not None:
+        c.A16, c.lda16, c.a16_kmajor, c.a_ready = a16.buf.data_ptr(), a16.buf.shape[1], int((sak != 1) != a16.transposed), int(a16.ready)
+    if b16 is not None:
+        c.B16, c.ldb16, c.b16_kmajor, c.b_ready = b16.buf.data_ptr(), b16.buf.shape[1], int((sbk != 1) != b16.transposed), int(b16.ready)
+    L.check(L.lib().t2_gemm_ex16(C.byref(a), C.byref(c), L.stream()))
+    if a16 is not None:
+        a16.ready = bool(c.a_ready)
+    if b16 is not None:
+        b16.ready = bool(c.b_ready)
+    return bool(c.a_taken), bool(c.b_taken)
+
+
+def _weight_copy(reg, W, kind):
+    hit = None if reg is None else reg.get(W, kind)
+    tr = kind == L.PREP_CAST_TRANSPOSE
+    if hit is not None:
+        return Copy16(buf=hit, transposed=tr)
+    Wd = W.detach()
+    return Copy16(like=Wd.t() if tr else Wd, transposed=tr)
 
 
 def colsum(x2d: torch.Tensor) -> torch.Tensor:
@@ -50,7 +85,16 @@
         M, K = x2.shape
         N = W.shape[0]
         y = torch.empty(M, N, dtype=torch.float32, device=x.device)
-        gemm_ex(x2, W, y, M, N, K, K, 1, W.stride(0), 1, N, bias=b)
+        ctx.x16 = ctx.wt16 = ctx.prep = None
+        if share_copies() and W.is_contiguous():
+            reg = ctx.prep = prepared.current()
+            ctx.x16, w16 = Copy16(like=x2), _weight_copy(reg, W, L.PREP_CAST_ROWS)
+            ctx.wt16 = None if reg is None else reg.get(W, L.PREP_CAST_TRANSPOSE)
+            _, took = gemm_ex(x2, W, y, M, N, K, K, 1, W.stride(0), 1, N, bias=b, a16=ctx.x16, b16=w16)
+            if took and reg is not None:
+                reg.note_cast(W, L.PREP_CAST_ROWS)
+        else:
+            gemm_ex(x2, W, y, M, N, K, K, 1, W.stride(0), 1, N, bias=b)
         ctx.save_for_backward(x2, W)
         ctx.has_bias, ctx.shape = b is not None, shape
         return y.view(*shape[:-1], N)
@@ -62,13 +106,25 @@
         N = W.shape[0]
         dy2 = dy.reshape(M, N).contiguous()
         dx = dW = db = None
+        share = ctx.x16 is not None and share_copies()
+        dy16 = Copy16(like=dy2) if share else None
         if ctx.needs_input_grad[0]:
             dx = torch.empty(M, K, dtype=torch.float32, device=dy.device)
-            gemm_ex(dy2, W, dx, M, K, N, N, 1, 1, W.stride(0), K)
+            if share:
+                wt16 = Copy16(buf=ctx.wt16, transposed=True) if ctx.wt16 is not None else _weight_copy(None, W, L.PREP_CAST_TRANSPOSE)
+                _, took = gemm_ex(dy2, W, dx, M, K, N, N, 1, 1, W.stride(0), K, a16=dy16, b16=wt16)
+                if took and ctx.prep is not None:
+                    ctx.prep.note_cast(W, L.PREP_CAST_TRANSPOSE)
+            else:
+                gemm_ex(dy2, W, dx, M, K, N, N, 1, 1, W.stride(0), K)
             dx = dx.view(ctx.shape)
         if ctx.needs_input_grad[1]:
             dW = torch.empty(N, K, dtype=torch.float32, device=dy.device)
-            gemm_ex(dy2, x2, dW, N, K, M, 1, N, 1, K, K)
+            if share:
+                gemm_ex(dy2, x2, dW, N, K, M, 1, N, 1, K, K, a16=dy16, b16=ctx.x16)
+            else:
+                gemm_ex(dy2, x2, dW, N, K, M, 1, N, 1, K, K)
+        ctx.x16 = None
         if ctx.has_bias and ctx.needs_input_grad[2]:
             db = colsum(dy2)
         return dx, dW, db
@@ -101,6 +157,15 @@
 
 def embedding(ids, table):
     return _EmbeddingFn.apply(ids, table)
+
+
+def _conv_prepared(hit) -> L.ConvPrepared:
+    return L.ConvPrepared(None, 0, -1) if hit is None else L.ConvPrepared(hit[0].data_ptr(), int(hit[1]), -1)
+
+
+def _note_conv(cfg, i: int, kind: int, p: L.ConvPrepared) -> None:
+    if cfg["prep"] is not None:
+        cfg["prep"].note_conv(cfg["weights"][i], kind, p.kind_out)
 
 
 class _ConvStackFn(torch.autograd.Function):
@@ -130,7 +195,9 @@
                              cfg["drop_p"] if cfg["training"] else 0.0, cfg["seed"], cfg["site0"] + i, L.ptr(res),
                              L.ptr(z), L.ptr(st[0]), L.ptr(st[1]), L.ptr(st[2]), L.ptr(y), L.ptr(ws), ws.numel(),
                              L.ptr(cur16), L.ptr(y16), int(handoff))
-            L.check(L.lib().t2_conv_bn_forward(C.byref(a), L.stream()))
+            wp = _conv_prepared(cfg["wfwd"][i])
+            L.check(L.lib().t2_conv_bn_forward_prepared(C.byref(a), C.byref(wp), L.stream()))
+            _note_conv(cfg, i, L.PREP_CONV_W_FWD, wp)
             saved.append((cur, z, st, cur16))
             cur, cur16 = y, y16
         ctx.cfg, ctx.saved_acts, ctx.params, ctx.handoff = cfg, saved, [p.detach() for p in params], handoff
@@ -160,7 +227,9 @@
                                 int(cfg["training"]), 1e-5, cfg["acts"][i], cfg["drop_p"] if cfg["training"] else 0.0, cfg["seed"],
                                 cfg["site0"] + i, L.ptr(dy), L.ptr(dw), L.ptr(db), L.ptr(dg), L.ptr(dbt), L.ptr(dx), 0,
                                 L.ptr(ws), ws.numel(), L.ptr(xin16), int(ctx.handoff and L.get_precision() == "bf16"))
-            L.check(L.lib().t2_conv_bn_backward(C.byref(a), L.stream()))
+            wp = _conv_prepared(cfg["wbwd"][i])
+            L.check(L.lib().t2_conv_bn_backward_prepared(C.byref(a), C.byref(wp), L.stream()))
+            _note_conv(cfg, i, L.PREP_CONV_W_BWD, wp)
             grads[4 * i:4 * i + 4] = [dw, db, dg, dbt]
             dy = dx
         if dy is not None and d_res is not None:
@@ -174,10 +243,13 @@
     for conv, bn in layers:
         params += [conv.weight, conv.bias, bn.weight, bn.bias]
         buffers.append((bn.running_mean, bn.running_var))
-        if training:
-            bn.num_batches_tracked += 1
+    if training:
+        torch._foreach_add_([bn.num_batches_tracked for _, bn in layers], 1)
+    prep = prepared.current()
+    weights = [conv.weight for conv, _ in layers]
+    hits = lambda kind: [None if prep is None else prep.conv_weight(w, kind) for w in weights]
     cfg = dict(acts=list(acts), buffers=buffers, training=bool(training), drop_p=float(drop_p), seed=int(seed), site0=int(site0),
-               residual=bool(residual))
+               residual=bool(residual), prep=prep, weights=weights, wfwd=hits(L.PREP_CONV_W_FWD), wbwd=hits(L.PREP_CONV_W_BWD))
     return _ConvStackFn.apply(x, cfg, *params)
 
 
@@ -190,9 +262,24 @@
         dev = x.device
         xt = x.transpose(0, 1).contiguous()
         pre = torch.empty(2, T * B, 4 * H, dtype=torch.float32, device=dev)
-        bsum = torch.stack((b_ih.detach() + b_hh.detach(), b_ih_r.detach() + b_hh_r.detach()))
+        reg = ctx.prep = prepared.current()
+        share = share_copies() and w_ih.is_contiguous() and w_ih_r.is_contiguous()
+        bsum = []
+        for bi, bh in ((b_ih, b_hh), (b_ih_r, b_hh_r)):
+            hit = None if reg is None else reg.get(bi, L.PREP_SUM2)
+            bsum.append(bi.detach() + bh.detach() if hit is None else hit)
+            if reg is not None:
+                reg.note_sum(bi, bh)
+        ctx.xt16, ctx.wt16 = (Copy16(like=xt.view(T * B, E)) if share else None), [None, None]
         for d, W in enumerate((w_ih, w_ih_r)):
-            gemm_ex(xt, W.detach(), pre[d], T * B, 4 * H, E, E, 1, W.stride(0), 1, 4 * H, bias=bsum[d])
+            if share:
+                w16 = _weight_copy(reg, W, L.PREP_CAST_ROWS)
+                ctx.wt16[d] = None if reg is None else reg.get(W, L.PREP_CAST_TRANSPOSE)
+                _, took = gemm_ex(xt, W.detach(), pre[d], T * B, 4 * H, E, E, 1, W.stride(0), 1, 4 * H, bias=bsum[d], a16=ctx.xt16, b16=w16)
+                if took and reg is not None:
+                    reg.note_cast(W, L.PREP_CAST_ROWS)
+            else:
+                gemm_ex(xt, W.detach(), pre[d], T * B, 4 * H, E, E, 1, W.stride(0), 1, 4 * H, bias=bsum[d])
         out = torch.empty(T, B, 2 * H, dtype=torch.float32, device=dev)
         cells = torch.empty(2, T, B, H, dtype=torch.float32, device=dev)
         gates = torch.empty(2, T, B, 4 * H, dtype=torch.float32, device=dev)
@@ -240,12 +327,22 @@
         TB = T * B
         dxt = torch.empty(TB, E, dtype=torch.float32, device=dev)
         res = []
+        share = ctx.xt16 is not None and share_copies()
         for d, W in enumerate((w_ih, w_ih_r)):
-            gemm_ex(dpre[d], W, dxt, TB, E, 4 * H, 4 * H, 1, 1, W.stride(0), E, beta=float(d))
             dW = torch.empty(4 * H, E, dtype=torch.float32, device=dev)
-            gemm_ex(dpre[d], xt, dW, 4 * H, E, TB, 1, 4 * H, 1, E, E)
+            if share:
+                dp16 = Copy16(like=dpre[d])
+                wt16 = Copy16(buf=ctx.wt16[d], transposed=True) if ctx.wt16[d] is not None else _weight_copy(None, W, L.PREP_CAST_TRANSPOSE)
+                _, took = gemm_ex(dpre[d], W, dxt, TB, E, 4 * H, 4 * H, 1, 1, W.stride(0), E, beta=float(d), a16=dp16, b16=wt16)
+                if took and ctx.prep is not None:
+                    ctx.prep.note_cast(W, L.PREP_CAST_TRANSPOSE)
+                gemm_ex(dpre[d], xt, dW, 4 * H, E, TB, 1, 4 * H, 1, E, E, a16=dp16, b16=ctx.xt16)
+            else:
+                gemm_ex(dpre[d], W, dxt, TB, E, 4 * H, 4 * H, 1, 1, W.stride(0), E, beta=float(d))
+                gemm_ex(dpre[d], xt, dW, 4 * H, E, TB, 1, 4 * H, 1, E, E)
             db = colsum(dpre[d])
             res.append((dW, dwhh[d], db, db))
+        ctx.xt16 = None
         dx = dxt.view(T, B, E).transpose(0, 1).contiguous()
         return (dx, None) + res[0] + res[1]
 
diff --git a/tacotron2_subword_amd/build.py b/tacotron2_subword_amd/build.py
--- a/tacotron2_subword_amd/build.py
+++ b/tacotron2_subword_amd/build.py
@@ -7,7 +7,7 @@
 _HERE = os.path.dirname(os.path.abspath(__file__))
 CSRC = os.path.join(_HERE, "csrc")
 OUT = os.path.join(_HERE, "libt2amd.so")
-SOURCES = ["gemm.hip", "gemm_f32.hip", "gemm_bf16conv.hip", "gemm_dispatch.hip", "lstm.hip", "chain_plan.hip", "chain.hip", "chain_bwd.hip", "chain_enc.hip", "attention.hip", "attention_lsa_bwd.hip", "attention_gmm.hip", "attention_dca.hip", "conv.hip", "elementwise.hip", "infer.hip", "optim.hip", "softdtw.hip", "ssim.hip", "bert.hip", "vocoder.hip", "waveglow.hip", "stft.hip", "melspec.hip", "decoder_plan.hip", "decoder.hip", "c_api.hip"]
+SOURCES = ["gemm.hip", "gemm_f32.hip", "gemm_bf16conv.hip", "gemm_dispatch.hip", "lstm.hip", "chain_plan.hip", "chain.hip", "chain_bwd.hip", "chain_enc.hip", "attention.hip", "attention_lsa_bwd.hip", "attention_gmm.hip", "attention_dca.hip", "conv.hip", "elementwise.hip", "infer.hip", "optim.hip", "prepare.hip", "softdtw.hip", "ssim.hip", "bert.hip", "vocoder.hip", "waveglow.hip", "stft.hip", "melspec.hip", "decoder_plan.hip", "decoder.hip", "c_api.hip"]
 
 
 def _newest(paths):
diff --git a/tacotron2_subword_amd/csrc/c_api.hip b/tacotron2_subword_amd/csrc/c_api.hip
--- a/tacotron2_subword_amd/csrc/c_api.hip
+++ b/tacotron2_subword_amd/csrc/c_api.hip
@@ -234,7 +234,7 @@
     return 0;
 }
 
-int t2_conv_bn_forward(const t2_conv_bn_args* a, void* stream) {
+int t2_conv_bn_forward_prepared(const t2_conv_bn_args* a, t2_conv_prepared* p, void* stream) {
     T2_REQUIRE(a, "null argument");
     const size_t nw = (size_t)a->Cout * a->Cin * a->K;
     T2_REQUIRE(a->ws_floats >= nw + 128 * (size_t)a->Cout, "t2_conv_bn_forward: workspace too small");
@@ -247,10 +247,12 @@
     const size_t used = align4(nw) + 128 * (size_t)a->Cout;
     if (a->ws_floats > used) { f.gemm_ws = a->ws + used; f.gemm_ws_bytes = (a->ws_floats - used) * sizeof(float); }
     f.handoff = a->handoff; f.x16 = static_cast<const __bf16*>(a->x16); f.y16 = static_cast<__bf16*>(a->y16);
+    if (p) { f.wprep = p->w; f.wprep_bf16 = p->bf16; f.wkind_out = &p->kind_out; }
     return conv_bn_fwd(f, (hipStream_t)stream);
 }
-
-int t2_conv_bn_backward(const t2_conv_bn_bwd_args* a, void* stream) {
+int t2_conv_bn_forward(const t2_conv_bn_args* a, void* stream) { return t2_conv_bn_forward_prepared(a, nullptr, stream); }
+
+int t2_conv_bn_backward_prepared(const t2_conv_bn_bwd_args* a, t2_conv_prepared* p, void* stream) {
     T2_REQUIRE(a, "null argument");
     const size_t nw = align4((size_t)a->Cout * a->Cin * a->K), ndz = align4((size_t)a->B * a->T * a->Cout), nsc = 128 * (size_t)a->Cout;
     T2_REQUIRE(a->ws_floats >= nw + ndz + nsc, "t2_conv_bn_backward: workspace too small");
@@ -263,8 +265,23 @@
     f.dz = a->ws; f.wperm = a->ws + ndz; f.scratch = a->ws + ndz + nw;
     f.gemm_ws = a->ws + ndz + nw + nsc; f.gemm_ws_bytes = (a->ws_floats - (ndz + nw + nsc)) * sizeof(float);
     f.handoff = a->handoff; f.x16 = static_cast<const __bf16*>(a->x16);
+    if (p) { f.wprep = p->w; f.wprep_bf16 = p->bf16; f.wkind_out = &p->kind_out; }
     return conv_bn_bwd(f, (hipStream_t)stream);
 }
+int t2_conv_bn_backward(const t2_conv_bn_bwd_args* a, void* stream) { return t2_conv_bn_backward_prepared(a, nullptr, stream); }
+
+static_assert(sizeof(t2_prep_row) == sizeof(PrepRow) && sizeof(PrepRow) == 72 && T2_PREP_MAX_TAPS == kPrepMaxK &&
+              (int)T2_PREP_SUM2 == (int)PREP_SUM2 && (int)T2_PREP_CONV_W_BWD == (int)PREP_CONV_W_BWD, "t2_prep_row mirrors PrepRow");
+int t2_prep_plan_row(t2_prep_row* row, int first_chunk) { return prep_plan_row(reinterpret_cast<PrepRow*>(row), first_chunk); }
+int t2_prepare_operands(const t2_prep_row* table_dev, int n_rows, int n_chunks, void* stream) {
+    return prepare_operands(reinterpret_cast<const PrepRow*>(table_dev), n_rows, n_chunks, (hipStream_t)stream);
+}
+int t2_prep_counts(uint64_t* out_host, int reset) {
+    T2_REQUIRE(out_host, "null argument");
+    prep_counts(out_host, reset);
+    return 0;
+}
+int t2_set_prep_fuse(int on) { set_prep_fuse(on); return 0; }
 
 int t2_embedding_forward(const int64_t* ids, const float* table, float* out, int rows, int dim, void* stream) {
     return embedding_fwd(reinterpret_cast<const long*>(ids), table, out, rows, dim, (hipStream_t)stream);
@@ -386,6 +403,31 @@
     T2_REQUIRE(a, "null argument");
     return gemm(desc_of(*a), (hipStream_t)stream);
 }
+int t2_gemm_ex16(const t2_gemm_args* a, t2_gemm_copies* c, void* stream) {
+    T2_REQUIRE(a && c, "null argument");
+    hipStream_t s = (hipStream_t)stream;
+    const GemmDesc plain = desc_of(*a);
+    c->a_taken = c->b_taken = 0;
+    GemmPlan p0;
+    T2_TRY(gemm_plan(plain, &p0));
+    for (int mask = 3; mask >= 1; --mask) {
+        const bool ta = mask & 1, tb = mask & 2;
+        if ((ta && !c->A16) || (tb && !c->B16)) continue;
+        if ((ta && p0.a.src != GemmSrc::staged) || (tb && p0.b.src != GemmSrc::staged)) continue;
+        GemmDesc g = plain;
+        if (ta) { g.A16 = static_cast<const __bf16*>(c->A16); g.lda16 = c->lda16; g.a16_kmajor = c->a16_kmajor; }
+        if (tb) { g.B16 = static_cast<const __bf16*>(c->B16); g.ldb16 = c->ldb16; g.b16_kmajor = c->b16_kmajor; }
+        if ((ta && c->lda16 != p0.a.ld) || (tb && c->ldb16 != p0.b.ld)) continue;
+        const size_t skip = (ta ? p0.a.bytes : 0) + (tb ? p0.b.bytes : 0);
+        g.ws = reinterpret_cast<float*>(reinterpret_cast<unsigned char*>(plain.ws) + skip); g.ws_bytes = plain.ws_bytes - skip;
+        if (!gemm_handoff(plain, g)) continue;
+        if (ta && !c->a_ready) { T2_TRY(stage_planned(plain.A, p0.a, false, static_cast<__bf16*>(c->A16), s)); c->a_ready = 1; }
+        if (tb && !c->b_ready) { T2_TRY(stage_planned(plain.B, p0.b, false, static_cast<__bf16*>(c->B16), s)); c->b_ready = 1; }
+        c->a_taken = ta; c->b_taken = tb;
+        return gemm(g, s);
+    }
+    return gemm(plain, s);
+}
 static GemmDesc desc_of(const t2_gemm_args& a, const t2_gemm_plan_opts* o) {
     GemmDesc g = desc_of(a);
     if (o) {
diff --git a/tacotron2_subword_amd/csrc/conv.hip b/tacotron2_subword_amd/csrc/conv.hip
--- a/tacotron2_subword_amd/csrc/conv.hip
+++ b/tacotron2_subword_amd/csrc/conv.hip
@@ -30,6 +30,7 @@
 }
 template <class OUT>
 void permute_w(bool bwd, const float* w, OUT* out, int Co, int Ci, int K, hipStream_t s) {
+    prep_count(PREP_COUNT_RELAYOUTS);
     const size_t n = (size_t)Co * Ci * K;
     const dim3 grid(grid_for(n)), block(256);
     if (n < (1ull << 31)) {
@@ -365,6 +366,9 @@
 }
 inline bool aligned8(const void* p) { return (reinterpret_cast<uintptr_t>(p) & 7) == 0; }
 inline size_t round256(size_t n) { return (n + 255) & ~(size_t)255; }
+inline bool prepared_ok(const void* prep, int prep_bf16, bool want_bf16, const float* wperm) {
+    return prep && (prep_bf16 != 0) == want_bf16 && (reinterpret_cast<uintptr_t>(prep) & 15) == 0 && (reinterpret_cast<uintptr_t>(wperm) & 15) == 0;
+}
 inline bool same_route(const GemmPlan& p, const GemmPlan& q) { return p.kernel == q.kernel && p.split == q.split && p.splitk == q.splitk && p.kchunks == q.kchunks; }
 
 std::atomic<int> g_bn_fuse{env_int("T2_BN_FUSE", 1)};
@@ -425,12 +429,16 @@
     GemmDesc g16 = g;
     g16.A16 = a.x16; g16.lda16 = a.Cin;
     g16.B16 = reinterpret_cast<const __bf16*>(a.wperm); g16.ldb16 = (long)a.K * a.Cin;
-    if (a.handoff && gemm_handoff(g, g16)) {
-        g = g16;
-        permute_w(false, a.w, reinterpret_cast<__bf16*>(a.wperm), a.Cout, a.Cin, a.K, s);
-    } else
-        permute_w(false, a.w, a.wperm, a.Cout, a.Cin, a.K, s);
-    T2_LAUNCH_CHECK();
+    const bool w16 = a.handoff && gemm_handoff(g, g16);
+    if (w16) g = g16;
+    if (a.wkind_out) *a.wkind_out = w16;
+    if (prepared_ok(a.wprep, a.wprep_bf16, w16, a.wperm)) {
+        if (w16) g.B16 = static_cast<const __bf16*>(a.wprep); else g.B = static_cast<const float*>(a.wprep);
+    } else {
+        if (w16) permute_w(false, a.w, reinterpret_cast<__bf16*>(a.wperm), a.Cout, a.Cin, a.K, s);
+        else permute_w(false, a.w, a.wperm, a.Cout, a.Cin, a.K, s);
+        T2_LAUNCH_CHECK();
+    }
     T2_TRY_RC(gemm(g, s));
     BnElem e{a.z, a.mean, a.invstd, a.gamma, a.beta, a.Cout, a.act, a.drop_p, rng_key(a.seed, a.site)};
     const size_t n = (size_t)M * a.Cout;
@@ -532,10 +540,15 @@
         hipLaunchKernelGGL(unpermute_dw_kernel, dim3(grid_for(nw)), dim3(256), 0, s, a.wperm, a.dw, a.Cout, a.Cin, a.K);
         T2_LAUNCH_CHECK();
     }
+    if (a.wkind_out) *a.wkind_out = a.dx ? (int)w16 : -1;
     if (a.dx) {
-        if (w16) permute_w(true, a.w, reinterpret_cast<__bf16*>(a.wperm), a.Cout, a.Cin, a.K, s);
-        else permute_w(true, a.w, a.wperm, a.Cout, a.Cin, a.K, s);
-        T2_LAUNCH_CHECK();
+        if (prepared_ok(a.wprep, a.wprep_bf16, w16, a.wperm)) {
+            if (w16) h.B16 = static_cast<const __bf16*>(a.wprep); else h.B = static_cast<const float*>(a.wprep);
+        } else {
+            if (w16) permute_w(true, a.w, reinterpret_cast<__bf16*>(a.wperm), a.Cout, a.Cin, a.K, s);
+            else permute_w(true, a.w, a.wperm, a.Cout, a.Cin, a.K, s);
+            T2_LAUNCH_CHECK();
+        }
         T2_TRY_RC(gemm(h, s));
     }
     return 0;
diff --git a/tacotron2_subword_amd/csrc/decoder.hip b/tacotron2_subword_amd/csrc/decoder.hip
--- a/tacotron2_subword_amd/csrc/decoder.hip
+++ b/tacotron2_subword_amd/csrc/decoder.hip
@@ -166,6 +166,27 @@
     const Sizes& z = c.z;
     const long K = z.Ha + z.E, ldi = z.P + z.E;
     const size_t loa = (size_t)4 * z.Ha * K, lod = (size_t)4 * z.Hd * z.Hd;
+    if (!split && get_prep_fuse() && 4 * z.NS + 2 <= kPrepArgRows) {
+        PrepRow rows[kPrepArgRows];
+        int n = 0;
+        auto part = [&](const float* src, long lds, __bf16* dst, long ldd, int r, int cc, bool transpose) {
+            PrepRow p{};
+            p.src = src; p.dst = dst; p.lds = lds; p.ldd = ldd; p.d0 = r; p.d1 = cc;
+            p.kind = transpose ? PREP_CAST_TRANSPOSE : PREP_CAST_ROWS;
+            rows[n++] = p;
+        };
+        for (int s = 0; s < z.NS; ++s) {
+            const t2_lstm_weights& lw = *c.st[s].lw;
+            __bf16 *f = c.P16(c.st[s].w16), *tr = c.P16(c.st[s].wt16);
+            part(lw.w_hh, z.Ha, f, K, 4 * z.Ha, z.Ha, false);
+            part(lw.w_ih + z.P, ldi, f + z.Ha, K, 4 * z.Ha, z.E, false);
+            part(lw.w_ih + z.P, ldi, tr, 4 * z.Ha, 4 * z.Ha, z.E, true);
+            part(lw.w_hh, z.Ha, tr + (long)z.E * 4 * z.Ha, 4 * z.Ha, 4 * z.Ha, z.Ha, true);
+        }
+        part(c.w.dec.w_hh, z.Hd, c.P16(c.L.w16d), z.Hd, 4 * z.Hd, z.Hd, false);
+        part(c.w.dec.w_hh, z.Hd, c.P16(c.L.wt16d), 4 * z.Hd, 4 * z.Hd, z.Hd, true);
+        return prepare_rows(rows, n, c.s);
+    }
     for (int s = 0; s < z.NS; ++s) {
         const t2_lstm_weights& lw = *c.st[s].lw;
         __bf16 *f = c.P16(c.st[s].w16), *tr = c.P16(c.st[s].wt16);
diff --git a/tacotron2_subword_amd/csrc/gemm.hip b/tacotron2_subword_amd/csrc/gemm.hip
--- a/tacotron2_subword_amd/csrc/gemm.hip
+++ b/tacotron2_subword_amd/csrc/gemm.hip
@@ -492,6 +492,7 @@
 }
 
 int stage_planned(const float* src, const GemmOperandPlan& o, bool split, __bf16* dst, hipStream_t s) {
+    prep_count(PREP_COUNT_STAGING);
     return gemm_detail::launch_stage(src, o.kc, o.ld_src, dst, o.rows, o.K, split, o.lo_slot, o.row_group, s);
 }
 
diff --git a/tacotron2_subword_amd/csrc/kernels.h b/tacotron2_subword_amd/csrc/kernels.h
--- a/tacotron2_subword_amd/csrc/kernels.h
+++ b/tacotron2_subword_amd/csrc/kernels.h
@@ -334,6 +334,7 @@
     float* gemm_ws; size_t gemm_ws_bytes;
     int handoff;
     const __bf16* x16; __bf16* y16;
+    const void* wprep; int wprep_bf16; int* wkind_out;
 };
 int conv_bn_fwd(const ConvBnFwd& a, hipStream_t s);
 void set_bn_fuse(int on);
@@ -351,6 +352,7 @@
     float* wperm; float* scratch; float* gemm_ws; size_t gemm_ws_bytes;
     int handoff;
     const __bf16* x16;
+    const void* wprep; int wprep_bf16; int* wkind_out;
 };
 int conv_bn_bwd(const ConvBnBwd& a, hipStream_t s);
 int embedding_fwd(const long* ids, const float* table, float* out, int rows, int D, hipStream_t s);
@@ -454,6 +456,19 @@
 int adam_step(const AdamTensor* table_dev, int n_tensors, int n_chunks, float* partial, float* norm_out, float max_norm,
               float lr, float b1, float b2, float eps, float wd, int step, hipStream_t s);
 
+enum PrepKind : int { PREP_CAST_ROWS = 0, PREP_CAST_TRANSPOSE = 1, PREP_CONV_W_FWD = 2, PREP_CONV_W_BWD = 3, PREP_SUM2 = 4 };
+enum PrepCount : int { PREP_COUNT_LAUNCHES = 0, PREP_COUNT_STAGING = 1, PREP_COUNT_RELAYOUTS = 2 };
+constexpr int kPrepMaxK = 7;
+constexpr int kPrepArgRows = 10;
+struct PrepRow { const float* src; const float* src2; void* dst; long lds, ldd; int kind, out_bf16; int d0, d1, d2; int first_chunk, n_chunks, tiles_x; };
+int prep_plan_row(PrepRow* row, int first_chunk);
+int prepare_operands(const PrepRow* table_dev, int n_rows, int n_chunks, hipStream_t s);
+int prepare_rows(const PrepRow* rows_host, int n_rows, hipStream_t s);
+void prep_count(int which);
+void set_prep_fuse(int on);
+int get_prep_fuse();
+void prep_counts(uint64_t* out, int reset);
+
 int rng_keep_mask(uint64_t seed, uint32_t site, uint32_t n, float p, uint8_t* out, hipStream_t s);
 int rng_normal(uint64_t seed, uint32_t site, uint32_t n, float* out, hipStream_t s);
 int teacher_inputs(const float* mel, float* X, int B, int M, int T, hipStream_t s);
diff --git a/tacotron2_subword_amd/csrc/prepare.hip b/tacotron2_subword_amd/csrc/prepare.hip
--- /dev/null
+++ b/tacotron2_subword_amd/csrc/prepare.hip
@@ -0,0 +1,230 @@
+#include "kernels.h"
+#include <atomic>
+#include <cstdlib>
+
+namespace t2 {
+
+namespace {
+
+constexpr int kPrepChunk = 8192;
+constexpr int kPrepTile = 32;
+constexpr int kPrepThreads = 256;
+constexpr int kPrepLds = kPrepTile * (kPrepTile * kPrepMaxK + 1);
+
+typedef __bf16 bf16x8 __attribute__((ext_vector_type(8)));
+typedef __bf16 bf16x4v __attribute__((ext_vector_type(4)));
+
+__host__ __device__ inline bool al16(const void* p) { return (reinterpret_cast<uintptr_t>(p) & 15) == 0; }
+
+template <class OUT, int V>
+__device__ __forceinline__ void store_out(OUT* p, const float* v) {
+    if constexpr (V == 1) *p = (OUT)v[0];
+    else if constexpr (sizeof(OUT) == 4) {
+        static_assert(V == 4, "fp32 rows are written 16 bytes wide");
+        f32x4 t; t[0] = v[0]; t[1] = v[1]; t[2] = v[2]; t[3] = v[3];
+        *reinterpret_cast<f32x4*>(p) = t;
+    } else if constexpr (V == 4) {
+        bf16x4v t;
+#pragma unroll
+        for (int e = 0; e < 4; ++e) t[e] = (__bf16)v[e];
+        *reinterpret_cast<bf16x4v*>(p) = t;
+    } else {
+        bf16x8 t;
+#pragma unroll
+        for (int e = 0; e < 8; ++e) t[e] = (__bf16)v[e];
+        *reinterpret_cast<bf16x8*>(p) = t;
+    }
+}
+
+template <class OUT, int V, bool BWD>
+__device__ __forceinline__ void conv_tile_write(const float* lds, OUT* dst, int Co, int Ci, int K, int co0, int ci0, int nco, int nci) {
+    const int P = kPrepTile * K + 1;
+    const int nrun = BWD ? nco : nci, nrow = BWD ? nci : nco;
+    const int groups = nrun / V;
+    const int total = nrow * K * groups;
+    for (int t = threadIdx.x; t < total; t += kPrepThreads) {
+        const int g = t % groups, rest = t / groups, dk = rest % K, row = rest / K;
+        float v[V];
+#pragma unroll
+        for (int e = 0; e < V; ++e)
+            v[e] = BWD ? lds[(g * V + e) * P + row * K + (K - 1 - dk)] : lds[row * P + (g * V + e) * K + dk];
+        const size_t o = BWD ? ((size_t)(ci0 + row) * K + dk) * Co + co0 + g * V : ((size_t)(co0 + row) * K + dk) * Ci + ci0 + g * V;
+        store_out<OUT, V>(dst + o, v);
+    }
+}
+template <class OUT, bool BWD>
+__device__ __forceinline__ void conv_tile(const PrepRow& r, int local, float* lds) {
+    const int Co = r.d0, Ci = r.d1, K = r.d2, P = kPrepTile * K + 1;
+    const int co0 = (local / r.tiles_x) * kPrepTile, ci0 = (local % r.tiles_x) * kPrepTile;
+    const int nco = min(kPrepTile, Co - co0), nci = min(kPrepTile, Ci - ci0);
+    const int L = nci * K;
+    if (Ci % 4 == 0 && al16(r.src)) {
+        const int q4 = L / 4;
+        for (int t = threadIdx.x; t < nco * q4; t += kPrepThreads) {
+            const int co_l = t / q4, q = t % q4;
+            const f32x4 x = *reinterpret_cast<const f32x4*>(r.src + ((size_t)(co0 + co_l) * Ci + ci0) * K + 4 * q);
+#pragma unroll
+            for (int e = 0; e < 4; ++e) lds[co_l * P + 4 * q + e] = x[e];
+        }
+    } else {
+        for (int t = threadIdx.x; t < nco * L; t += kPrepThreads) {
+            const int co_l = t / L, j = t % L;
+            lds[co_l * P + j] = r.src[((size_t)(co0 + co_l) * Ci + ci0) * K + j];
+        }
+    }
+    __syncthreads();
+    OUT* dst = static_cast<OUT*>(r.dst);
+    const int ext = BWD ? Co : Ci;
+    if (sizeof(OUT) == 2 && ext % 8 == 0 && al16(dst)) conv_tile_write<OUT, sizeof(OUT) == 2 ? 8 : 4, BWD>(lds, dst, Co, Ci, K, co0, ci0, nco, nci);
+    else if (ext % 4 == 0 && al16(dst)) conv_tile_write<OUT, 4, BWD>(lds, dst, Co, Ci, K, co0, ci0, nco, nci);
+    else conv_tile_write<OUT, 1, BWD>(lds, dst, Co, Ci, K, co0, ci0, nco, nci);
+}
+
+__device__ __forceinline__ void cast_rows_chunk(const PrepRow& r, int local) {
+    const int C = r.d1;
+    const size_t n = (size_t)r.d0 * C, off = (size_t)local * kPrepChunk;
+    const int cnt = (int)min((size_t)kPrepChunk, n - off);
+    __bf16* dst = static_cast<__bf16*>(r.dst);
+    if (C % 4 == 0 && r.lds % 4 == 0 && r.ldd % 4 == 0 && al16(r.src) && (reinterpret_cast<uintptr_t>(dst) & 7) == 0) {
+        for (int q = threadIdx.x; q < cnt / 4; q += kPrepThreads) {
+            const size_t i = off + 4 * (size_t)q, rr = i / C; const int c = (int)(i % C);
+            const f32x4 x = *reinterpret_cast<const f32x4*>(r.src + rr * r.lds + c);
+            const float v[4] = {x[0], x[1], x[2], x[3]};
+            store_out<__bf16, 4>(dst + rr * r.ldd + c, v);
+        }
+    } else {
+        for (int j = threadIdx.x; j < cnt; j += kPrepThreads) {
+            const size_t i = off + j, rr = i / C; const int c = (int)(i % C);
+            dst[rr * r.ldd + c] = (__bf16)r.src[rr * r.lds + c];
+        }
+    }
+}
+__device__ __forceinline__ void sum2_chunk(const PrepRow& r, int local) {
+    const size_t n = (size_t)r.d0, off = (size_t)local * kPrepChunk;
+    const int cnt = (int)min((size_t)kPrepChunk, n - off);
+    const float* a = r.src + off; const float* b = r.src2 + off; float* dst = static_cast<float*>(r.dst) + off;
+    for (int j = threadIdx.x; j < cnt; j += kPrepThreads) dst[j] = a[j] + b[j];
+}
+__device__ __forceinline__ void cast_transpose_tile(const PrepRow& r, int local, float* lds) {
+    const int R = r.d0, C = r.d1;
+    const int r0 = (local / r.tiles_x) * kPrepTile, c0 = (local % r.tiles_x) * kPrepTile;
+    const int tx = threadIdx.x & 31, ty = threadIdx.x >> 5;
+    __bf16* dst = static_cast<__bf16*>(r.dst);
+    for (int i = ty; i < 32; i += 8) {
+        const int rr = r0 + i, c = c0 + tx;
+        lds[i * 33 + tx] = (rr < R && c < C) ? r.src[(size_t)rr * r.lds + c] : 0.f;
+    }
+    __syncthreads();
+    for (int i = ty; i < 32; i += 8) {
+        const int c = c0 + i, rr = r0 + tx;
+        if (c < C && rr < R) dst[(size_t)c * r.ldd + rr] = (__bf16)lds[tx * 33 + i];
+    }
+}
+
+__device__ __forceinline__ void prep_chunk(const PrepRow& r, int local, float* lds) {
+    if (local < 0 || local >= r.n_chunks) return;
+    switch (r.kind) {
+    case PREP_CAST_ROWS: cast_rows_chunk(r, local); break;
+    case PREP_CAST_TRANSPOSE: cast_transpose_tile(r, local, lds); break;
+    case PREP_CONV_W_FWD: if (r.out_bf16) conv_tile<__bf16, false>(r, local, lds); else conv_tile<float, false>(r, local, lds); break;
+    case PREP_CONV_W_BWD: if (r.out_bf16) conv_tile<__bf16, true>(r, local, lds); else conv_tile<float, true>(r, local, lds); break;
+    case PREP_SUM2: sum2_chunk(r, local); break;
+    default: break;
+    }
+}
+
+__global__ __launch_bounds__(kPrepThreads) void prepare_table_kernel(const PrepRow* __restrict__ tab, int n) {
+    __shared__ float lds[kPrepLds];
+    const int chunk = blockIdx.x;
+    int lo = 0, hi = n - 1;
+    while (lo < hi) {
+        const int mid = (lo + hi + 1) >> 1;
+        if (tab[mid].first_chunk <= chunk) lo = mid; else hi = mid - 1;
+    }
+    const PrepRow r = tab[lo];
+    prep_chunk(r, chunk - r.first_chunk, lds);
+}
+struct PrepRowsArg { PrepRow r[kPrepArgRows]; int n; };
+__global__ __launch_bounds__(kPrepThreads) void prepare_rows_kernel(PrepRowsArg a) {
+    __shared__ float lds[kPrepLds];
+    const int chunk = blockIdx.x;
+    int i = 0;
+    while (i + 1 < a.n && a.r[i + 1].first_chunk <= chunk) ++i;
+    prep_chunk(a.r[i], chunk - a.r[i].first_chunk, lds);
+}
+
+std::atomic<uint64_t> g_prep_counts[3];
+
+}
+
+static std::atomic<int> g_prep_fuse{getenv("T2_PREP_FUSE") && *getenv("T2_PREP_FUSE") ? atoi(getenv("T2_PREP_FUSE")) != 0 : 1};
+void set_prep_fuse(int on) { g_prep_fuse = on != 0; }
+int get_prep_fuse() { return g_prep_fuse; }
+void prep_count(int which) { ++g_prep_counts[which]; }
+void prep_counts(uint64_t* out, int reset) {
+    for (int i = 0; i < 3; ++i) { out[i] = g_prep_counts[i]; if (reset) g_prep_counts[i] = 0; }
+}
+
+int prep_plan_row(PrepRow* r, int first_chunk) {
+    T2_REQUIRE(r && first_chunk >= 0, "prep_plan_row: bad arguments");
+    T2_REQUIRE(r->src && r->dst, "prep_plan_row: a row needs a source and a destination");
+    long chunks = 0;
+    r->tiles_x = 0;
+    auto tiles = [](long n) { return (n + kPrepTile - 1) / kPrepTile; };
+    switch (r->kind) {
+    case PREP_CAST_ROWS:
+        T2_REQUIRE(r->d0 >= 1 && r->d1 >= 1 && r->lds >= r->d1 && r->ldd >= r->d1, "prep_plan_row: cast rows R=%d C=%d lds=%ld ldd=%ld", r->d0, r->d1, r->lds, r->ldd);
+        chunks = ((long)r->d0 * r->d1 + kPrepChunk - 1) / kPrepChunk;
+        r->out_bf16 = 1;
+        break;
+    case PREP_CAST_TRANSPOSE:
+        T2_REQUIRE(r->d0 >= 1 && r->d1 >= 1 && r->lds >= r->d1 && r->ldd >= r->d0, "prep_plan_row: cast transpose R=%d C=%d lds=%ld ldd=%ld", r->d0, r->d1, r->lds, r->ldd);
+        r->tiles_x = (int)tiles(r->d1);
+        chunks = tiles(r->d0) * r->tiles_x;
+        r->out_bf16 = 1;
+        break;
+    case PREP_CONV_W_FWD:
+    case PREP_CONV_W_BWD:
+        T2_REQUIRE(r->d0 >= 1 && r->d1 >= 1 && r->d2 >= 1 && r->d2 <= kPrepMaxK, "prep_plan_row: conv weights [%d,%d,%d]: up to %d taps", r->d0, r->d1, r->d2, kPrepMaxK);
+        T2_REQUIRE((long)r->d0 * r->d1 * r->d2 < (1l << 31), "prep_plan_row: conv weights too large");
+        r->tiles_x = (int)tiles(r->d1);
+        chunks = tiles(r->d0) * r->tiles_x;
+        break;
+    case PREP_SUM2:
+        T2_REQUIRE(r->d0 >= 1 && r->src2, "prep_plan_row: a sum needs two sources and a length");
+        chunks = ((long)r->d0 + kPrepChunk - 1) / kPrepChunk;
+        r->out_bf16 = 0;
+        break;
+    default:
+        T2_REQUIRE(false, "prep_plan_row: unknown kind %d", r->kind);
+    }
+    T2_REQUIRE(first_chunk + chunks < (1l << 30), "prep_plan_row: too many chunks");
+    r->first_chunk = first_chunk;
+    r->n_chunks = (int)chunks;
+    return 0;
+}
+
+int prepare_operands(const PrepRow* table_dev, int n_rows, int n_chunks, hipStream_t s) {
+    T2_REQUIRE(table_dev && n_rows >= 1 && n_chunks >= 1, "prepare_operands: bad arguments");
+    hipLaunchKernelGGL(prepare_table_kernel, dim3(n_chunks), dim3(kPrepThreads), 0, s, table_dev, n_rows);
+    T2_LAUNCH_CHECK();
+    prep_count(PREP_COUNT_LAUNCHES);
+    return 0;
+}
+
+int prepare_rows(const PrepRow* rows_host, int n_rows, hipStream_t s) {
+    T2_REQUIRE(rows_host && n_rows >= 1 && n_rows <= kPrepArgRows, "prepare_rows: 1..%d rows", kPrepArgRows);
+    PrepRowsArg a{};
+    int chunk = 0;
+    for (int i = 0; i < n_rows; ++i) {
+        a.r[i] = rows_host[i];
+        T2_TRY_RC(prep_plan_row(&a.r[i], chunk));
+        chunk += a.r[i].n_chunks;
+    }
+    a.n = n_rows;
+    hipLaunchKernelGGL(prepare_rows_kernel, dim3(chunk), dim3(kPrepThreads), 0, s, a);
+    T2_LAUNCH_CHECK();
+    return 0;
+}
+
+}
diff --git a/tacotron2_subword_amd/model.py b/tacotron2_subword_amd/model.py
--- a/tacotron2_subword_amd/model.py
+++ b/tacotron2_subword_amd/model.py
@@ -6,6 +6,7 @@
 from . import _lib as L
 from . import blocks
 from . import ops
+from . import prepared
 from .attention import (DynamicConvolutionAttention, ForwardAttentionV2, GMMAttention, LocationSensitiveAttention,
                         StepwiseMonotonicAttention)
 from .layers import ConvNorm, LinearNorm
@@ -317,6 +318,10 @@
         return memory, memory_sub
 
     def forward(self, inputs):
+        with prepared.of(self).scope():
+            return self._forward(inputs)
+
+    def _forward(self, inputs):
         text, tl, bl, mels, _, ol, sub_ids, pcls, bcls = inputs
         tl, bl, ol = tl.data, bl.data, ol.data
         seed = _next_seed(self)
@@ -338,6 +343,10 @@
         return [mel, post, gate, al, alb]
 
     def inference(self, inputs, embeddings, phoneme_embeddings_cls, bert_embeddings_cls):
+        with prepared.of(self).scope():
+            return self._inference(inputs, embeddings, phoneme_embeddings_cls, bert_embeddings_cls)
+
+    def _inference(self, inputs, embeddings, phoneme_embeddings_cls, bert_embeddings_cls):
         seed = _next_seed(self)
         memory, memory_sub = self._fronts(inputs, None, phoneme_embeddings_cls, embeddings, None, bert_embeddings_cls, seed)
         mel_btc, gate, al, alb, flag = self.decoder.inference(memory, memory_sub, channels_last=True)
@@ -370,6 +379,10 @@
         return ((text, il, mel, max_len, ol), (mel, gate))
 
     def forward(self, inputs):
+        with prepared.of(self).scope():
+            return self._forward(inputs)
+
+    def _forward(self, inputs):
         text, tl, mels, _, ol = inputs
         tl, ol = tl.data, ol.data
         seed = _next_seed(self)
@@ -386,6 +399,10 @@
         return [mel, post, gate, al]
 
     def inference(self, inputs):
+        with prepared.of(self).scope():
+            return self._inference(inputs)
+
+    def _inference(self, inputs):
         seed = _next_seed(self)
         memory = self.encoder.forward_btc(blocks.embedding(inputs, self.embedding.weight), None, L.SITE["ENC0"], seed)
         mel_btc, gate, al, _, flag = self.decoder.inference(memory, None, channels_last=True)
diff --git a/tacotron2_subword_amd/prepared.py b/tacotron2_subword_amd/prepared.py
--- /dev/null
+++ b/tacotron2_subword_amd/prepared.py
@@ -0,0 +1,162 @@
+from __future__ import annotations
+
+import contextlib
+import ctypes as C
+import os
+import weakref
+
+import torch
+
+from . import _lib as L
+
+_enabled = os.environ.get("T2_PREPARED", "1") != "0"
+_current = None
+
+
+def set_enabled(on: bool) -> None:
+    global _enabled
+    _enabled = bool(on)
+
+
+def enabled() -> bool:
+    return _enabled
+
+
+def current():
+    return _current if _enabled else None
+
+
+def counts(reset: bool = False):
+    out = (C.c_uint64 * 3)()
+    L.check(L.lib().t2_prep_counts(out, int(reset)))
+    return tuple(int(v) for v in out)
+
+
+def plan_rows(rows) -> int:
+    chunk = 0
+    for r in rows:
+        L.check(L.lib().t2_prep_plan_row(C.byref(r), chunk))
+        chunk += r.n_chunks
+    return chunk
+
+
+def conv_row(w: torch.Tensor, dst: torch.Tensor, backward: bool) -> L.PrepRow:
+    Co, Ci, K = w.shape
+    return L.PrepRow(src=w.data_ptr(), src2=None, dst=dst.data_ptr(), lds=0, ldd=0, kind=L.PREP_CONV_W_BWD if backward else L.PREP_CONV_W_FWD,
+                     out_bf16=int(dst.dtype == torch.bfloat16), d0=Co, d1=Ci, d2=K)
+
+
+def _row(kind, w: torch.Tensor, dst: torch.Tensor, other=None) -> L.PrepRow:
+    if kind in (L.PREP_CONV_W_FWD, L.PREP_CONV_W_BWD):
+        return conv_row(w, dst, kind == L.PREP_CONV_W_BWD)
+    if kind == L.PREP_SUM2:
+        return L.PrepRow(src=w.data_ptr(), src2=other.data_ptr(), dst=dst.data_ptr(), kind=kind, d0=w.numel())
+    R, Cc = w.shape
+    return L.PrepRow(src=w.data_ptr(), src2=None, dst=dst.data_ptr(), lds=Cc, ldd=R if kind == L.PREP_CAST_TRANSPOSE else Cc, kind=kind, out_bf16=1, d0=R, d1=Cc)
+
+
+BACKWARD_ONLY = (L.PREP_CONV_W_BWD, L.PREP_CAST_TRANSPOSE)
+
+
+class _Demand:
+    __slots__ = ("ref", "kind", "bf16", "buf", "other")
+
+    def __init__(self, p, kind, bf16, other=None):
+        self.ref, self.kind, self.bf16, self.buf = weakref.ref(p), kind, bool(bf16), None
+        self.other = None if other is None else weakref.ref(other)
+
+
+class Registry:
+
+    def __init__(self):
+        self.demands = {}
+        self.valid = {}
+        self.launches = 0
+        self._table = None
+        self._depth = 0
+
+    def conv_weight(self, w: torch.Tensor, kind: int):
+        return self.valid.get((id(w), kind))
+
+    def note_conv(self, w: torch.Tensor, kind: int, kind_out: int) -> None:
+        if kind_out < 0 or w.dim() != 3 or w.shape[2] > L.PREP_MAX_TAPS or w.dtype != torch.float32 or not w.is_contiguous():
+            return
+        d = self.demands.get((id(w), kind))
+        if d is None or d.ref() is not w:
+            self.demands[(id(w), kind)] = _Demand(w, kind, kind_out)
+        elif d.bf16 != bool(kind_out):
+            d.bf16, d.buf = bool(kind_out), None
+
+    def get(self, w: torch.Tensor, kind: int):
+        hit = self.valid.get((id(w), kind))
+        return None if hit is None else hit[0]
+
+    def note_cast(self, w: torch.Tensor, kind: int) -> None:
+        d = self.demands.get((id(w), kind))
+        if (d is None or d.ref() is not w) and w.dim() == 2 and w.dtype == torch.float32 and w.is_contiguous():
+            self.demands[(id(w), kind)] = _Demand(w, kind, True)
+
+    def note_sum(self, a: torch.Tensor, b: torch.Tensor) -> None:
+        d = self.demands.get((id(a), L.PREP_SUM2))
+        if (d is None or d.ref() is not a or d.other() is not b) and a.shape == b.shape and a.dtype == b.dtype == torch.float32 and \
+                a.is_contiguous() and b.is_contiguous():
+            self.demands[(id(a), L.PREP_SUM2)] = _Demand(a, L.PREP_SUM2, False, b)
+
+    @contextlib.contextmanager
+    def scope(self):
+        global _current
+        if not _enabled or self._depth:
+            yield self
+            return
+        outer = _current
+        self._depth, _current = 1, self
+        try:
+            self._prepare()
+            yield self
+        finally:
+            self._depth, _current = 0, outer
+            self.valid = {}
+
+    def _prepare(self) -> None:
+        grad = torch.is_grad_enabled()
+        live, sig, dev = [], [], None
+        for key, d in list(self.demands.items()):
+            w = d.ref()
+            if w is None:
+                del self.demands[key]
+                continue
+            other = None if d.other is None else d.other()
+            if d.other is not None and other is None:
+                del self.demands[key]
+                continue
+            dev = w.device if dev is None else dev
+            if w.device != dev or (d.kind in BACKWARD_ONLY and not grad):
+                continue
+            dt = torch.bfloat16 if d.bf16 else torch.float32
+            shape = tuple(w.shape[::-1]) if d.kind == L.PREP_CAST_TRANSPOSE else (w.numel(),) if w.dim() == 3 else tuple(w.shape)
+            if d.buf is None or d.buf.dtype != dt or tuple(d.buf.shape) != shape or d.buf.device != dev:
+                d.buf = torch.empty(shape, dtype=dt, device=dev)
+            live.append((key, d, w, other))
+            sig.append((w.data_ptr(), None if other is None else other.data_ptr(), d.buf.data_ptr(), d.kind, d.bf16, tuple(w.shape)))
+        if not live:
+            return
+        if self._table is None or self._table[0] != sig:
+            rows = (L.PrepRow * len(live))(*[_row(d.kind, w, d.buf, other) for _, d, w, other in live])
+            chunks = plan_rows(rows)
+            host = torch.frombuffer(bytearray(bytes(rows)), dtype=torch.uint8)
+            self._table = (sig, host.to(dev), len(live), chunks)
+        _, table, n, chunks = self._table
+        self._launch(table, n, chunks)
+        self.launches += 1
+        self.valid = {key: (d.buf, d.bf16) for key, d, _, _ in live}
+
+    @staticmethod
+    def _launch(table: torch.Tensor, n: int, chunks: int) -> None:
+        L.check(L.lib().t2_prepare_operands(table.data_ptr(), n, chunks, L.stream()))
+
+
+def of(model) -> Registry:
+    r = model.__dict__.get("_t2_prepared")
+    if r is None:
+        r = model.__dict__["_t2_prepared"] = Registry()
+    return r
```

After: 1.072 million mel-frames/s (median of 6 runs). Within noise of the previous version (+0.9%).
